# mozendr/FHE-SPEAR

Measured on AMD Instinct MI355X. Metric: BSGS matvecs/sec at d=2048,N=16384,L0=36; sec/RWKV-block at 1/2/4/8 GPU, higher is better.
Workload: dtype u64

## Files before the change

### fhe-spear_amd/csrc/fhs_host.hip

```cpp
#include <execinfo.h>
#include <hip/hip_runtime.h>
#include <unistd.h>

#include <algorithm>
#include <csignal>
#include <atomic>
#include <cmath>
#include <complex>
#include <cstdio>
#include <cstring>
#include <map>
#include <unordered_map>
#include <chrono>
#include <memory>
#include <mutex>
#include <set>
#include <string>
#include <thread>
#include <vector>

#include "../../include/fhespear.h"
#include "fhs_kernels.h"
#include "fhs_modarith.h"
#include "fhs_tables.h"

using fhs::DevTables;
using fhs::KsItem;

static thread_local std::string g_err;
static fhs_status fail(fhs_status code, const std::string& msg) {
    g_err = msg;
    return code;
}
static void segv_trace(int sig) {
    void* fr[64];
    const int n = backtrace(fr, 64);
    static const char hdr[] = "[fhespear] native backtrace:\n";
    (void)!write(2, hdr, sizeof(hdr) - 1);
    backtrace_symbols_fd(fr, n, 2);
    signal(sig, SIG_DFL);
    raise(sig);
}
__attribute__((constructor)) static void segv_trace_install() {
    if (getenv("FHESPEAR_SEGV_TRACE")) signal(SIGSEGV, segv_trace);
}
static fhs_status hip_fail(hipError_t e, const char* where) {
    if (e == hipErrorOutOfMemory || e == hipErrorMemoryAllocation)
        return fail(FHS_ERR_OOM, std::string("HIP out of memory in ") + where);
    return fail(FHS_ERR_HIP, std::string("HIP error in ") + where + ": " + hipGetErrorString(e));
}
#define HIPCHK(expr, where)                                  \
    do {                                                     \
        hipError_t _e = (expr);                              \
        if (_e != hipSuccess) return hip_fail(_e, where);    \
    } while (0)

extern "C" const char* fhs_last_error(void) { return g_err.c_str(); }
extern "C" const char* fhs_version(void) { return "fhespear-mi355x 0.1 (gfx950)"; }
extern "C" int fhs_device_count(void) {
    int n = 0;
    if (hipGetDeviceCount(&n) != hipSuccess) return 0;
    return n;
}
extern "C" fhs_status fhs_device_pci_bus_id(int device, char* buf, int len) {
    if (!buf || len < 13) return fail(FHS_ERR_INVALID, "device_pci_bus_id: buffer of at least 13 bytes");
    hipError_t e = hipDeviceGetPCIBusId(buf, len, device);
    if (e != hipSuccess) return hip_fail(e, "device_pci_bus_id");
    return FHS_OK;
}

extern "C" fhs_status fhs_create_coeff_modulus(uint64_t N, const int* bits, int n, uint64_t* out) {
    if (!bits || !out || n <= 0 || N < 2 || (N & (N - 1))) return fail(FHS_ERR_INVALID, "create_coeff_modulus: bad args");
    for (int i = 0; i < n; ++i)
        if (bits[i] < 2 || bits[i] > 61) return fail(FHS_ERR_INVALID, "create_coeff_modulus: bit size must be in [2, 61]");
    if (!coeff_modulus_search(N, bits, n, out)) return fail(FHS_ERR_INVALID, "create_coeff_modulus: not enough primes");
    return FHS_OK;
}
extern "C" uint64_t fhs_galois_elt_from_step(int step, uint64_t N) { return galois_elt_from_step(step, N); }

struct PendingRot {
    KsItem item;
    fhs_ciphertext* out;
    const fhs_ciphertext* in;
};

struct fhs_context {
    int device = 0;
    hipStream_t st = nullptr;
    std::recursive_mutex mu;
    uint64_t N = 0;
    int logN = 0, L0 = 0, P = 0, K = 0, dnum = 0;
    std::vector<uint64_t> q;
    std::vector<uint64_t> elts;
    DevTables T{};
    std::vector<void*> tables;
    void* items_dev = nullptr;
    void* ptrs_dev = nullptr;
    std::vector<PendingRot> pending;
    int pending_l = -1;
    std::set<const void*> pending_refs;
    std::set<const void*> pending_outs;
    int debug_fail_flushes = 0;
    int debug_fail_alloc = -1;
    std::vector<std::complex<double>> fft_w;
    std::vector<std::complex<double>> dec_twist;
    std::vector<uint64_t> slot_index;
    std::atomic<uint64_t> bytes_live{0};
    std::atomic<int> refs{1};
    std::unordered_map<size_t, std::vector<void*>> free_blocks;
    std::unordered_map<const void*, uint64_t*> key_a;
    size_t cached_bytes = 0;
    size_t cache_cap = 0;
    uint64_t cache_tick = 0;
    std::unordered_map<size_t, uint64_t> size_tick;
    uint32_t timer_mask = 0;
    std::vector<hipEvent_t> timer_open;
    std::vector<std::vector<std::pair<hipEvent_t, hipEvent_t>>> timer_pairs;
    fhs::KTimer ktimer{};
    unsigned char* ring = nullptr;
    size_t ring_head = 0;
    int ring_seg = 0;
    static constexpr size_t kRingBytes = 16u << 20;
    static constexpr int kRingSegs = 8;
    static constexpr size_t kSegBytes = kRingBytes / kRingSegs;
    hipEvent_t ring_ev[kRingSegs] = {};
    uint64_t ring_waits = 0, ring_blocked = 0;
    fhs::Stager stager{};
    std::map<std::pair<int, int>, std::vector<uint64_t>> crt_cache;
    double* readback = nullptr;
    size_t readback_bytes = 0;
    std::map<std::pair<const uint64_t*, int>, uint64_t*> seal_corr;
    size_t seal_corr_bytes = 0;
    size_t seal_corr_cap = 0;
    fhs::SealHoist seal_hoist{};
    enum { SCR_KS, SCR_BSGS_INNER, SCR_BSGS_WS, SCR_BSGS_SUM, SCR_RESCALE, SCR_ENC_PTRS, SCR_COUNT };
    uint64_t* scr[SCR_COUNT] = {};
    size_t scr_bytes[SCR_COUNT] = {};
    static constexpr int kMaxItems = 512;
    static constexpr int kMaxPtrs = 1 << 16;
};

struct fhs_ciphertext {
    fhs_context* ctx;
    uint64_t* d;
    int ncomp, ci, l;
    double scale;
    bool lost = false;
    struct PtSlab* slab = nullptr;
};
struct PtSlab {
    uint64_t* base;
    size_t bytes;
    int refs;
};
struct fhs_plaintext {
    fhs_context* ctx;
    uint64_t* d;
    int ci, l;
    double scale;
    PtSlab* slab = nullptr;
    uint64_t* dc = nullptr;
    int tlog = 0;
    PtSlab* cslab = nullptr;
};
struct fhs_secret_key {
    fhs_context* ctx;
    uint64_t* s;
    PrfKey key;
    uint64_t ctr;
    uint64_t pk_gen = 0;
};
struct fhs_public_key {
    fhs_context* ctx;
    uint64_t* pk;
    PrfKey rng;
    uint64_t ctr;
};
struct fhs_relin_key {
    fhs_context* ctx;
    uint64_t* key;
};
struct fhs_galois_keys {
    fhs_context* ctx;
    std::map<uint64_t, uint64_t*> keys;
};

static void ctx_retain(fhs_context* c) { c->refs.fetch_add(1); }

static std::mutex g_live_mu;
static std::set<fhs_context*> g_live;
static void trim_cache(fhs_context* c);
static void release_at_exit() {
    std::lock_guard<std::mutex> lk(g_live_mu);
    for (fhs_context* c : g_live) {
        std::unique_lock<std::recursive_mutex> cl(c->mu, std::try_to_lock);
        if (cl.owns_lock()) trim_cache(c);
    }
}
static void ctx_release(fhs_context* c);

static size_t key_words(const fhs_context* c) { return (size_t)c->dnum * c->K * c->N + (size_t)c->dnum; }
static size_t key_words_full(const fhs_context* c) { return (size_t)c->dnum * 2 * c->K * c->N; }
static void dfree(fhs_context* c, void* p, size_t bytes);
static const uint64_t* key_akey(const fhs_context* c, const uint64_t* key) {
    auto it = c->key_a.find(key);
    return it == c->key_a.end() ? nullptr : it->second;
}
static void drop_seal_corr(fhs_context* c, const uint64_t* key);
static void free_key(fhs_context* c, uint64_t* key) {
    if (!key) return;
    drop_seal_corr(c, key);
    auto it = c->key_a.find(key);
    if (it != c->key_a.end()) {
        dfree(c, it->second, 8ull * c->dnum * c->K * c->N);
        c->key_a.erase(it);
    }
    dfree(c, key, 8 * key_words(c));
}

static void ctx_sync(fhs_context* c) {
    hipStreamSynchronize(c->st);
}
static void trim_cache(fhs_context* c) {
    if (c->free_blocks.empty()) return;
    if (getenv("FHESPEAR_TRACE_LIFETIME"))
        fprintf(stderr, "[fhespear] trim: %zu cached bytes in %zu sizes, %llu live\n", c->cached_bytes,
                c->free_blocks.size(), (unsigned long long)c->bytes_live.load());
    ctx_sync(c);
    for (auto& kv : c->free_blocks)
        for (void* p : kv.second) (void)hipFree(p);
    c->free_blocks.clear();
    c->cached_bytes = 0;
}
static void trim_other_caches(fhs_context* self) {
    std::lock_guard<std::mutex> lk(g_live_mu);
    for (fhs_context* c : g_live) {
        if (c == self || c->device != self->device) continue;
        std::unique_lock<std::recursive_mutex> cl(c->mu, std::try_to_lock);
        if (cl.owns_lock()) trim_cache(c);
    }
}
static void evict_cold(fhs_context* c, size_t keep) {
    std::vector<void*> victims;
    while (c->cached_bytes > c->cache_cap) {
        size_t victim = 0;
        uint64_t oldest = ~0ull;
        for (auto& kv : c->free_blocks)
            if (kv.first != keep && !kv.second.empty() && c->size_tick[kv.first] < oldest) {
                oldest = c->size_tick[kv.first];
                victim = kv.first;
            }
        if (!victim) victim = keep;
        auto& v = c->free_blocks[victim];
        while (!v.empty() && c->cached_bytes > c->cache_cap) {
            victims.push_back(v.back());
            v.pop_back();
            c->cached_bytes -= victim;
        }
        if (v.empty()) c->free_blocks.erase(victim);
    }
    if (victims.empty()) return;
    ctx_sync(c);
    for (void* p : victims) (void)hipFree(p);
}
static hipError_t dalloc(fhs_context* c, uint64_t** p, size_t bytes) {
    if (c->debug_fail_alloc >= 0 && c->debug_fail_alloc-- == 0) return hipErrorOutOfMemory;
    bytes = bytes ? bytes : 8;
    c->size_tick[bytes] = ++c->cache_tick;
    auto it = c->free_blocks.find(bytes);
    if (it != c->free_blocks.end() && !it->second.empty()) {
        *p = static_cast<uint64_t*>(it->second.back());
        it->second.pop_back();
        c->cached_bytes -= bytes;
        c->bytes_live += bytes;
        return hipSuccess;
    }
    void* v = nullptr;
    hipError_t e = hipMalloc(&v, bytes);
    if (e == hipErrorOutOfMemory || e == hipErrorMemoryAllocation) {
        (void)hipGetLastError();
        trim_cache(c);
        trim_other_caches(c);
        e = hipMalloc(&v, bytes);
    }
    if (e == hipSuccess) {
        *p = (uint64_t*)v;
        c->bytes_live += bytes;
    } else {
        (void)hipGetLastError();
    }
    return e;
}
static void dfree(fhs_context* c, void* p, size_t bytes) {
    if (!p) return;
    bytes = bytes ? bytes : 8;
    c->free_blocks[bytes].push_back(p);
    c->cached_bytes += bytes;
    c->bytes_live -= bytes;
    c->size_tick[bytes] = ++c->cache_tick;
    if (c->cached_bytes > c->cache_cap) evict_cold(c, bytes);
}
struct DevTmp {
    fhs_context* c;
    uint64_t* p = nullptr;
// ... 383 lines not shown
    }
    const int U = (int)uniq.size();
    const size_t wsb = fhs::keyswitch_workspace_bytes(c->T, R, U, l);
    uint64_t* ws = nullptr;
    HostTrace ht;
    hipError_t e = c->debug_fail_flushes > 0 ? (--c->debug_fail_flushes, hipErrorOutOfMemory)
                                             : scratch(c, fhs_context::SCR_KS, wsb, &ws);
    ht.mark("flush: workspace");
    if (e != hipSuccess) return drop_pending(c, hip_fail(e, "key-switch workspace"));
    fhs::SealHoist* sh = nullptr;
    if (c->T.ks_seal && U < R) {
        e = seal_prepare(c, items, l);
        if (e == hipSuccess) sh = &c->seal_hoist;
        else if (e == hipErrorOutOfMemory || e == hipErrorMemoryAllocation) {
            for (auto& it : items) it.corr = nullptr;
            e = hipSuccess;
        }
        ht.mark("flush: seal corrections");
        if (e != hipSuccess) return drop_pending(c, hip_fail(e, "seal corrections"));
    }
    e = fhs::launch_keyswitch(c->T, items.data(), R, reinterpret_cast<const fhs::u64* const*>(uniq.data()), U, l, ws,
                              wsb, c->items_dev, c->stager, c->st, c->timer_mask ? &c->ktimer : nullptr, sh);
    ht.mark("flush: launch keyswitch");
    if (e != hipSuccess) return drop_pending(c, hip_fail(e, "key-switch launch"));
    return drop_pending(c, FHS_OK);
}

struct Guard {
    fhs_context* c;
    std::lock_guard<std::recursive_mutex> lk;
    explicit Guard(fhs_context* c_) : c(c_), lk(c_->mu) {}
};
static fhs_status live_ct(const fhs_ciphertext* a) {
    if (a && a->lost) return fail(FHS_ERR_INVALID, "ciphertext lost: the queued rotation producing it could not run "
                                                   "(an earlier call reported why)");
    return FHS_OK;
}
#define LIVE(ct)                                   \
    do {                                           \
        fhs_status _ls = live_ct(ct);              \
        if (_ls != FHS_OK) return _ls;             \
    } while (0)
#define ENTER(ctx)                                                           \
    if (!(ctx)) return fail(FHS_ERR_INVALID, "null context");               \
    Guard _g(ctx);                                                           \
    (void)hipGetLastError();  \
    do {                                                                     \
        fhs_status _s = flush(ctx);                                          \
        if (_s != FHS_OK) return _s;                                         \
    } while (0)

static void ctx_free(fhs_context* c);
static hipError_t upload_table(fhs_context* c, const void* src, size_t bytes, const void** dst) {
    void* d = nullptr;
    const hipError_t e = hipMalloc(&d, bytes);
    if (e != hipSuccess) return e;
    c->tables.push_back(d);
    *dst = d;
    return hipMemcpy(d, src, bytes, hipMemcpyHostToDevice);
}
extern "C" fhs_status fhs_context_create(uint64_t N, const uint64_t* primes, int nprimes, int special,
                                         const uint64_t* galois_elts, int n_elts, int device, fhs_context** out) {
    if (!out) return fail(FHS_ERR_INVALID, "context_create: null argument");
    if (const char* bad = context_params_error(N, primes, nprimes, special, galois_elts, n_elts))
        return fail(FHS_ERR_INVALID, bad);
    segv_trace_install();
    int ndev = 0;
    if (hipGetDeviceCount(&ndev) != hipSuccess || ndev == 0)
        return fail(FHS_ERR_NODEVICE, "no HIP device: libfhespear_hip needs an MI355X (gfx950)");
    if (device < 0 || device >= ndev) return fail(FHS_ERR_INVALID, "context_create: bad device index");
    HIPCHK(hipSetDevice(device), "hipSetDevice");

    HostTables H;
    if (const char* bad = build_host_tables(N, primes, nprimes, special, H)) return fail(FHS_ERR_INVALID, bad);

    std::unique_ptr<fhs_context, void (*)(fhs_context*)> c(new fhs_context, ctx_free);
    c->device = device;
    c->N = N; c->logN = H.logN; c->K = H.K; c->P = H.P; c->L0 = H.L0; c->dnum = H.dnum;
    c->q.assign(primes, primes + nprimes);
    c->elts = galois_elts && n_elts > 0 ? std::vector<uint64_t>(galois_elts, galois_elts + n_elts) : default_galois_elts(N);
    c->fft_w = std::move(H.fft_w);
    c->slot_index = std::move(H.slot_index);
    HIPCHK(hipStreamCreateWithFlags(&c->st, hipStreamNonBlocking), "hipStreamCreate");
    {
        static std::once_flag exit_once;
        std::call_once(exit_once, [] { atexit(release_at_exit); });
        size_t free_b = 0, total_b = 0;
        (void)hipMemGetInfo(&free_b, &total_b);
        c->cache_cap = total_b / 4;
        if (const char* e = getenv("FHESPEAR_CACHE_BYTES")) c->cache_cap = strtoull(e, nullptr, 10);
        c->seal_corr_cap = total_b ? total_b / 16 : (size_t)16 << 30;
        if (const char* e = getenv("FHESPEAR_SEAL_CORR_BYTES")) c->seal_corr_cap = strtoull(e, nullptr, 10);
    }
    DevTables& T = c->T;
    T.N = H.N; T.logN = H.logN; T.L0 = H.L0; T.P = H.P; T.K = H.K; T.dnum = H.dnum;
    T.max_qbits = H.max_qbits; T.modup_dp = H.modup_dp; T.md_xform = H.md_xform;
    T.conv_b59 = H.conv_b59; T.all_b59 = H.all_b59;
#define UP(field, count) \
    HIPCHK(upload_table(c.get(), H.field.data(), sizeof(H.field[0]) * (count), (const void**)&T.field), "tables")
#define UP_ALL(field) UP(field, H.field.size())
    UP_ALL(primes); UP_ALL(tw_fwd); UP_ALL(tw_inv);
    UP_ALL(modup_intt); UP_ALL(modup_hat); UP_ALL(modup_R); UP_ALL(modup_Q); UP_ALL(modup_xd); UP_ALL(modup_xt);
    UP_ALL(md_xd); UP_ALL(md_intt); UP_ALL(md_hat); UP_ALL(md_pinv);
    UP_ALL(rescale); UP_ALL(pow2);
    UP_ALL(dec_w); UP(dec_twist, N / 2); UP_ALL(dec_pos);
    UP_ALL(enc_w); UP_ALL(enc_twist); UP_ALL(enc_pos);
#undef UP_ALL
#undef UP
    c->dec_twist = std::move(H.dec_twist);
    HIPCHK(hipHostMalloc(reinterpret_cast<void**>(&c->ring), fhs_context::kRingBytes, hipHostMallocDefault),
           "staging ring");
    c->stager = fhs::Stager{c.get(), stage_h2d};
    HIPCHK(hipMalloc(&c->items_dev, (sizeof(KsItem) + sizeof(void*)) * fhs_context::kMaxItems), "items buffer");
    c->tables.push_back(c->items_dev);
    HIPCHK(hipMalloc(&c->ptrs_dev, sizeof(void*) * 2 * fhs_context::kMaxPtrs), "pointer buffer");
    c->tables.push_back(c->ptrs_dev);
    {
        std::lock_guard<std::mutex> lk(g_live_mu);
        g_live.insert(c.get());
    }
    *out = c.release();
    return FHS_OK;
}

static void ctx_free(fhs_context* c) {
    const bool trace = getenv("FHESPEAR_TRACE_LIFETIME") != nullptr;
    if (trace)
        fprintf(stderr, "[fhespear] context %p: freeing (%zu cached bytes, %llu live)\n", (void*)c, c->cached_bytes,
                (unsigned long long)c->bytes_live.load());
    {
        Guard g(c);
        flush(c);
        if (c->st) {
            hipStreamSynchronize(c->st);
            ctx_sync(c);
        }
        for (void* p : c->tables) hipFree(p);
        for (auto& kv : c->seal_corr) hipFree(kv.second);
        c->seal_corr.clear();
        if (c->seal_hoist.zflag_dev) hipFree(c->seal_hoist.zflag_dev);
        if (c->seal_hoist.zflag_host) hipHostFree(c->seal_hoist.zflag_host);
        for (int k = 0; k < fhs_context::SCR_COUNT; ++k)
            if (c->scr[k]) hipFree(c->scr[k]);
        {
            std::lock_guard<std::mutex> lk(g_live_mu);
            g_live.erase(c);
        }
        for (auto& kv : c->free_blocks)
            for (void* p : kv.second) hipFree(p);
        c->free_blocks.clear();
        if (c->ring) hipHostFree(c->ring);
        if (c->readback) hipHostFree(c->readback);
        for (hipEvent_t e : c->ring_ev)
            if (e) hipEventDestroy(e);
        for (auto& v : c->timer_pairs)
            for (auto& pr : v) { ev_put(pr.first); ev_put(pr.second); }
        for (hipEvent_t e : c->timer_open)
            if (e) ev_put(e);
        if (c->st) hipStreamDestroy(c->st);
    }
    delete c;
    if (trace) fprintf(stderr, "[fhespear] context %p: freed\n", (void*)c);
}
static void ctx_release(fhs_context* c) {
    if (c->refs.fetch_sub(1) == 1) ctx_free(c);
}
extern "C" fhs_status fhs_context_destroy(fhs_context* c) {
    if (!c) return FHS_OK;
    ctx_release(c);
    return FHS_OK;
}
extern "C" fhs_status fhs_context_info(const fhs_context* c, uint64_t* N, int* L0, int* P, int* n_elts) {
    if (!c) return fail(FHS_ERR_INVALID, "null context");
    if (N) *N = c->N;
    if (L0) *L0 = c->L0;
    if (P) *P = c->P;
    if (n_elts) *n_elts = (int)c->elts.size();
    return FHS_OK;
}
extern "C" fhs_status fhs_context_galois_elts(const fhs_context* c, uint64_t* out) {
    if (!c || !out) return fail(FHS_ERR_INVALID, "null argument");
    std::copy(c->elts.begin(), c->elts.end(), out);
    return FHS_OK;
}
extern "C" fhs_status fhs_synchronize(fhs_context* c) {
    ENTER(c);
    HIPCHK(hipStreamSynchronize(c->st), "hipStreamSynchronize");
    return FHS_OK;
}
extern "C" fhs_status fhs_memory_in_use(fhs_context* c, uint64_t* bytes) {
    if (!c || !bytes) return fail(FHS_ERR_INVALID, "null argument");
    *bytes = c->bytes_live.load();
    return FHS_OK;
}

static bool os_random(void* buf, size_t n) {
    FILE* f = fopen("/dev/urandom", "rb");
    if (!f) return false;
    const size_t got = fread(buf, 1, n, f);
    fclose(f);
    return got == n;
}
static uint64_t prf_u64(const PrfKey& K, uint64_t sid) {
    uint64_t w0, w1;
    prf128(K, sid, 0, w0, w1);
    return w0;
}
static uint64_t stream_id(uint64_t kind, uint64_t a, uint64_t b) { return (kind << 56) | (a << 16) | b; }
static bool parity_rng() {
    const char* v = getenv("FHESPEAR_PARITY_RNG");
    if (!v || strcmp(v, "1") != 0) return false;
    static std::atomic<bool> warned{false};
    if (!warned.exchange(true))
        fprintf(stderr, "[fhespear] FHESPEAR_PARITY_RNG=1: deterministic encryption randomness (parity tests "
                        "only; never for real data)\n");
    return true;
}
enum { ST_SECRET = 1, ST_PUBKEY = 2, ST_RELIN = 3, ST_GALOIS = 4, ST_ENC_SYM = 5, ST_ENC_ASYM = 6, ST_PK_RNG = 7 };

static hipError_t sample_small_ntt(fhs_context* c, int mode, const PrfKey& K, uint64_t sid, uint64_t* out, int limbs) {
    hipError_t e = fhs::launch_sample(c->T, mode, K, sid, out, limbs, c->st);
    if (e != hipSuccess) return e;
    return fhs::launch_ntt_fwd(c->T, out, limbs, limbs, 1, 0, c->st);
}

extern "C" fhs_status fhs_secret_key_create(fhs_context* c, const uint8_t* key32, fhs_secret_key** out) {
    ENTER(c);
    if (!out) return fail(FHS_ERR_INVALID, "null out");
    PrfKey K{};
    if (key32) {
        for (int w = 0; w < 8; ++w)
            K.k[w] = (uint32_t)key32[4 * w] | ((uint32_t)key32[4 * w + 1] << 8) | ((uint32_t)key32[4 * w + 2] << 16) |
                     ((uint32_t)key32[4 * w + 3] << 24);
    } else if (!os_random(K.k, sizeof(K.k))) {
        return fail(FHS_ERR_INVALID, "secret_key: /dev/urandom unavailable");
    }
    uint64_t ctr0 = 0;
    if (!parity_rng() && !os_random(&ctr0, sizeof ctr0)) return fail(FHS_ERR_INVALID, "secret_key: /dev/urandom unavailable");
    auto sk = adopt_key(new fhs_secret_key{c, nullptr, K, ctr0 & ((1ull << 39) - 1)});
    HIPCHK(dalloc(c, &sk->s, 8ull * c->K * c->N), "secret key");
    HIPCHK(sample_small_ntt(c, fhs::SAMPLE_TERNARY, sk->key, stream_id(ST_SECRET, 0, 0), sk->s, c->K),
// ... 296 lines not shown
    delete ct;
    ctx_release(c);
    return FHS_OK;
}
extern "C" fhs_status fhs_plaintext_destroy(fhs_plaintext* pt) {
    if (!pt) return FHS_OK;
    fhs_context* c = pt->ctx;
    {
        Guard g(c);
        if (pt->slab) {
            if (--pt->slab->refs == 0) {
                dfree(c, pt->slab->base, pt->slab->bytes);
                delete pt->slab;
            }
        } else {
            dfree(c, pt->d, pt_bytes(pt));
        }
        if (pt->cslab && --pt->cslab->refs == 0) {
            dfree(c, pt->cslab->base, pt->cslab->bytes);
            delete pt->cslab;
        }
    }
    delete pt;
    ctx_release(c);
    return FHS_OK;
}
static constexpr int kMaxBatch = 4096;
extern "C" fhs_status fhs_ciphertext_info(const fhs_ciphertext* ct, int* ncomp, int* ci, int* l, double* scale) {
    if (!ct) return fail(FHS_ERR_INVALID, "null ciphertext");
    if (ncomp) *ncomp = ct->ncomp;
    if (ci) *ci = ct->ci;
    if (l) *l = ct->l;
    if (scale) *scale = ct->scale;
    return FHS_OK;
}
extern "C" fhs_status fhs_ciphertext_set_scale(fhs_ciphertext* ct, double scale) {
    if (!ct) return fail(FHS_ERR_INVALID, "null ciphertext");
    ct->scale = scale;
    return FHS_OK;
}
extern "C" fhs_status fhs_plaintext_info(const fhs_plaintext* pt, int* ci, int* l, double* scale) {
    if (!pt) return fail(FHS_ERR_INVALID, "null plaintext");
    if (ci) *ci = pt->ci;
    if (l) *l = pt->l;
    if (scale) *scale = pt->scale;
    return FHS_OK;
}
extern "C" fhs_status fhs_ciphertext_export(fhs_context* c, const fhs_ciphertext* ct, uint64_t* host) {
    ENTER(c);
    if (!ct || !host) return fail(FHS_ERR_INVALID, "null argument");
    LIVE(ct);
    return export_dev(c, ct->d, ct_bytes(ct), host);
}
extern "C" fhs_status fhs_plaintext_export(fhs_context* c, const fhs_plaintext* pt, uint64_t* host) {
    ENTER(c);
    if (!pt || !host) return fail(FHS_ERR_INVALID, "null argument");
    PT_DENSE(pd, pt, "plaintext_export");
    return export_dev(c, pd, pt_bytes(pt), host);
}
extern "C" fhs_status fhs_ciphertext_import(fhs_context* c, const uint64_t* host, int ncomp, int ci, double scale,
                                            fhs_ciphertext** out) {
    ENTER(c);
    if (!host || !out || ncomp < 2 || ncomp > 3) return fail(FHS_ERR_INVALID, "ciphertext_import: bad args");
    NEW_CT(ct, ncomp, ci, scale);
    HIPCHK(hipMemcpyAsync(ct->d, host, ct_bytes(ct.p), hipMemcpyHostToDevice, c->st), "ciphertext_import");
    HIPCHK(hipStreamSynchronize(c->st), "ciphertext_import");
    *out = ct.release();
    return FHS_OK;
}
extern "C" fhs_status fhs_plaintext_import(fhs_context* c, const uint64_t* host, int ci, double scale,
                                           fhs_plaintext** out) {
    ENTER(c);
    if (!host || !out) return fail(FHS_ERR_INVALID, "plaintext_import: bad args");
    NEW_PT(pt, ci, scale);
    HIPCHK(hipMemcpyAsync(pt->d, host, pt_bytes(pt.p), hipMemcpyHostToDevice, c->st), "plaintext_import");
    HIPCHK(hipStreamSynchronize(c->st), "plaintext_import");
    *out = pt.release();
    return FHS_OK;
}
extern "C" fhs_status fhs_debug_fail_next_flushes(fhs_context* c, int count) {
    if (!c || count < 0) return fail(FHS_ERR_INVALID, "debug_fail_next_flushes: bad args");
    Guard g(c);
    c->debug_fail_flushes = count;
    return FHS_OK;
}
extern "C" fhs_status fhs_debug_fail_alloc(fhs_context* c, int nth, int* was_armed) {
    if (!c) return fail(FHS_ERR_INVALID, "debug_fail_alloc: null context");
    Guard g(c);
    if (was_armed) *was_armed = c->debug_fail_alloc >= 0;
    c->debug_fail_alloc = nth < 0 ? -1 : nth;
    return FHS_OK;
}
extern "C" fhs_status fhs_debug_launch_ledger(int op, char* buf, uint64_t len, uint64_t* needed) {
    if (op == FHS_LEDGER_ARM || op == FHS_LEDGER_DISARM) {
        fhs::ledger_arm(op == FHS_LEDGER_ARM);
        return FHS_OK;
    }
    if (op != FHS_LEDGER_READ) return fail(FHS_ERR_INVALID, "debug_launch_ledger: unknown operation");
    const std::string names = fhs::ledger_read();
    if (needed) *needed = names.size() + 1;
    if (!buf || len < names.size() + 1) return fail(FHS_ERR_INVALID, "debug_launch_ledger: buffer too short");
    memcpy(buf, names.c_str(), names.size() + 1);
    return FHS_OK;
}
extern "C" fhs_status fhs_ciphertext_device_ptr(const fhs_ciphertext* ct, void** dptr, uint64_t* bytes) {
    if (!ct || !dptr) return fail(FHS_ERR_INVALID, "null argument");
    fhs_context* c = ct->ctx;
    Guard g(c);
    fhs_status s = flush(c);
    if (s != FHS_OK) return s;
    LIVE(ct);
    *dptr = ct->d;
    if (bytes) *bytes = ct_bytes(ct);
    return FHS_OK;
}

static void fft_inplace(std::vector<std::complex<double>>& a, const std::vector<std::complex<double>>& w, int logN,
                        size_t wstride = 1) {
    const size_t n = a.size();
    for (size_t i = 0; i < n; ++i) {
        const size_t r = h_bitrev((uint32_t)i, logN);
        if (r > i) std::swap(a[i], a[r]);
    }
    double* x = reinterpret_cast<double*>(a.data());
    const double* wt = reinterpret_cast<const double*>(w.data());
    for (size_t len = 2; len <= n; len <<= 1) {
        const size_t step = n / len * wstride, h = len / 2;
        for (size_t i = 0; i < n; i += len) {
            for (size_t k = 0; k < h; ++k) {
                const double wr = wt[2 * k * step], wi = wt[2 * k * step + 1];
                double* u = x + 2 * (i + k);
                double* v = x + 2 * (i + k + h);
                const double vr = v[0] * wr - v[1] * wi, vi = v[0] * wi + v[1] * wr;
                v[0] = u[0] - vr;
                v[1] = u[1] - vi;
                u[0] += vr;
                u[1] += vi;
            }
        }
    }
}


static hipError_t enc_periods(fhs_context* c, const double* dvals, size_t cnt, size_t n, size_t stride, bool is_real,
                              DevTmp& tl) {
    static const bool dense = getenv("FHESPEAR_ENCODE_DENSE") != nullptr;
    const int smax = fhs::encode_sparse_max_log(c->logN);
    if (dense || smax < 1 || n != c->N / 2 || cnt == 0) return hipSuccess;
    hipError_t e = tl.alloc((cnt + 7) & ~(size_t)7);
    if (e != hipSuccess) return e;
    return fhs::launch_enc_period(dvals, (int)cnt, n, stride, is_real, smax, tl.as<unsigned char>(), c->st);
}
static fhs_status new_pts_compact(fhs_context* c, size_t count, int ci, double scale, int tlog, fhs_plaintext** outs) {
    const int l = c->L0 + 1 - ci;
    const size_t per = (size_t)l * (c->N >> tlog);
    auto* cs = new PtSlab{nullptr, 8 * count * per, 0};
    hipError_t e = dalloc_fit(c, &cs->base, &cs->bytes);
    if (e != hipSuccess) {
        delete cs;
        return hip_fail(e, "plaintext allocation");
    }
    for (size_t k = 0; k < count; ++k) {
        outs[k] = new fhs_plaintext{c, nullptr, ci, l, scale};
        outs[k]->dc = cs->base + k * per;
        outs[k]->tlog = tlog;
        outs[k]->cslab = cs;
// ... 1011 lines not shown
    fhs_ciphertext* r;
    fhs_status s = new_ct(c, 2, a->ci, a->scale, &r);
    if (s != FHS_OK) return s;
    const size_t S = (size_t)a->l * c->N;
    c->pending.push_back(PendingRot{KsItem{a->d + S, a->d, nullptr, it->second, r->d, r->d + S, elt, 0,
                                           key_akey(c, it->second)}, r, a});
    c->pending_l = a->l;
    c->pending_refs.insert(r);
    c->pending_refs.insert(a);
    c->pending_outs.insert(r);
    *out = r;
    return FHS_OK;
}
extern "C" fhs_status fhs_rotate(fhs_context* c, const fhs_ciphertext* a, int step, const fhs_galois_keys* gk,
                                 fhs_ciphertext** out) {
    if (!c) return fail(FHS_ERR_INVALID, "null context");
    Guard g(c);
    if (step == 0 || std::abs(step) >= (int)(c->N / 2)) {
        if (step == 0) return fail(FHS_ERR_INVALID, "rotate: step 0 (use apply_galois for conjugation)");
        return fail(FHS_ERR_INVALID, "rotate: |step| must be < slot count");
    }
    return queue_rotation(c, a, fhs_galois_elt_from_step(step, c->N), gk, out);
}
extern "C" fhs_status fhs_apply_galois(fhs_context* c, const fhs_ciphertext* a, uint64_t elt, const fhs_galois_keys* gk,
                                       fhs_ciphertext** out) {
    if (!c) return fail(FHS_ERR_INVALID, "null context");
    Guard g(c);
    return queue_rotation(c, a, elt, gk, out);
}
extern "C" fhs_status fhs_rotate_many(fhs_context* c, const fhs_ciphertext* const* in, const int* steps, int n,
                                      const fhs_galois_keys* gk, fhs_ciphertext** out) {
    if (!c) return fail(FHS_ERR_INVALID, "null context");
    Guard g(c);
    for (int i = 0; i < n; ++i) {
        fhs_status s = queue_rotation(c, in[i], fhs_galois_elt_from_step(steps[i], c->N), gk, &out[i]);
        if (s != FHS_OK) return s;
    }
    return flush(c);
}

static fhs_status bsgs_core(fhs_context* c, const fhs_ciphertext* const* baby, int G, const uint64_t* const* pt_ptrs,
                            int D, int B, int ci, double pt_scale, const fhs_galois_keys* gk, fhs_ciphertext** out,
                            const uint64_t* giant_elts = nullptr, bool rescale = true, int ptl = 0) {
    if (G < 1 || D < 1 || !baby) return fail(FHS_ERR_INVALID, "bsgs: bad G/D");
    const int Beff = std::min(B, (D + G - 1) / G);
    if (Beff < 1) return fail(FHS_ERR_INVALID, "bsgs: no giant groups");
    if (G > 2048 || (size_t)D + G > (size_t)fhs_context::kMaxPtrs) return fail(FHS_ERR_INVALID, "bsgs: too many diagonals");
    const int l = baby[0]->l;
    for (int b = 0; b < G; ++b) {
        if (!baby[b] || baby[b]->l != l || baby[b]->ncomp != 2 || baby[b]->ci != ci)
            return fail(FHS_ERR_LEVEL, "bsgs: baby steps and diagonals must share one chain index");
        LIVE(baby[b]);
    }
    if (rescale && l < 2) return fail(FHS_ERR_LEVEL, "bsgs: no level left for the final rescale");
    if (giant_elts && giant_elts[0] != 1) return fail(FHS_ERR_INVALID, "linear_transform: giant group 0 must be the identity");
    HostTrace ht;
    std::vector<const uint64_t*> keys(Beff, nullptr), akeys(Beff, nullptr);
    for (int g = 1; g < Beff; ++g) {
        const uint64_t elt = giant_elts ? giant_elts[g] : fhs_galois_elt_from_step(g * G, c->N);
        auto it = gk->keys.find(elt);
        if (it == gk->keys.end()) return fail(FHS_ERR_KEY, "bsgs: galois key for a giant step is missing");
        keys[g] = it->second;
        akeys[g] = key_akey(c, it->second);
    }
    const size_t S = (size_t)l * c->N;
    std::vector<const uint64_t*> ptrs(G + D);
    for (int b = 0; b < G; ++b) ptrs[b] = baby[b]->d;
    for (int k = 0; k < D; ++k) ptrs[G + k] = pt_ptrs[k];
    ht.mark("keys+ptrs");
    HIPCHK(stage_h2d(c, c->ptrs_dev, ptrs.data(), sizeof(void*) * (G + D)), "bsgs");
    ht.mark("stage ptrs");
    const uint64_t* const* dbaby = reinterpret_cast<const uint64_t* const*>(c->ptrs_dev);
    const uint64_t* const* dpts = dbaby + G;
    uint64_t* inner = nullptr;
    HIPCHK(scratch(c, fhs_context::SCR_BSGS_INNER, 8ull * Beff * 2 * S, &inner), "bsgs inner products");
    const fhs::KTimer* tm = c->timer_mask ? &c->ktimer : nullptr;
    const size_t wsb = std::max<size_t>(8, fhs::bsgs_workspace_bytes(c->T, Beff - 1, l));
    uint64_t* ws = nullptr;
    HIPCHK(scratch(c, fhs_context::SCR_BSGS_WS, wsb, &ws), "bsgs workspace");
    uint64_t* sum = nullptr;
    HIPCHK(scratch(c, fhs_context::SCR_BSGS_SUM, 16 * S, &sum), "bsgs sum");
    ht.mark("workspaces");
    HIPCHK(fhs::launch_bsgs(c->T, dbaby, dpts, G, Beff, D, l, keys.data(), akeys.data(), giant_elts, inner, sum, ws, wsb,
                            c->items_dev, c->stager, c->st, tm, ptl),
           "bsgs");
    ht.mark("launch bsgs");
    if (!rescale) {
        NEW_CT(r, 2, ci, baby[0]->scale * pt_scale);
        HIPCHK(hipMemcpyAsync(r->d, sum, 8 * 2 * S, hipMemcpyDeviceToDevice, c->st), "linear_transform");
        *out = r.release();
        return FHS_OK;
    }
    NEW_CT(r, 2, ci + 1, baby[0]->scale * pt_scale / (double)c->q[l - 1]);
    uint64_t* scr = nullptr;
    HIPCHK(scratch(c, fhs_context::SCR_RESCALE, 16ull * c->N, &scr), "bsgs rescale");
    HIPCHK(fhs::launch_rescale(c->T, sum, r->d, scr, 2, l, c->st, tm), "bsgs rescale");
    ht.mark("rescale+frees");
    *out = r.release();
    return FHS_OK;
}

static int pts_ptl(const fhs_context* c, const fhs_plaintext* const* pts, int D) {
    static const bool dense = getenv("FHESPEAR_BSGS_DENSE") != nullptr;
    if (dense || D < 1 || c->T.max_qbits > 59 || !pts[0]->dc) return 0;
    for (int k = 1; k < D; ++k)
        if (!pts[k]->dc || pts[k]->tlog != pts[0]->tlog) return 0;
    return pts[0]->tlog;
}
extern "C" fhs_status fhs_bsgs_multiply_accumulate(fhs_context* c, const fhs_ciphertext* const* baby, int G,
                                                   const fhs_plaintext* const* pts, int D, int B,
                                                   const fhs_galois_keys* gk, fhs_ciphertext** out) {
    ENTER(c);
    if (!pts || !gk || !out || !baby) return fail(FHS_ERR_INVALID, "null argument");
    std::vector<const uint64_t*> p(D);
    for (int k = 0; k < D; ++k) {
        if (!pts[k] || pts[k]->ci != baby[0]->ci) return fail(FHS_ERR_LEVEL, "bsgs: diagonal at a different chain index");
        if (!scales_close(pts[k]->scale, pts[0]->scale)) return fail(FHS_ERR_SCALE, "bsgs: diagonal scales differ");
    }
    const int ptl = pts_ptl(c, pts, D);
    for (int k = 0; k < D; ++k) {
        p[k] = pts[k]->dc;
        if (!ptl) HIPCHK(pt_dense(c, pts[k], &p[k]), "bsgs");
    }
    return bsgs_core(c, baby, G, p.data(), D, B, baby[0]->ci, pts[0]->scale, gk, out, nullptr, true, ptl);
}

static fhs_status inner_products_core(fhs_context* c, const fhs_ciphertext* const* baby, int G,
                                      const fhs_plaintext* const* pts, int B, uint64_t* dst) {
    if (G < 1 || G > 2048 || B < 1) return fail(FHS_ERR_INVALID, "bsgs_inner_products: 1 <= G <= 2048, B >= 1");
    const int D = B * G, ci = baby[0]->ci, l = baby[0]->l;
    if ((size_t)D + G > (size_t)fhs_context::kMaxPtrs) return fail(FHS_ERR_INVALID, "bsgs_inner_products: too many plaintexts");
    std::vector<const uint64_t*> ptrs(G + D);
    for (int b = 0; b < G; ++b) {
        if (!baby[b] || baby[b]->l != l || baby[b]->ncomp != 2 || baby[b]->ci != ci)
            return fail(FHS_ERR_LEVEL, "bsgs_inner_products: baby steps must share one chain index");
        LIVE(baby[b]);
        ptrs[b] = baby[b]->d;
    }
    for (int k = 0; k < D; ++k) {
        if (!pts[k] || pts[k]->ci != ci) return fail(FHS_ERR_LEVEL, "bsgs_inner_products: plaintext at a different chain index");
        if (!scales_close(pts[k]->scale, pts[0]->scale)) return fail(FHS_ERR_SCALE, "bsgs_inner_products: plaintext scales differ");
    }
    const int ptl = pts_ptl(c, pts, D);
    for (int k = 0; k < D; ++k) {
        ptrs[G + k] = pts[k]->dc;
        if (!ptl) HIPCHK(pt_dense(c, pts[k], &ptrs[G + k]), "bsgs_inner_products");
    }
    HIPCHK(stage_h2d(c, c->ptrs_dev, ptrs.data(), sizeof(void*) * (G + D)), "bsgs_inner_products");
    const uint64_t* const* dbaby = reinterpret_cast<const uint64_t* const*>(c->ptrs_dev);
    HIPCHK(fhs::launch_bsgs_inner(c->T, dbaby, dbaby + G, G, 0, B, D, l, dst, c->st, ptl), "bsgs_inner_products");
    return FHS_OK;
}
extern "C" fhs_status fhs_bsgs_inner_products(fhs_context* c, const fhs_ciphertext* const* baby, int G,
                                              const fhs_plaintext* const* pts, int B, fhs_ciphertext** outs) {
    ENTER(c);
    if (!pts || !outs || !baby || !baby[0]) return fail(FHS_ERR_INVALID, "null argument");
    const int ci = baby[0]->ci;
    const size_t S = (size_t)baby[0]->l * c->N;
    uint64_t* inner = nullptr;
    HIPCHK(scratch(c, fhs_context::SCR_BSGS_INNER, 8ull * std::max(B, 1) * 2 * S, &inner), "bsgs_inner_products");
    fhs_status cs = inner_products_core(c, baby, G, pts, B, inner);
    if (cs != FHS_OK) return cs;
    BatchOutT<fhs_ciphertext> bo(outs, (size_t)B);
    for (int g = 0; g < B; ++g) {
        fhs_status st = new_ct(c, 2, ci, baby[0]->scale * pts[0]->scale, &outs[g]);
        if (st != FHS_OK) return st;
        HIPCHK(hipMemcpyAsync(outs[g]->d, inner + (size_t)g * 2 * S, 16 * S, hipMemcpyDeviceToDevice, c->st),
// ... 56 lines not shown
    uint64_t* tdst = (!rk && !rescale) ? outs[0]->d : t3;
    HIPCHK(fhs::launch_dot_tensor(c->T, dq, dq + J, J, C, l, tdst, c->st, tm), "dot_product_many");
    if (rk) {
        uint64_t* kdst = rescale ? relin : outs[0]->d;
        const uint64_t* akey = key_akey(c, rk->key);
        for (int c0 = 0; c0 < C; c0 += kDotKsBatch) {
            const int R = std::min(kDotKsBatch, C - c0);
            std::vector<KsItem> items(R);
            std::vector<const uint64_t*> uniq(R);
            for (int r = 0; r < R; ++r) {
                const uint64_t* t = t3 + (size_t)(c0 + r) * 3 * S;
                uint64_t* o = kdst + (size_t)(c0 + r) * 2 * S;
                items[r] = KsItem{t + 2 * S, t, t + S, rk->key, o, o + S, 1, (uint64_t)r, akey};
                uniq[r] = t + 2 * S;
            }
            HIPCHK(fhs::launch_keyswitch(c->T, items.data(), R, reinterpret_cast<const fhs::u64* const*>(uniq.data()), R,
                                         l, ws, wsb, c->items_dev, c->stager, c->st, tm), "key-switch");
        }
    }
    if (rescale) HIPCHK(fhs::launch_rescale(c->T, rk ? relin : t3, outs[0]->d, scr, ocomp * C, l, c->st, tm), "rescale");
    return bo.keep(FHS_OK);
}

template <int FOLD>
static void dot_accumulate_host(const RedU& R, const uint64_t* a0, const uint64_t* a1, const uint64_t* b0,
                                const uint64_t* b1, int J, uint64_t* out3) {
    for (int j0 = 0; j0 < J; j0 += kDotWindowMax) {
        const int Jw = std::min(kDotWindowMax, J - j0);
        Dot3 s;
        dot3_clear(s);
        for (int j = 0; j < Jw; ++j)
            dot3_term<FOLD>(s, j, unpack30(pack30(a0[j0 + j])), unpack30(pack30(a1[j0 + j])), split30(b0[j0 + j]),
                            split30(b1[j0 + j]));
        uint64_t prev[3] = {out3[0], out3[1], out3[2]};
        dot3_finish(s, R, j0 ? prev : nullptr, out3);
    }
}
extern "C" fhs_status fhs_debug_dot_accumulate(uint64_t q, const uint64_t* a0, const uint64_t* a1, const uint64_t* b0,
                                               const uint64_t* b1, int J, uint64_t* out3) {
    if (!a0 || !a1 || !b0 || !b1 || !out3 || J < 1) return fail(FHS_ERR_INVALID, "debug_dot_accumulate: bad argument");
    if (q < 3 || q >= (1ull << 60)) return fail(FHS_ERR_INVALID, "debug_dot_accumulate: q must be < 2^60");
    for (int j = 0; j < J; ++j)
        if (a0[j] >= q || a1[j] >= q || b0[j] >= q || b1[j] >= q)
            return fail(FHS_ERR_INVALID, "debug_dot_accumulate: operands must be < q");
    const uint64_t w = pm_word(q, 14);
    const hu128 r = ~(hu128)0 / q;
    const RedU R{q, (uint64_t)r, (uint64_t)(r >> 64), (unsigned)(w & 127), (unsigned)((w >> 8) & 0xFFFFFFFFu), false, false};
    out3[0] = out3[1] = out3[2] = 0;
    if (q < (1ull << 59)) dot_accumulate_host<16>(R, a0, a1, b0, b1, J, out3);
    else dot_accumulate_host<8>(R, a0, a1, b0, b1, J, out3);
    return FHS_OK;
}

template <class Src>
static fhs_status giant_steps_core(fhs_context* c, Src src, int k, int ci, double scale, const uint64_t* elts,
                                   const fhs_galois_keys* gk, fhs_ciphertext** out) {
    const int l = c->L0 + 1 - ci;
    for (int j = 0; j < k; ++j) {
        if ((elts[j] & 1) == 0 || elts[j] >= 2 * c->N) return fail(FHS_ERR_INVALID, "bsgs_giant_steps: bad Galois element");
        if (j > 0 && elts[j] == 1) return fail(FHS_ERR_INVALID, "bsgs_giant_steps: only the first term may be unrotated");
    }
    const int pad = elts[0] == 1 ? 0 : 1, B = k + pad;
    std::vector<uint64_t> ge(B, 1);
    std::vector<const uint64_t*> keys(B, nullptr), akeys(B, nullptr);
    for (int g = 1; g < B; ++g) {
        ge[g] = elts[g - pad];
        auto it = gk->keys.find(ge[g]);
        if (it == gk->keys.end()) return fail(FHS_ERR_KEY, "bsgs_giant_steps: galois key missing");
        keys[g] = it->second;
        akeys[g] = key_akey(c, it->second);
    }
    const size_t S = (size_t)l * c->N;
    uint64_t *inner = nullptr, *ws = nullptr, *sum = nullptr;
    HIPCHK(scratch(c, fhs_context::SCR_BSGS_INNER, 8ull * B * 2 * S, &inner), "bsgs_giant_steps");
    if (pad) HIPCHK(hipMemsetAsync(inner, 0, 16 * S, c->st), "bsgs_giant_steps");
    for (int j = 0; j < k; ++j)
        HIPCHK(hipMemcpyAsync(inner + (size_t)(j + pad) * 2 * S, src(j), 16 * S, hipMemcpyDeviceToDevice, c->st),
               "bsgs_giant_steps");
    const size_t wsb = std::max<size_t>(8, fhs::bsgs_workspace_bytes(c->T, B - 1, l));
    HIPCHK(scratch(c, fhs_context::SCR_BSGS_WS, wsb, &ws), "bsgs_giant_steps");
    HIPCHK(scratch(c, fhs_context::SCR_BSGS_SUM, 16 * S, &sum), "bsgs_giant_steps");
    const fhs::KTimer* tm = c->timer_mask ? &c->ktimer : nullptr;
    HIPCHK(fhs::launch_bsgs(c->T, nullptr, nullptr, 1, B, B, l, keys.data(), akeys.data(), ge.data(), inner, sum, ws, wsb,
                            c->items_dev, c->stager, c->st, tm),
           "bsgs_giant_steps");
    NEW_CT(r, 2, ci, scale);
    HIPCHK(hipMemcpyAsync(r->d, sum, 16 * S, hipMemcpyDeviceToDevice, c->st), "bsgs_giant_steps");
    *out = r.release();
    return FHS_OK;
}
extern "C" fhs_status fhs_bsgs_giant_steps(fhs_context* c, const fhs_ciphertext* const* inners, int k,
                                           const uint64_t* elts, const fhs_galois_keys* gk, fhs_ciphertext** out) {
    ENTER(c);
    if (!inners || !elts || !gk || !out || k < 1 || !inners[0]) return fail(FHS_ERR_INVALID, "null argument");
    if (k > 511) return fail(FHS_ERR_INVALID, "bsgs_giant_steps: 1 <= k <= 511");
    const int l = inners[0]->l, ci = inners[0]->ci;
    for (int j = 0; j < k; ++j) {
        if (!inners[j] || inners[j]->ncomp != 2 || inners[j]->l != l || inners[j]->ci != ci)
            return fail(FHS_ERR_LEVEL, "bsgs_giant_steps: inner products must be 2-component at one chain index");
        LIVE(inners[j]);
        if (!scales_close(inners[j]->scale, inners[0]->scale)) return fail(FHS_ERR_SCALE, "bsgs_giant_steps: scales differ");
    }
    return giant_steps_core(c, [&](int j) { return inners[j]->d; }, k, ci, inners[0]->scale, elts, gk, out);
}
extern "C" fhs_status fhs_bsgs_giant_steps_device(fhs_context* c, const uint64_t* src, int k, int chain_index,
                                                  double scale, const uint64_t* elts, const fhs_galois_keys* gk,
                                                  fhs_ciphertext** out) {
    ENTER(c);
    if (!src || !elts || !gk || !out) return fail(FHS_ERR_INVALID, "null argument");
    if (k < 1 || k > 511) return fail(FHS_ERR_INVALID, "bsgs_giant_steps: 1 <= k <= 511");
    if (chain_index < 1 || chain_index > c->L0) return fail(FHS_ERR_LEVEL, "bsgs_giant_steps: bad chain index");
    const size_t W = 2 * (size_t)(c->L0 + 1 - chain_index) * c->N;
    return giant_steps_core(c, [&](int j) { return src + (size_t)j * W; }, k, chain_index, scale, elts, gk, out);
}

extern "C" fhs_status fhs_linear_transform(fhs_context* c, const fhs_ciphertext* const* baby, int G,
                                           const fhs_plaintext* const* pts, int D, int B, const uint64_t* giant_elts,
                                           const fhs_galois_keys* gk, int rescale, fhs_ciphertext** out) {
    ENTER(c);
    if (!pts || !gk || !out || !baby || !giant_elts) return fail(FHS_ERR_INVALID, "null argument");
    if (B < 1 || D != B * G) return fail(FHS_ERR_INVALID, "linear_transform: expects D = B * G plaintexts");
    std::vector<const uint64_t*> p(D);
    for (int k = 0; k < D; ++k) {
        if (!pts[k] || pts[k]->ci != baby[0]->ci) return fail(FHS_ERR_LEVEL, "linear_transform: plaintext at a different chain index");
        if (!scales_close(pts[k]->scale, pts[0]->scale)) return fail(FHS_ERR_SCALE, "linear_transform: plaintext scales differ");
    }
    const int ptl = pts_ptl(c, pts, D);
    for (int k = 0; k < D; ++k) {
        p[k] = pts[k]->dc;
        if (!ptl) HIPCHK(pt_dense(c, pts[k], &p[k]), "linear_transform");
    }
    for (int g = 0; g < B; ++g)
        if ((giant_elts[g] & 1) == 0 || giant_elts[g] >= 2 * c->N) return fail(FHS_ERR_INVALID, "linear_transform: bad Galois element");
    return bsgs_core(c, baby, G, p.data(), D, B, baby[0]->ci, pts[0]->scale, gk, out, giant_elts, rescale != 0, ptl);
}

static uint64_t dbl_int_mod(double p, uint64_t q) {
    const bool neg = p < 0;
    const double a = std::fabs(p);
    uint64_t r;
    if (a < 18446744073709551616.0) {
        r = (uint64_t)a % q;
    } else {
        int e;
        const double f = std::frexp(a, &e);
        const uint64_t m = (uint64_t)std::ldexp(f, 53);
        r = h_mulmod(m % q, h_pow(2, (uint64_t)(e - 53), q), q);
    }
    return neg && r ? q - r : r;
}
static fhs_status scalar_consts(fhs_context* c, double v, int l, fhs::ScalarConsts& K) {
    if (!std::isfinite(v)) return fail(FHS_ERR_INVALID, "constant is not finite");
    if (l > fhs::kMaxScalarLimbs) return fail(FHS_ERR_INVALID, "too many limbs for a constant op");
    const double p = std::round(v);
    for (int i = 0; i < l; ++i) {
        K.v[i] = dbl_int_mod(p, c->q[i]);
        K.vs[i] = h_shoup(K.v[i], c->q[i]);
    }
    return FHS_OK;
}
extern "C" fhs_status fhs_multiply_const(fhs_context* c, const fhs_ciphertext* a, double value, double const_scale,
                                         fhs_ciphertext** out) {
    ENTER(c);
    if (!a || !out) return fail(FHS_ERR_INVALID, "null argument");
    LIVE(a);
    if (!(const_scale > 0) || !std::isfinite(const_scale)) return fail(FHS_ERR_INVALID, "multiply_const: bad scale");
    fhs::ScalarConsts K;
// ... 445 lines not shown
```

### fhe-spear_amd/csrc/fhs_kernels.h

```cpp
#pragma once
#include <hip/hip_runtime.h>
#include <stdint.h>

#include <string>

struct PrfKey;

namespace fhs {

typedef uint64_t u64;

struct DevTables {
    const void* primes;
    const u64* tw_fwd;
    const u64* tw_inv;
    const u64* modup_intt;
    const u64* modup_hat;
    const u64* modup_R;
    const u64* modup_Q;
    const u64* modup_xd;
    const u64* modup_xt;
    const u64* md_xd;
    const u64* md_intt;
    const u64* md_hat;
    const u64* md_pinv;
    const u64* rescale;
    const u64* pow2;
    const double* enc_w;
    const double* enc_twist;
    const unsigned* enc_pos;
    const double* dec_w;
    const double* dec_twist;
    const unsigned* dec_pos;
    int N, logN, L0, P, K, dnum;
    int ks_seal;
    int max_qbits;
    int md_xform;
    int conv_b59;
    int all_b59;
    int modup_dp;
};
#ifndef FHS_NTT_HALF_MIN
#define FHS_NTT_HALF_MIN 14
#endif
constexpr bool ks_uses_half(int logN) { return logN >= 9; }
static_assert(FHS_NTT_HALF_MIN >= 9, "N = 256 runs the full-limb kernels only");
inline bool modup_xform(const DevTables& T, int l) { return T.modup_dp == 3 && l % 3 == 0 && ks_uses_half(T.logN); }

struct KsItem {
    const u64* a;
    const u64* add0;
    const u64* add1;
    const u64* key;
    u64* out0;
    u64* out1;
    u64 elt;
    u64 src;
    const u64* akey;
    const u64* corr;
};

struct SealHoist {
    unsigned* zflag_dev;
    unsigned* zflag_host;
    unsigned long long hoisted = 0, fallback = 0;
};
hipError_t launch_seal_corr(const DevTables& T, const u64* key, const u64* akey, u64 elt, int l, u64* mask_scratch,
                            u64* out, hipStream_t st);

enum KernelId { KID_BSGS_INNER = 0, KID_MODUP = 1, KID_KS_IP = 2, KID_MODDOWN = 3, KID_KS_INTT = 4, KID_SPECIAL_INTT = 5,
                KID_GIANT_SUM = 6, KID_GIANT_FINAL = 7, KID_RESCALE = 8, KID_DOT_TENSOR = 9, KID_ENCRYPT_PK = 10,
                KID_COUNT = 11 };
struct KTimer {
    void* ctx;
    void (*rec)(void* ctx, int id, int begin, hipStream_t st);
};
#define FHS_TMARK(tm, id, b, st) do { if (tm) (tm)->rec((tm)->ctx, (id), (b), (st)); } while (0)

hipError_t launch_ntt_fwd(const DevTables& T, u64* data, int limbs, int l_split, int npoly, size_t poly_stride,
                          hipStream_t st);
hipError_t launch_ntt_inv(const DevTables& T, u64* data, int limbs, int l_split, int npoly, size_t poly_stride,
                          hipStream_t st);
hipError_t launch_eltwise(const DevTables& T, int op, const u64* a, const u64* b, u64* out, int ncomp, int l,
                          size_t a_cstride, size_t b_cstride, hipStream_t st);
hipError_t launch_tensor(const DevTables& T, const u64* a, const u64* b, u64* out3, int l, hipStream_t st);
hipError_t launch_rescale(const DevTables& T, const u64* in, u64* out, u64* scratch, int ncomp, int l,
                          hipStream_t st, const KTimer* tm = nullptr);
struct Stager {
    void* user;
    hipError_t (*h2d)(void* user, void* dst, const void* src, size_t bytes);
};
hipError_t launch_keyswitch(const DevTables& T, const KsItem* items_host, int R, const u64* const* uniq_host, int U,
                            int l, u64* workspace, size_t ws_bytes, void* items_dev, const Stager& sg, hipStream_t st,
                            const KTimer* tm, SealHoist* sh = nullptr);
size_t keyswitch_workspace_bytes(const DevTables& T, int R, int U, int l);

size_t bsgs_workspace_bytes(const DevTables& T, int R, int l);
hipError_t launch_bsgs(const DevTables& T, const u64* const* baby_dev, const u64* const* pts_dev, int G, int B, int D,
                       int l, const u64* const* keys_host, const u64* const* akeys_host, const u64* giant_elts, u64* inner,
                       u64* out, u64* workspace, size_t ws_bytes, void* items_dev, const Stager& sg, hipStream_t st,
                       const KTimer* tm, int ptl = 0);
hipError_t launch_bsgs_inner(const DevTables& T, const u64* const* baby_dev, const u64* const* pts_dev, int G, int g0,
                             int g1, int D, int l, u64* inner, hipStream_t st, int ptl = 0);
hipError_t launch_dot_tensor(const DevTables& T, const u64* const* q_dev, const u64* const* db_dev, int J, int C, int l,
                             u64* out3, hipStream_t st, const KTimer* tm = nullptr);
hipError_t launch_encode(const DevTables& T, const double* vals, int count, size_t n, size_t stride, bool is_real,
                         double scale, u64* const* outs_dev, int l, hipStream_t st,
                         double* coef_scratch = nullptr, const unsigned char* tlog = nullptr,
                         u64* const* couts_dev = nullptr, int ss = 0);
hipError_t launch_enc_period(const double* vals, int count, size_t n, size_t stride, bool is_real, int smax,
                             unsigned char* tlog, hipStream_t st);
int encode_sparse_max_log(int logN);
hipError_t launch_expand_compact(const u64* dc, u64* d, int l, int N, int tl, hipStream_t st);
hipError_t launch_sample(const DevTables& T, int mode, const ::PrfKey& K, u64 sid, u64* out, int l, hipStream_t st,
                         int npoly = 1, u64 sid_step = 0, u64* const* outs_dev = nullptr);
hipError_t launch_switch_key_assemble(const DevTables& T, u64* b_out, const u64* a, const u64* e_ntt, const u64* s_ntt,
                                      const u64* snew_ntt, int digit, hipStream_t st);
hipError_t launch_galois_perm(const DevTables& T, const u64* in, u64* out, int limbs, u64 elt, hipStream_t st);
hipError_t launch_encrypt_sym_batch(const DevTables& T, const ::PrfKey& K, u64 sid_mask, u64 sid_err, u64 sid_step,
                                    u64* const* cts_dev, const u64* s, const u64* const* pts_dev, int count, int l,
                                    signed char* small, u64* eb, hipStream_t st, const double* coef = nullptr);
hipError_t launch_encode_coef(const DevTables& T, const double* vals, int count, size_t n, size_t stride, bool is_real,
                              double scale, double* coef, hipStream_t st, const unsigned char* tlog = nullptr);
hipError_t launch_encrypt_pk_batch(const DevTables& T, const ::PrfKey& K, u64 sid, u64 sid_step, u64* cts,
                                   const u64* pk0, const u64* pk1, const u64* const* pts_dev, const u64* pt,
                                   const double* coef, int count, int l, signed char* small, u64* ub, hipStream_t st,
                                   const KTimer* tm = nullptr);
hipError_t launch_encrypt_combine(const DevTables& T, int mode, u64* c0, u64* c1, const u64* s_or_pk0, const u64* pk1,
                                  const u64* u_ntt, const u64* e0, const u64* e1, const u64* pt, int l, hipStream_t st);
hipError_t launch_decrypt(const DevTables& T, const u64* ct, int ncomp, const u64* s, u64* out, int l, hipStream_t st);
hipError_t launch_decrypt_many(const DevTables& T, const u64* const* cts_dev, int count, int ncomp, const u64* s, u64* out,
                               size_t out_stride, int l, hipStream_t st);
hipError_t launch_diag_gather(const double* M1, const double* M2, int D, int G, int n, int k0, int rows, int trans,
                              double* out, hipStream_t st);
hipError_t launch_decode_slots(const DevTables& T, const double* m, const double* scales, int count, double* spec,
                               int nslots, double* out, hipStream_t st);
hipError_t launch_key_prod(const DevTables& T, const u64* a, const u64* b, u64* out, int limbs, hipStream_t st);
constexpr int kCrtMaxL = 7;
struct CrtConsts {
    int l, W;
    u64 q[kCrtMaxL], ihat[kCrtMaxL], ihat_s[kCrtMaxL];
    u64 hat[kCrtMaxL][kCrtMaxL + 1];
    u64 Q[kCrtMaxL + 1], halfQ[kCrtMaxL + 1];
};
hipError_t launch_crt_compose(const CrtConsts& K, const u64* limbs, double* out, int N, hipStream_t st);
constexpr int kCrtVtabWords = 3 + kCrtMaxL + 1;
struct CrtJob {
    CrtConsts K;
    const u64* limbs;
    double* out;
    const u64* extra;
    const u64* vtab;
    unsigned* flag;
    int nx, pad;
};
hipError_t launch_crt_compose_jobs(const CrtJob* jobs_dev, int count, int max_nx, int N, hipStream_t st);

constexpr int kMaxScalarLimbs = 64;
struct ScalarConsts {
    u64 v[kMaxScalarLimbs];
    u64 vs[kMaxScalarLimbs];
};
enum ScalarOp { SCALAR_MUL = 0, SCALAR_ADD = 1 };
hipError_t launch_scalar(const DevTables& T, int op, const u64* a, u64* out, int ncomp, int l, const ScalarConsts& K,
                         hipStream_t st);
hipError_t launch_mod_raise(const DevTables& T, const u64* in, int l, u64* out, u64* scratch, int ncomp,
                            hipStream_t st);

hipError_t launch_encode_int128(const DevTables& T, const int64_t* hi, const u64* lo, int count, u64* const* outs_dev,
                                int l, hipStream_t st);

enum EltOp { OP_ADD = 0, OP_SUB = 1, OP_NEG = 2, OP_MULP = 3, OP_ADDP = 4, OP_SUBP = 5, OP_SUBNEG = 6 };
enum SampleMode { SAMPLE_UNIFORM = 0, SAMPLE_TERNARY = 1, SAMPLE_CBD = 2, SAMPLE_SEEDED = 3, SAMPLE_TESTDATA = 4 };

void ledger_arm(bool on);
std::string ledger_read();

}
```

### fhe-spear_amd/csrc/fhs_kernels.hip

```cpp
#include "fhs_kernels.h"
typedef unsigned long long u64x2_t __attribute__((ext_vector_type(2)));
#ifndef FHS_MODUP_STORE_AUX
#define FHS_MODUP_STORE_AUX 2
#endif
#ifndef FHS_KSIP_UNROLL
#define FHS_KSIP_UNROLL 4
#endif
#include "fhs_ntt.h"
#include "fhs_buffer.h"

#include <atomic>
#include <cxxabi.h>
#include <mutex>
#include <set>
#include <string>
#include <cstdio>
#include <cstdlib>
#include <cstring>
#include <vector>
#include <algorithm>

#define FHS_INNER_WAVES 16
#define FHS_INNER_VEC 2
#ifndef FHS_MODUPH_CH
#define FHS_MODUPH_CH 2
#endif
#ifndef FHS_MODUPH_RL
#define FHS_MODUPH_RL 3
#endif
#define FHS_NTT_RL 3
#ifndef FHS_FWD_FIRST3
#define FHS_FWD_FIRST3 1
#endif
#ifndef FHS_KSIP_HALVES
#define FHS_KSIP_HALVES 1
#endif

namespace fhs {

static std::atomic<bool> g_ledger_armed{false};
static std::mutex g_ledger_mu;
static std::set<const void*> g_ledger;
static void ledger_note(const void* k) {
    std::lock_guard<std::mutex> g(g_ledger_mu);
    g_ledger.insert(k);
}
#define FHS_LAUNCH(K, ...)                                                                                 \
    do {                                                                                                   \
        if (g_ledger_armed.load(std::memory_order_relaxed)) ledger_note(reinterpret_cast<const void*>(K)); \
        hipLaunchKernelGGL(K, __VA_ARGS__);                                                                \
    } while (0)
void ledger_arm(bool on) {
    std::lock_guard<std::mutex> g(g_ledger_mu);
    if (on) g_ledger.clear();
    g_ledger_armed.store(on, std::memory_order_relaxed);
}
static std::string ledger_normalise(const std::string& demangled) {
    auto outside = [](const std::string& s, const char* tok, bool last) {
        const size_t n = strlen(tok);
        long found = -1;
        int depth = 0;
        for (size_t i = 0; i < s.size(); ++i) {
            if (s[i] == '<') ++depth;
            else if (s[i] == '>') --depth;
            else if (depth == 0 && s.compare(i, n, tok) == 0) {
                found = (long)i;
                if (!last) break;
            }
        }
        return found;
    };
    std::string s = demangled;
    long i = outside(s, "(", false);
    if (i >= 0) s.resize(i);
    i = outside(s, " ", true);
    if (i >= 0) s.erase(0, i + 1);
    i = outside(s, "::", true);
    if (i >= 0) s.erase(0, i + 2);
    return s;
}
std::string ledger_read() {
    std::vector<const void*> ptrs;
    {
        std::lock_guard<std::mutex> g(g_ledger_mu);
        ptrs.assign(g_ledger.begin(), g_ledger.end());
    }
    std::set<std::string> names;
    for (const void* p : ptrs) {
        const char* mangled = hipKernelNameRefByPtr(p, nullptr);
        if (!mangled || !*mangled) {
            char buf[32];
            snprintf(buf, sizeof buf, "?%p", p);
            names.insert(buf);
            continue;
        }
        int status = 0;
        char* d = abi::__cxa_demangle(mangled, nullptr, nullptr, &status);
        names.insert(ledger_normalise(status == 0 && d ? d : mangled));
        free(d);
    }
    std::string out;
    for (const std::string& n : names) out += n + "\n";
    return out;
}

#define FHS_DISPATCH_LOGN(logN, ...)                   \
    switch (logN) {                                    \
        case 8: { constexpr int LOGN = 8; __VA_ARGS__; } break;   \
        case 9: { constexpr int LOGN = 9; __VA_ARGS__; } break;   \
        case 10: { constexpr int LOGN = 10; __VA_ARGS__; } break; \
        case 11: { constexpr int LOGN = 11; __VA_ARGS__; } break; \
        case 12: { constexpr int LOGN = 12; __VA_ARGS__; } break; \
        case 13: { constexpr int LOGN = 13; __VA_ARGS__; } break; \
        case 14: { constexpr int LOGN = 14; __VA_ARGS__; } break; \
        case 15: { constexpr int LOGN = 15; __VA_ARGS__; } break; \
        default: return hipErrorInvalidValue;          \
    }

__device__ __forceinline__ const PrimeK& PK(const DevTables& T, int i) {
    return reinterpret_cast<const PrimeK*>(T.primes)[i];
}

__host__ __device__ __forceinline__ int xcd_grid(int E, int M) { return 8 * ((E + 7) / 8) * M; }
__device__ __forceinline__ bool xcd_tinner(int E, int M, int& t, int& m) {
    const int b = blockIdx.x, x = b & 7, k = b >> 3, nx = (E - x + 7) >> 3;
    if (nx <= 0 || k >= nx * M) return false;
    t = x + 8 * (k % nx);
    m = k / nx;
    return true;
}
__host__ __device__ __forceinline__ int xcd_grid_q(int E, int M) { return 8 * ((E + 3) / 4) * ((M + 1) / 2); }
__device__ __forceinline__ bool xcd_quadpair(int E, int M, int& t, int& m) {
    const int b = blockIdx.x, x = b & 7, k = b >> 3, pg = x & 3, mh = x >> 2;
    const int nx = (E - pg + 3) >> 2, nm = (M - mh + 1) >> 1;
    if (nx <= 0 || nm <= 0 || k >= nx * nm) return false;
    t = pg + 4 * (k % nx);
    m = mh + 2 * (k / nx);
    return true;
}
__device__ __forceinline__ bool plain_tm(int E, int M, int& t, int& m) {
    t = blockIdx.x % E;
    m = blockIdx.x / E;
    return m < M;
}
__device__ __forceinline__ bool xcd_touter(int E, int M, int& t, int& m) {
    const int b = blockIdx.x, x = b & 7, k = b >> 3, nx = (E - x + 7) >> 3;
    if (nx <= 0 || k >= nx * M) return false;
    t = x + 8 * (k / M);
    m = k % M;
    return true;
}
__device__ __forceinline__ int limb_prime(int b, int l_split, int L0) { return b < l_split ? b : L0 + (b - l_split); }

__device__ __forceinline__ int galois_src(int e, u64 elt, int logN) {
    if (elt == 1) return e;
    const unsigned r = __brev((unsigned)e) >> (32 - logN);
    const u64 m = (u64)2 << logN;
    const u64 e2 = ((2 * (u64)r + 1) * elt) & (m - 1);
    return (int)(__brev((unsigned)((e2 - 1) >> 1)) >> (32 - logN));
}

template <int LOGN, bool B59>
__device__ __forceinline__ bool lazy_of(const RedU& R) { return (B59 && LOGN <= 14) || R.lazy; }

template <int LOGN>
constexpr size_t lds_bytes() { return (size_t)((1 << LOGN) + (1 << LOGN) / 16) * 8; }

template <int LOGN> constexpr bool ntt_half() { return LOGN >= FHS_NTT_HALF_MIN; }
template <int LOGN, bool H = ntt_half<LOGN>()> constexpr int ntt_threads() { return H ? (1 << LOGN) / 32 : (1 << LOGN) / 16; }
template <int LOGN, bool H = ntt_half<LOGN>()> constexpr int ntt_lds_words() {
    return H ? (1 << (LOGN - 1)) + (1 << (LOGN - 1)) / 16 : (1 << LOGN) + (1 << LOGN) / 16;
}
#ifndef FHS_FULL_FORM_MAX_WG
#define FHS_FULL_FORM_MAX_WG 256
#endif
#define FHS_NTT_LAUNCH(K, nwg, grid, st, ...)                                                          \
    do {                                                                                               \
        constexpr bool FH_ = (LOGN > 14);                      \
        if ((nwg) < FHS_FULL_FORM_MAX_WG && !FH_)                                                      \
            FHS_LAUNCH((K<LOGN, FH_>), grid, dim3(ntt_threads<LOGN, FH_>()), 0, st, __VA_ARGS__); \
        else                                                                                           \
            FHS_LAUNCH((K<LOGN>), grid, dim3(ntt_threads<LOGN>()), 0, st, __VA_ARGS__);        \
    } while (0)
struct Tw4 {
    u64 w1, w1p, w2, w2p, w3, w3p;
};
__device__ __forceinline__ Tw4 ld_tw4(const u64* __restrict__ tw) {
    Tw4 t;
    ld_tw(tw, 1, t.w1, t.w1p);
    ld_tw(tw, 2, t.w2, t.w2p);
    ld_tw(tw, 3, t.w3, t.w3p);
    return t;
}
template <int TH>
__device__ __forceinline__ void fwd_quad_first2(u64 x[4], const Tw4& w, u64 q, bool lazy, u64* lds, int tid, int c,
                                                u64 hi[16]) {
    const u64 q2 = 2 * q;
#pragma unroll
    for (int k = 0; k < 2; ++k) {
        const u64 tt = shoup_lazy(x[2 + k], w.w1, w.w1p, q);
        const u64 X = x[k];
        x[k] = X + tt;
        x[2 + k] = X + (q2 - tt);
    }
    if (!lazy) {
        x[0] = x[0] >= q2 ? x[0] - q2 : x[0];
        x[2] = x[2] >= q2 ? x[2] - q2 : x[2];
    }
    const u64 ta = shoup_lazy(x[1], w.w2, w.w2p, q), tb = shoup_lazy(x[3], w.w3, w.w3p, q);
    lds[row_pad<TH>(tid, c)] = x[0] + ta;
    lds[row_pad<TH>(tid, c + 8)] = x[0] + (q2 - ta);
    hi[c] = x[2] + tb;
    hi[c + 8] = x[2] + (q2 - tb);
}
template <int TH>
__device__ __forceinline__ void fwd_oct_first3(u64 x[8], const u64* __restrict__ tw, u64 q, bool lazy, u64* lds,
                                               int tid, int c, u64 hi[16]) {
    const u64 q2 = 2 * q;
    auto bfly = [&](int a, int b, int wi) {
        u64 w, wp;
        ld_tw(tw, wi, w, wp);
        u64 X = x[a];
        if (!lazy) X = X >= q2 ? X - q2 : X;
        const u64 t = shoup_lazy(x[b], w, wp, q);
        x[a] = X + t;
        x[b] = X + (q2 - t);
    };
#pragma unroll
    for (int k = 0; k < 4; ++k) bfly(k, k + 4, 1);
#pragma unroll
    for (int k = 0; k < 8; k += 4) {
        bfly(k, k + 2, 2 + k / 4);
        bfly(k + 1, k + 3, 2 + k / 4);
    }
// ... 325 lines not shown
    constexpr int N = 1 << LOGN, NH = N / 2, TH = N / 32;
    __shared__ __attribute__((aligned(16))) u64 lds[ntt_lds_words<LOGN, true>()];
    const int i = blockIdx.x, comp = blockIdx.y, g = blockIdx.z, tid = threadIdx.x;
    const PrimeK& P = PK(T, i);
    const RedU RU = redu(P);
    const u64* rs = T.rescale + ((size_t)l * T.L0 + i) * 4;
    const u64 inv = rs[0], inv_s = rs[1], hq = rs[2], q = RU.q;
    const PrimeK& PL = PK(T, l - 1);
    const u64 qL = PL.q, halfL = qL >> 1;
    const u64* twL = T.tw_inv + (size_t)(l - 1) * N * 2;
    const u64* tw = T.tw_fwd + (size_t)i * N * 2;
    const u64* pr = pre + (size_t)comp * 2 * 16 * TH + tid;
    auto conv = [&](u64 y) { return submod(reduce64(addmod(csub(y, qL), halfL, qL), P), hq, q); };
    u64 hi[16];
#pragma unroll
    for (int c = 0; c < 4; ++c) {
        u64 x[8];
#pragma unroll
        for (int j = 0; j < 2; ++j) {
            const int r = c + 4 * j;
            u64 y[4] = {pr[(size_t)r * TH], pr[(size_t)(r + 8) * TH], pr[(size_t)(16 + r) * TH], pr[(size_t)(24 + r) * TH]};
            inv_quad_last2(y, twL, qL, PL.ninv, PL.ninv_s, PL.w1ninv, PL.w1ninv_s);
            x[j] = conv(y[0]);
            x[j + 2] = conv(y[1]);
            x[4 + j] = conv(y[2]);
            x[6 + j] = conv(y[3]);
        }
        fwd_oct_first3<TH>(x, tw, q, RU.lazy, lds, tid, c, hi);
    }
    if (g) {
#pragma unroll
        for (int c = 0; c < 16; ++c) lds[row_pad<TH>(tid, c)] = hi[c];
    }
    __syncthreads();
    const u64* a = in + ((size_t)comp * l + i) * N;
    u64* o = out + ((size_t)comp * (l - 1) + i) * N;
    constexpr bool WLX = FHS_NTT_WAVELOCAL && fwd_exit_wave_local<LOGN - 1, 3, 2>();
    ntt_fwd_lds<LOGN - 1, 3, 16, 2, WLX>(lds, tid, tw, q, RU.lazy, 1 + g);
    if constexpr (WLX) {
        const int wb = wl_base<LOGN - 1, 16, 8>(tid), wp = lds_pad(wb);
#pragma unroll
        for (int c = 0; c < 16; ++c) {
            const int off = wl_off<LOGN - 1, 16, 8>(c);
            const int e = g * NH + wb + off;
            o[e] = shoup(submod(a[e], fwd_canon(lds[wp + off + off / 16], RU), q), inv, inv_s, q);
        }
    } else {
#pragma unroll
        for (int c = 0; c < 16; ++c) {
            const int e = g * NH + tid + c * TH;
            o[e] = shoup(submod(a[e], fwd_canon(lds[row_pad<TH>(tid, c)], RU), q), inv, inv_s, q);
        }
    }
}
#ifndef FHS_SPLIT_MAX_WG
#define FHS_SPLIT_MAX_WG 256
#endif
hipError_t launch_rescale(const DevTables& T, const u64* in, u64* out, u64* scratch, int ncomp, int l,
                          hipStream_t st, const KTimer* tm) {
    FHS_TMARK(tm, KID_RESCALE, 1, st);
    FHS_DISPATCH_LOGN(T.logN, {
        if constexpr (LOGN == 15) {
            if (ncomp <= 2) {
                FHS_LAUNCH((k_rescale_intt_hs<LOGN>), dim3(2, ncomp), dim3(ntt_threads<LOGN, true>()), 0, st, T,
                           in, scratch, l);
                FHS_LAUNCH((k_rescale_ntt_hs<LOGN>), dim3(l - 1, ncomp, 2), dim3(ntt_threads<LOGN, true>()), 0, st,
                           T, in, scratch, out, l);
                break;
            }
        }
        FHS_NTT_LAUNCH(k_rescale_intt, ncomp, dim3(ncomp), st, T, in, scratch, l);
        FHS_NTT_LAUNCH(k_rescale_ntt, (l - 1) * ncomp, dim3(l - 1, ncomp), st, T, in, scratch, out, l);
    });
    FHS_TMARK(tm, KID_RESCALE, 0, st);
    return hipGetLastError();
}

template <int LOGN>
__global__ void __launch_bounds__((1 << LOGN) / 16) k_ks_intt(DevTables T, const u64* const* uniq, u64* acoef, int l, int U) {
    constexpr int N = 1 << LOGN, TH = N / 16;
    __shared__ __attribute__((aligned(16))) u64 lds[ntt_lds_words<LOGN, false>()];
    const int tid = threadIdx.x;
    int i, u;
    if (!plain_tm(l, U, i, u)) return;
    const PrimeK& P = PK(T, i);
    const u64* src = uniq[u] + (size_t)i * N;
#pragma unroll
    for (int c = 0; c < 16; ++c) lds[row_pad<TH>(tid, c)] = src[tid + c * TH];
    __syncthreads();
    const u64* cst = T.modup_intt + ((size_t)l * T.L0 + i) * 4;
    ntt_inv_lds<LOGN, FHS_NTT_RL>(lds, tid, T.tw_inv + (size_t)i * N * 2, P.q, cst[0], cst[1], cst[2], cst[3]);
    u64* dst = acoef + ((size_t)u * l + i) * N;
#pragma unroll
    for (int k = 0; k < 16; ++k) dst[tid + k * TH] = csub(lds[row_pad<TH>(tid, k)], P.q);
}

template <int LOGN>
__global__ void __launch_bounds__((1 << LOGN) / 32, 4) k_ks_intt_h(DevTables T, const u64* const* uniq, u64* acoef,
                                                                   int l, int U) {
    constexpr int N = 1 << LOGN, NH = N / 2, TH = N / 32;
    __shared__ __attribute__((aligned(16))) u64 lds[(1 << (LOGN - 1)) + (1 << (LOGN - 1)) / 16];
    const int tid = threadIdx.x;
    int i, u;
    if (!plain_tm(l, U, i, u)) return;
    const PrimeK& P = PK(T, i);
    const u64 q = P.q;
    const __amdgpu_buffer_rsrc_t rs = brsrc(uniq[u] + (size_t)i * N, N * 8);
    const u64* tw = T.tw_inv + (size_t)i * N * 2;
    u64 lo[16];
    constexpr bool WLI = FHS_NTT_WAVELOCAL && (LOGN - 2) % FHS_NTT_RL == 0;
    constexpr int GS = 1 << FHS_NTT_RL;
    const int tb = WLI ? wl_base<LOGN - 1, 16, GS>(tid) : tid;
    auto eoff = [&](int c) { return WLI ? wl_off<LOGN - 1, 16, GS>(c) : c * TH; };
    auto lidx = [&](int c) { return WLI ? lds_pad(tb) + eoff(c) + eoff(c) / 16 : row_pad<TH>(tid, c); };
#pragma unroll 1
    for (int h = 0; h < 2; ++h) {
        if (h) __syncthreads();
        u64 v[16];
#pragma unroll
        for (int c = 0; c < 16; ++c) v[c] = bload64(rs, tb * 8, (h * NH + eoff(c)) * 8);
#pragma unroll
        for (int c = 0; c < 16; ++c) lds[lidx(c)] = v[c];
        if constexpr (!WLI) __syncthreads();
        ntt_inv_half_lds<LOGN - 1, FHS_NTT_RL, 16, 1, WLI>(lds, tid, tw, q, 1 + h);
        if (h == 0) {
#pragma unroll
            for (int c = 0; c < 16; ++c) lo[c] = lds[row_pad<TH>(tid, c)];
        }
    }
    const u64* cst = T.modup_intt + ((size_t)l * T.L0 + i) * 4;
    const u64 s0 = cst[0], s0s = cst[1], s1 = cst[2], s1s = cst[3];
    const __amdgpu_buffer_rsrc_t rd = brsrc(acoef + ((size_t)u * l + i) * N, N * 8);
#pragma unroll
    for (int c = 0; c < 8; ++c) {
        u64 x[4] = {lo[c], lo[c + 8], lds[row_pad<TH>(tid, c)], lds[row_pad<TH>(tid, c + 8)]};
        inv_quad_last2(x, tw, q, s0, s0s, s1, s1s);
#pragma unroll
        for (int k = 0; k < 4; ++k)
            bstore64(csub(x[k], q), rd, tid * 8, ((k >> 1) * NH + (c + 8 * (k & 1)) * TH) * 8);
    }
}

__device__ __noinline__ int centered_exact(const u64* y, const u64* qs, int ns, int carry) {
    u64 X[10], Q[10], t[10];
    for (int w = 0; w < 10; ++w) { X[w] = 0; Q[w] = 0; }
    Q[0] = 1;
    for (int u = 0; u < ns; ++u) {
        u64 cy = 0;
        for (int w = 0; w < 10; ++w) {
            const u64 lo = Q[w] * qs[u], hi = __umul64hi(Q[w], qs[u]);
            const u64 z = lo + cy;
            cy = hi + (z < lo);
            Q[w] = z;
        }
    }
    for (int u = 0; u < ns; ++u) {
        for (int w = 0; w < 10; ++w) t[w] = 0;
        t[0] = y[u];
        for (int v = 0; v < ns; ++v) {
            if (v == u) continue;
            u64 cy = 0;
            for (int w = 0; w < 10; ++w) {
                const u64 lo = t[w] * qs[v], hi = __umul64hi(t[w], qs[v]);
                const u64 z = lo + cy;
                cy = hi + (z < lo);
                t[w] = z;
            }
        }
        u64 cy = 0;
        for (int w = 0; w < 10; ++w) {
            const u64 z1 = X[w] + t[w];
            const u64 c1 = z1 < X[w];
            const u64 z2 = z1 + cy;
            cy = c1 + (z2 < z1);
            X[w] = z2;
        }
    }
    const u64 mlt = (u64)(2 * carry + 1);
    u64 L[10], Rr[10], cl = 0, cr = 0;
    for (int w = 0; w < 10; ++w) {
        L[w] = (X[w] << 1) | cl;
        cl = X[w] >> 63;
        const u64 lo = Q[w] * mlt, hi = __umul64hi(Q[w], mlt);
        const u64 z = lo + cr;
        cr = hi + (z < lo);
        Rr[w] = z;
    }
    for (int w = 9; w >= 0; --w)
        if (L[w] != Rr[w]) return carry + (L[w] > Rr[w] ? 1 : 0);
    return carry + 1;
}

__global__ void k_centered(DevTables T, const u64* acoef, unsigned char* vout, int l, int U, unsigned* zflag) {
    const int N = T.N, P_ = T.P, dn = (l + P_ - 1) / P_;
    const int n = blockIdx.x * blockDim.x + threadIdx.x;
    const int j = blockIdx.y % dn, u = blockIdx.y / dn;
    if (n >= N || u >= U) return;
    const size_t idx = ((size_t)u * dn + j) * N + n;
    {
        const int s0 = j * P_, ns = min(s0 + P_, l) - s0;
        const u64* yb = acoef + ((size_t)u * l + s0) * N + n;
        int v;
        if (ns == 1) {
            const u64 y0 = yb[0];
            v = T.ks_seal ? 0 : (y0 > (PK(T, s0).q >> 1) ? 1 : 0);
            if (zflag && y0 == 0) atomicOr(zflag, 1u);
        } else {
            const u64* R = T.modup_R + (((size_t)l * T.dnum + j) * P_) * 2;
            constexpr int PMAX = 8;
            u64 y[PMAX];
#pragma unroll
            for (int k = 0; k < PMAX; ++k) y[k] = k < ns ? yb[(size_t)k * N] : 0;
            u64 lo = 0;
            int carry = 0;
#pragma unroll
            for (int k = 0; k < PMAX; ++k) {
                if (k < ns) {
                    const u64 F = y[k] * R[2 * k + 1] + __umul64hi(y[k], R[2 * k]);
                    lo += F;
                    carry += lo < F;
                }
            }
            const u64 half = 1ULL << 63;
            const u64 d = lo >= half ? lo - half : half - lo;
            if (d > 64) {
                v = carry + (lo >= half ? 1 : 0);
            } else {
                u64 ys[PMAX], qs[PMAX];
                for (int k = 0; k < ns; ++k) {
                    ys[k] = yb[(size_t)k * N];
                    qs[k] = PK(T, s0 + k).q;
                }
                v = centered_exact(ys, qs, ns, carry);
            }
        }
        vout[idx] = (unsigned char)v;
    }
}
__global__ void k_centered_x(DevTables T, u64* acoef, int l, int U) {
    const int N = T.N, dn = l / 3;
    const int n = blockIdx.x * blockDim.x + threadIdx.x;
    const int j = blockIdx.y % dn, u = blockIdx.y / dn;
    if (n >= N || u >= U) return;
    u64* yb = acoef + ((size_t)u * l + 3 * j) * N + n;
    const u64 y[3] = {yb[0], yb[N], yb[2 * (size_t)N]};
    u64 w[3];
    centered_x_pack(y, T.modup_xd + (size_t)j * 32, w);
    yb[0] = w[0];
    yb[N] = w[1];
    yb[2 * (size_t)N] = w[2];
}

static void launch_centered(const DevTables& T, u64* acoef, unsigned char* vout, int l, int U, hipStream_t st,
                            unsigned* zflag = nullptr) {
    const int dn = (l + T.P - 1) / T.P;
    if (modup_xform(T, l))
        FHS_LAUNCH(k_centered_x, dim3((T.N + 255) / 256, U * dn), dim3(256), 0, st, T, acoef, l, U);
    else
        FHS_LAUNCH(k_centered, dim3((T.N + 255) / 256, U * dn), dim3(256), 0, st, T, acoef, vout, l, U, zflag);
}

template <int LOGN>
__global__ void __launch_bounds__((1 << LOGN) / 16) k_modup(DevTables T, const u64* const* uniq, const u64* acoef,
                                                            const unsigned char* vcnt, u64* ext, int l, int U) {
    constexpr int N = 1 << LOGN;
    __shared__ __attribute__((aligned(16))) u64 lds[ntt_lds_words<LOGN, false>()];
    const int P_ = T.P, K = T.K, E = l + P_, dn = (l + P_ - 1) / P_;
    int t, mi;
    if (!xcd_tinner(E, dn * U, t, mi)) return;
    const int j = mi % dn, u = mi / dn;
    const int s0 = j * P_, s1 = min(s0 + P_, l), ns = s1 - s0;
    u64* o = ext + (((size_t)u * dn + j) * E + t) * N;
    if (t >= s0 && t < s1) return;
    const int pt = t < l ? t : T.L0 + (t - l);
    const PrimeK& PM = PK(T, pt);
    const u64 m = PM.q;
    const u64* yb = acoef + ((size_t)u * l + s0) * N;
    const u64* hat = T.modup_hat + (((size_t)l * T.dnum + j) * P_) * K + pt;
    const u64* qv = T.modup_Q + (((size_t)l * T.dnum + j) * K + pt) * 2;
    const u64 Qm = qv[0], nsQm = qv[1];
    const unsigned char* vb = vcnt + ((size_t)u * dn + j) * N;
    const RedU R = redu(PM);
    fwd_limb<LOGN, FHS_NTT_RL, false>(
        lds, threadIdx.x, T.tw_fwd + (size_t)pt * N * 2, R,
        [&](int e) {
            Acc3 a3 = {0, 0, 0};
            for (int w = 0; w < ns; ++w)
                acc3_mac(a3, split30(yb[(size_t)w * N + e]), split30(hat[(size_t)w * K]));
            u128 acc = {0, 0};
            acc3_fold(acc, a3);
            mac128(acc, (u64)(ns - vb[e]), Qm);
            return submod(reduce128(acc.lo, acc.hi, R), nsQm, m);
        },
        [&](int e, u64 v) { o[e] = v; });
}

template <int LOGN, bool B59>
__device__ __forceinline__ void modup_convert3x(const u64* yb, const u64* xt, const RedU& R, const u64* tw, int tid,
                                                u64* lds, u64 hi[16]) {
    constexpr int N = 1 << LOGN, NH = N / 2, TH = N / 32;
    const __amdgpu_buffer_rsrc_t ry = brsrc(yb, 3 * N * 8);
    const uint32_t e1 = (uint32_t)xt[0];
    const Split30 e2 = unpack30(xt[1]);
    const u64 c3 = xt[2], m = R.q;
    const int vo = tid * 8;
    const Tw4 w4 = ld_tw4(tw);
#pragma unroll
    for (int ch = 0; ch < 8; ++ch) {
        u64 V[3][4];
#pragma unroll
        for (int k = 0; k < 4; ++k) {
            const int e = (ch + 8 * (k & 1)) * TH + (k >= 2 ? NH : 0);
#pragma unroll
            for (int w = 0; w < 3; ++w) V[w][k] = bload64(ry, vo, (w * N + e) * 8);
        }
        u64 x[4];
#pragma unroll
        for (int k = 0; k < 4; ++k)
            x[k] = B59 ? convert3x_b59(V[0][k], V[1][k], V[2][k], e1, e2, c3, R.d, k < 2)
                       : convert3x_value(V[0][k], V[1][k], V[2][k], e1, e2, c3, R.b, R.d);
        fwd_quad_first2<TH>(x, w4, m, lazy_of<LOGN, B59>(R), lds, tid, ch, hi);
    }
}

template <int LOGN>
__device__ __forceinline__ void modup_convert1(const u64* yb, const unsigned char* vb, u64 negQ, u64 m, u64 w0,
                                               u64 w0p, int tid, u64* lds, u64 hi[16]) {
    constexpr int N = 1 << LOGN, NH = N / 2, TH = N / 32;
    const __amdgpu_buffer_rsrc_t ry = brsrc(yb, N * 8), rv = brsrc(vb, N);
    const u64 q2 = 2 * m;
#pragma unroll
    for (int ch = 0; ch < 4; ++ch) {
        u64 x[8];
#pragma unroll
        for (int k = 0; k < 8; ++k) {
            const int e = (ch * 4 + (k & 3)) * TH + (k >= 4 ? NH : 0);
            const u64 y = bload64(ry, tid * 8, e * 8);
            const uint32_t v = __builtin_amdgcn_raw_buffer_load_b8(rv, tid, e, 0);
            x[k] = y + (v ? negQ : 0);
        }
#pragma unroll
        for (int k = 0; k < 4; ++k) {
            const u64 tt = shoup_lazy(x[4 + k], w0, w0p, m);
            lds[row_pad<TH>(tid, ch * 4 + k)] = x[k] + tt;
            hi[ch * 4 + k] = x[k] + (q2 - tt);
        }
    }
}

template <int LOGN>
__device__ __forceinline__ void modup_convert1_r4(const u64* yb, const unsigned char* vb, u64 negQ, u64 m,
                                                  bool lazy, const u64* tw, int tid, u64* lds, u64 hi[16]) {
// ... 61 lines not shown
            const Split30 hw = split30(hat[(size_t)w * K]);
            const u64* yw = yb + (size_t)w * N + tid;
            u64 y[2 * CH];
#pragma unroll
            for (int k = 0; k < CH; ++k) {
                y[k] = yw[(ch * CH + k) * TH];
                y[CH + k] = yw[(ch * CH + k) * TH + NH];
            }
#pragma unroll
            for (int k = 0; k < 2 * CH; ++k) acc3_mac(a3[k], split30(y[k]), hw);
        }
        u64 x[2 * CH];
        if (R.cpm) {
#pragma unroll
            for (int k = 0; k < 2 * CH; ++k) {
                const uint32_t v = vv[k];
                const u64 vq = mul32w(v, (uint32_t)negQ) + ((u64)(v * (uint32_t)(negQ >> 32)) << 32);
                x[k] = acc3_reduce_pm(a3[k].L + vq, a3[k].M, a3[k].H, R.b, R.d);
            }
        } else {
#pragma unroll
            for (int k = 0; k < 2 * CH; ++k) {
                u128 acc = {0, 0};
                acc3_fold(acc, a3[k]);
                mac128(acc, (u64)(ns - vv[k]), Qm);
                x[k] = submod(reduce128(acc.lo, acc.hi, R), nsQm, m);
            }
        }
#pragma unroll
        for (int k = 0; k < CH; ++k) {
            [[maybe_unused]] const int e = tid + (ch * CH + k) * TH;
            const u64 tt = shoup_lazy(x[CH + k], w0, w0p, m);
            lds[row_pad<TH>(tid, ch * CH + k)] = x[k] + tt;
            hi[ch * CH + k] = x[k] + (q2 - tt);
        }
    }
    }
#pragma unroll 1
    for (int h = 0; h < 2; ++h) {
        if (h) {
            __syncthreads();
#pragma unroll
            for (int c = 0; c < 16; ++c) lds[row_pad<TH>(tid, c)] = hi[c];
        }
        __syncthreads();
        constexpr int S0 = (DP == 3 || (DP == 1 && B59)) ? 1 : 0;
        constexpr bool WLX = FHS_NTT_WAVELOCAL && fwd_exit_wave_local<LOGN - 1, FHS_MODUPH_RL, S0>();
        ntt_fwd_lds<LOGN - 1, FHS_MODUPH_RL, 16, S0, WLX>(lds, tid, tw, m, lazy_of<LOGN, B59>(R), 1 + h);
        const __amdgpu_buffer_rsrc_t ro = brsrc(o, N * 8);
        if constexpr (WLX) {
            constexpr int GS = 1 << FHS_MODUPH_RL;
            const int wb = wl_base<LOGN - 1, 16, GS>(tid), wp = lds_pad(wb);
            if (lazy_of<LOGN, B59>(R)) {
#pragma unroll
                for (int c = 0; c < 16; ++c) {
                    const int off = wl_off<LOGN - 1, 16, GS>(c);
                    bstore64_aux<FHS_MODUP_STORE_AUX>(pm_fold_lt60(lds[wp + off + off / 16], R), ro, wb * 8,
                                                      (h * NH + off) * 8);
                }
            } else {
#pragma unroll
                for (int c = 0; c < 16; ++c) {
                    const int off = wl_off<LOGN - 1, 16, GS>(c);
                    bstore64_aux<FHS_MODUP_STORE_AUX>(fwd_canon(lds[wp + off + off / 16], R), ro, wb * 8,
                                                      (h * NH + off) * 8);
                }
            }
        } else if (lazy_of<LOGN, B59>(R)) {
#pragma unroll
            for (int c = 0; c < 16; ++c)
                bstore64_aux<FHS_MODUP_STORE_AUX>(pm_fold_lt60(lds[row_pad<TH>(tid, c)], R), ro, tid * 8,
                                                  (h * NH + c * TH) * 8);
        } else {
#pragma unroll
            for (int c = 0; c < 16; ++c)
                bstore64_aux<FHS_MODUP_STORE_AUX>(fwd_canon(lds[row_pad<TH>(tid, c)], R), ro, tid * 8,
                                                  (h * NH + c * TH) * 8);
        }
    }
}
template <int LOGN, int DP, bool B59>
__global__ void __launch_bounds__((1 << LOGN) / 32, 4) k_modup_h(DevTables T, const u64* const* uniq,
                                                                 const u64* acoef, const unsigned char* vcnt, u64* ext,
                                                                 int l, int U) {
    __shared__ __attribute__((aligned(16))) u64 lds[modup_h_lds_words<LOGN>()];
    const int E = l + T.P, dn = (l + T.P - 1) / T.P;
    int t, mi;
    if (!xcd_quadpair(E, dn * U, t, mi)) return;
    modup_h_body<LOGN, DP, B59>(T, acoef, vcnt, ext, l, t, mi, threadIdx.x, lds);
}

template <int LOGN>
static void launch_modup(const DevTables& T, const u64* const* uniq, const u64* acoef, const unsigned char* vcnt,
                         u64* ext, int l, int U, hipStream_t st) {
    const int E = l + T.P, M = (l + T.P - 1) / T.P * U;
    void (*k)(DevTables, const u64* const*, const u64*, const unsigned char*, u64*, int, int);
    dim3 g(xcd_grid_q(E, M)), b((1 << LOGN) / 32);
    if constexpr (!ks_uses_half(LOGN)) {
        k = k_modup<LOGN>;
        g = dim3(xcd_grid(E, M));
        b = dim3((1 << LOGN) / 16);
    } else if (modup_xform(T, l)) {
        k = T.conv_b59 ? k_modup_h<LOGN, 3, true> : k_modup_h<LOGN, 3, false>;
    } else if (T.modup_dp == 1) {
        k = T.all_b59 ? k_modup_h<LOGN, 1, true> : k_modup_h<LOGN, 1, false>;
    } else {
        k = k_modup_h<LOGN, 0, false>;
    }
    FHS_LAUNCH(k, g, b, 0, st, T, uniq, acoef, vcnt, ext, l, U);
}

struct KsOps {
    __amdgpu_buffer_rsrc_t ext, own, key, akey;
    int sn8, n8;
    int per_r8, kn8;
    int jown;
};
__device__ __forceinline__ KsOps ks_ops(const DevTables& T, const KsItem& it, const u64* const* uniq, const u64* ext,
                                        int t, int pt, int l, int n, int sn) {
    const int N = T.N, P_ = T.P, E = l + P_, dn = (l + P_ - 1) / P_, K = T.K;
    KsOps o;
    o.ext = brsrc(ext + ((size_t)it.src * dn * E + t) * N, (uint32_t)((size_t)dn * E * N * 8));
    o.own = brsrc(uniq[it.src] + (size_t)t * N, (uint32_t)N * 8);
    o.key = brsrc(it.key + (size_t)pt * N, (uint32_t)((size_t)T.dnum * K * N * 8));
    o.akey = brsrc(it.akey ? it.akey + (size_t)pt * N : it.key, (uint32_t)((size_t)T.dnum * K * N * 8));
    o.sn8 = sn * 8;
    o.n8 = n * 8;
    o.per_r8 = E * N * 8;
    o.kn8 = K * N * 8;
    o.jown = t < l ? t / P_ : -1;
    return o;
}
constexpr int kBufNT = 2;
typedef const __attribute__((address_space(4))) u64* cu64p;
template <bool EXPLICIT_A>
__device__ __forceinline__ void ks_digit(const KsOps& o, u64 x, int j, u64 seed, u64 cx, const RedU& RD, unsigned qb,
                                         Acc3& a0, Acc3& a1) {
    const Split30 v = split30(x);
    acc3_mac(a0, v, split30(__builtin_bit_cast(u64, __builtin_amdgcn_raw_buffer_load_b64(o.key, o.n8, j * o.kn8,
                                                                                         kBufNT))));
    if constexpr (EXPLICIT_A)
        acc3_mac(a1, v, split30(__builtin_bit_cast(u64, __builtin_amdgcn_raw_buffer_load_b64(o.akey, o.n8, j * o.kn8,
                                                                                             kBufNT))));
    else
        acc3_mac(a1, v, split30(seeded_uniform_x(seed + cx, RD.q, qb)));
}
template <bool EXPLICIT_A>
__device__ __forceinline__ void ks_digits(const KsOps& o, const u64* seeds_g, u64 cx, const RedU& RD, unsigned qb,
                                          int dn, u128& c0, u128& c1) {
    const cu64p seeds = (cu64p)seeds_g;
    Acc3 a0 = {0, 0, 0}, a1 = {0, 0, 0};
#pragma unroll FHS_KSIP_UNROLL
    for (int j = 0; j < dn; ++j) {
        const bool own = j == o.jown;
        const u64 x = own ? bload64(o.own, o.sn8, 0) : bload64(o.ext, o.sn8, j * o.per_r8);
        ks_digit<EXPLICIT_A>(o, x, j, seeds[j], cx, RD, qb, a0, a1);
        if ((j & 7) == 7) {
            acc3_fold(c0, a0);
            acc3_fold(c1, a1);
        }
    }
    acc3_fold(c0, a0);
    acc3_fold(c1, a1);
}
__global__ void __launch_bounds__(256) k_ks_ip(DevTables T, const KsItem* items, const u64* const* uniq, const u64* ext,
                                                u64* acc, int l, int R, int t0) {
    const int N = T.N, P_ = T.P, K = T.K, E = l + P_, dn = (l + P_ - 1) / P_;
    const int NB = N >> 8;
    int t, m;
    if (!(t0 > 0 ? plain_tm(E - t0, R * NB, t, m) : xcd_touter(E - t0, R * NB, t, m))) return;
    t += t0;
    int r, nb;
    if (FHS_KSIP_HALVES && t0 == 0 && NB >= 2 && (size_t)dn * N * 8 > ((size_t)3 << 20)) {
        const int hb = NB >> 1, h = m / (R * hb), k = m % (R * hb);
        r = k / hb;
        nb = h * hb + k % hb;
    } else {
        r = m / NB;
        nb = m % NB;
    }
    const int n = (nb << 8) + threadIdx.x;
    const int pt = t < l ? t : T.L0 + (t - l);
    const RedU RD = redu(PK(T, pt));
    const KsItem it = items[r];
    const int sn = galois_src(n, it.elt, T.logN);
    const KsOps o = ks_ops(T, it, uniq, ext, t, pt, l, n, sn);
    const u64* seeds = it.key + (size_t)T.dnum * K * N;
    const u64 cx = seeded_ctr_mix(pt, n);
    const unsigned qb = 64 - __clzll(RD.q);
    u128 c0 = {0, 0}, c1 = {0, 0};
    if (it.akey)
        ks_digits<true>(o, seeds, cx, RD, qb, dn, c0, c1);
    else
        ks_digits<false>(o, seeds, cx, RD, qb, dn, c0, c1);
    u64 v0 = reduce128(c0.lo, c0.hi, RD), v1 = reduce128(c1.lo, c1.hi, RD);
    if (it.corr) {
        v0 = addmod(v0, it.corr[(size_t)t * N + n], RD.q);
        v1 = addmod(v1, it.corr[((size_t)E + t) * N + n], RD.q);
    }
    acc[(((size_t)r * 2 + 0) * E + t) * N + n] = v0;
    acc[(((size_t)r * 2 + 1) * E + t) * N + n] = v1;
}

__global__ void __launch_bounds__(256) k_ks_ip_sum(DevTables T, const KsItem* items, const u64* const* uniq,
                                                    const u64* ext, u64* acc, int l, int R) {
    const int N = T.N, P_ = T.P, K = T.K, E = l + P_, dn = (l + P_ - 1) / P_;
    const int NB = N >> 8;
    int t, m;
    if (!xcd_touter(l, NB, t, m)) return;
    const int n = (m << 8) + threadIdx.x;
    const RedU RD = redu(PK(T, t));
    const u64 q = RD.q;
    const u64 cx = seeded_ctr_mix(t, n);
    const unsigned qb = 64 - __clzll(q);
    u64 s0 = 0, s1 = 0, sadd = 0;
    for (int r = 0; r < R; ++r) {
        const KsItem it = items[r];
        const int sn = galois_src(n, it.elt, T.logN);
        const KsOps o = ks_ops(T, it, uniq, ext, t, t, l, n, sn);
        const u64* seeds = it.key + (size_t)T.dnum * K * N;
        u128 c0 = {0, 0}, c1 = {0, 0};
        if (it.akey)
            ks_digits<true>(o, seeds, cx, RD, qb, dn, c0, c1);
        else
            ks_digits<false>(o, seeds, cx, RD, qb, dn, c0, c1);
        s0 = addmod(s0, reduce128(c0.lo, c0.hi, RD), q);
        s1 = addmod(s1, reduce128(c1.lo, c1.hi, RD), q);
        if (it.corr) {
            s0 = addmod(s0, it.corr[(size_t)t * N + n], q);
            s1 = addmod(s1, it.corr[((size_t)E + t) * N + n], q);
        }
        sadd = addmod(sadd, bload64(brsrc(it.add0 + (size_t)t * N, (uint32_t)N * 8), o.sn8, 0), q);
    }
    const u64 pinv = T.md_pinv[2 * t], pinv_s = T.md_pinv[2 * t + 1];
    acc[((size_t)0 * E + t) * N + n] = addmod(shoup(s0, pinv, pinv_s, q), sadd, q);
    acc[((size_t)1 * E + t) * N + n] = shoup(s1, pinv, pinv_s, q);
}

template <int LOGN, bool H = ntt_half<LOGN>()>
__global__ void __launch_bounds__((ntt_threads<LOGN, H>())) k_ks_special_intt(DevTables T, const u64* acc, u64* ycoef, int l,
                                                                         int R) {
    constexpr int N = 1 << LOGN;
    __shared__ __attribute__((aligned(16))) u64 lds[ntt_lds_words<LOGN, H>()];
    const int k = blockIdx.x, comp = blockIdx.y, r = blockIdx.z;
    const int P_ = T.P, E = l + P_, pi = T.L0 + k;
    const PrimeK& P = PK(T, pi);
    const u64* src = acc + (((size_t)r * 2 + comp) * E + l + k) * N;
    u64* dst = ycoef + (((size_t)r * 2 + comp) * P_ + k) * N;
    const u64* cst = T.md_intt + (size_t)k * 4;
    const u64 p = P.q, half = T.ks_seal ? p >> 1 : 0;
    inv_limb<LOGN, FHS_NTT_RL, H>(lds, threadIdx.x, T.tw_inv + (size_t)pi * N * 2, P.q, cst[0], cst[1], cst[2], cst[3],
                               [&](int e) { return src[e]; }, [&](int e, u64 v) { dst[e] = csub(csub(v, p) + half, p); });
}

__global__ void k_special_x(DevTables T, u64* ycoef, int R2) {
    const int N = T.N, n = blockIdx.x * blockDim.x + threadIdx.x, rc = blockIdx.y;
    if (n >= N || rc >= R2) return;
    u64* yb = ycoef + (size_t)rc * 3 * N + n;
    const u64 y[3] = {yb[0], yb[N], yb[2 * (size_t)N]};
    u64 w[3];
    centered_x_pack(y, T.md_xd, w);
    yb[0] = w[0];
    yb[N] = w[1];
    yb[2 * (size_t)N] = w[2];
}

template <int LOGN>
__global__ void __launch_bounds__((1 << LOGN) / 16) k_moddown(DevTables T, const KsItem* items, const u64* acc,
                                                              const u64* ycoef, int l, int R) {
    constexpr int N = 1 << LOGN;
    __shared__ __attribute__((aligned(16))) u64 lds[ntt_lds_words<LOGN, false>()];
    const int P_ = T.P, E = l + P_;
    int i, m;
    if (!plain_tm(l, 2 * R, i, m)) return;
    const int comp = m & 1, r = m >> 1;
    const PrimeK& P = PK(T, i);
    const u64 q = P.q;
    const KsItem it = items[r];
    const u64* y = ycoef + ((size_t)r * 2 + comp) * P_ * N;
    const u64 halfq = T.ks_seal ? T.md_pinv[3 * T.L0 + i] : 0;
    const u64 pinv = T.md_pinv[2 * i], pinv_s = T.md_pinv[2 * i + 1];
    const u64* add = comp == 0 ? it.add0 : it.add1;
    const u64 aelt = comp == 0 ? it.elt : 1;
    u64* o = (comp == 0 ? it.out0 : it.out1) + (size_t)i * N;
    const u64* ac = acc + (((size_t)r * 2 + comp) * E + i) * N;
    fwd_limb<LOGN, FHS_NTT_RL, false>(
        lds, threadIdx.x, T.tw_fwd + (size_t)i * N * 2, redu(P),
        [&](int e) {
            u128 s = {0, 0};
            for (int k = 0; k < P_; ++k) mac128(s, y[(size_t)k * N + e], T.md_hat[(size_t)k * T.L0 + i]);
            return submod(reduce128(s.lo, s.hi, P), halfq, q);
        },
        [&](int e, u64 v) {
            u64 res = shoup(submod(ac[e], v, q), pinv, pinv_s, q);
            if (add) res = addmod(res, add[(size_t)i * N + galois_src(e, aelt, LOGN)], q);
            o[e] = res;
        });
}

template <int LOGN>
__device__ __forceinline__ void moddown_convert3(const u64* y, const u64* hat, int L0, const RedU& R, const u64* tw,
                                                 int tid, u64* lds, u64 hi[16]) {
    constexpr int N = 1 << LOGN, NH = N / 2, TH = N / 32;
    const __amdgpu_buffer_rsrc_t ry = brsrc(y, 3 * N * 8);
    const Split30 h0 = split30(hat[0]), h1 = split30(hat[L0]), h2 = split30(hat[2 * L0]);
    const u64 m = R.q;
    const int vo = tid * 8;
    const Tw4 w4 = ld_tw4(tw);
#pragma unroll
    for (int ch = 0; ch < 8; ++ch) {
        u64 v[3][4];
#pragma unroll
        for (int k = 0; k < 4; ++k) {
            const int e = (ch + 8 * (k & 1)) * TH + (k >= 2 ? NH : 0);
#pragma unroll
            for (int w = 0; w < 3; ++w) v[w][k] = bload64(ry, vo, (w * N + e) * 8);
        }
        u64 x[4];
#pragma unroll
        for (int k = 0; k < 4; ++k) {
            Acc3 a = {0, 0, 0};
            acc3_mac(a, split30(v[0][k]), h0);
            acc3_mac(a, split30(v[1][k]), h1);
            acc3_mac(a, split30(v[2][k]), h2);
            x[k] = acc3_reduce_pm(a.L, a.M, a.H, R.b, R.d);
        }
        fwd_quad_first2<TH>(x, w4, m, R.lazy, lds, tid, ch, hi);
    }
}

template <int LOGN, bool B59>
__device__ __forceinline__ void moddown_convert3x(const u64* y, const u64* xt, const RedU& R, const u64* tw, int tid,
                                                  u64* lds, u64 hi[16]) {
    constexpr int N = 1 << LOGN, NH = N / 2, TH = N / 32;
    const __amdgpu_buffer_rsrc_t ry = brsrc(y, 3 * N * 8);
    const uint32_t e1 = (uint32_t)xt[0];
    const Split30 e2 = unpack30(xt[1]);
    const int vo = tid * 8;
    const Tw4 w4 = ld_tw4(tw);
#pragma unroll
    for (int ch = 0; ch < 8; ++ch) {
        u64 v[3][4];
#pragma unroll
        for (int k = 0; k < 4; ++k) {
            const int e = (ch + 8 * (k & 1)) * TH + (k >= 2 ? NH : 0);
#pragma unroll
            for (int w = 0; w < 3; ++w) v[w][k] = bload64(ry, vo, (w * N + e) * 8);
        }
        u64 x[4];
#pragma unroll
        for (int k = 0; k < 4; ++k)
            x[k] = B59 ? convert3x_b59(v[0][k], v[1][k], v[2][k], e1, e2, 0, R.d, k < 2)
                       : convert3x_value(v[0][k], v[1][k], v[2][k], e1, e2, 0, R.b, R.d);
        fwd_quad_first2<TH>(x, w4, R.q, lazy_of<LOGN, B59>(R), lds, tid, ch, hi);
    }
}

// ... 147 lines not shown
        KsItem& it = items[r];
        if (it.elt != 1) {
            u64* pc = perm + (size_t)r * 2 * S;
            it.a = pc + S;
            if (it.add0) it.add0 = pc;
            it.elt = 1;
        }
        it.corr = nullptr;
        uniq[r] = it.a;
        it.src = (u64)r;
    }
}
constexpr int kPermBatch = 32;
struct PermBatch {
    const u64* in[kPermBatch];
    u64* out[kPermBatch];
    u64 elt[kPermBatch];
};
__global__ void __launch_bounds__(256) k_galois_perm_batch(DevTables T, PermBatch pb, int limbs) {
    const int y = blockIdx.y;
    const u64* in = pb.in[y];
    u64* out = pb.out[y];
    const u64 elt = pb.elt[y];
    const size_t S = (size_t)limbs * T.N;
    for (size_t idx = blockIdx.x * (size_t)blockDim.x + threadIdx.x; idx < S; idx += (size_t)gridDim.x * blockDim.x) {
        const size_t base = idx - idx % T.N;
        out[idx] = in[base + galois_src((int)(idx % T.N), elt, T.logN)];
    }
}
static hipError_t seal_permute(const DevTables& T, const KsItem* orig, int R, int l, u64* perm, hipStream_t st) {
    const size_t S = (size_t)l * T.N;
    PermBatch pb;
    int n = 0;
    const int gx = std::max(1, eltwise_grid(S) / 8);
    auto flush = [&]() -> hipError_t {
        if (!n) return hipSuccess;
        FHS_LAUNCH(k_galois_perm_batch, dim3(gx, n), dim3(256), 0, st, T, pb, l);
        n = 0;
        return hipGetLastError();
    };
    for (int r = 0; r < R; ++r) {
        const KsItem& it = orig[r];
        if (it.elt == 1) continue;
        u64* pc = perm + (size_t)r * 2 * S;
        for (int c = 1; c >= 0; --c) {
            const u64* src = c ? it.a : it.add0;
            if (!src) continue;
            pb.in[n] = src;
            pb.out[n] = pc + (c ? S : 0);
            pb.elt[n] = it.elt;
            if (++n == kPermBatch) {
                hipError_t e = flush();
                if (e != hipSuccess) return e;
            }
        }
    }
    return flush();
}

template <int LOGN>
static void ks_intt_stage(const DevTables& T, const u64* const* uniq, int U, int l, const KsBufs& b, hipStream_t st,
                          const KTimer* tm, unsigned* zflag = nullptr) {
    FHS_TMARK(tm, KID_KS_INTT, 1, st);
    bool half = false;
    if constexpr (ks_uses_half(LOGN)) {
        half = LOGN > 14 || l * U >= FHS_FULL_FORM_MAX_WG;
        if (half)
            FHS_LAUNCH((k_ks_intt_h<LOGN>), dim3(l * U), dim3((1 << LOGN) / 32), 0, st, T, uniq, b.acoef, l, U);
    }
    if constexpr (LOGN <= 14) {
        if (!half)
            FHS_LAUNCH((k_ks_intt<LOGN>), dim3(l * U), dim3((1 << LOGN) / 16), 0, st, T, uniq, b.acoef, l, U);
    }
    launch_centered(T, b.acoef, b.vcnt, l, U, st, zflag);
    FHS_TMARK(tm, KID_KS_INTT, 0, st);
}
template <int LOGN>
static void ks_modup_stage(const DevTables& T, const u64* const* uniq, int U, int l, const KsBufs& b, hipStream_t st,
                           const KTimer* tm) {
    FHS_TMARK(tm, KID_MODUP, 1, st);
    launch_modup<LOGN>(T, uniq, b.acoef, b.vcnt, b.ext, l, U, st);
    FHS_TMARK(tm, KID_MODUP, 0, st);
}
static void ks_ip_stage(const DevTables& T, const KsItem* it, const u64* const* uniq, int R, int l, const KsBufs& b,
                        hipStream_t st, const KTimer* tm) {
    FHS_TMARK(tm, KID_KS_IP, 1, st);
    FHS_LAUNCH(k_ks_ip, dim3(xcd_grid(l + T.P, R * (T.N >> 8))), dim3(256), 0, st, T, it, uniq, b.ext, b.acc, l, R,
               0);
    FHS_TMARK(tm, KID_KS_IP, 0, st);
}
static void giant_ip_stage(const DevTables& T, const KsItem* it, const u64* const* uniq, int R, int l, const KsBufs& b,
                           hipStream_t st, const KTimer* tm) {
    const int NB = T.N >> 8;
    FHS_TMARK(tm, KID_KS_IP, 1, st);
    FHS_LAUNCH(k_ks_ip, dim3(T.P * R * NB), dim3(256), 0, st, T, it, uniq, b.ext, b.acc, l, R, l);
    FHS_LAUNCH(k_ks_ip_sum, dim3(xcd_grid(l, NB)), dim3(256), 0, st, T, it, uniq, b.ext, b.acc, l, R);
    FHS_TMARK(tm, KID_KS_IP, 0, st);
}
template <int LOGN>
static void ks_special_intt_stage(const DevTables& T, int R, int l, const KsBufs& b, hipStream_t st, const KTimer* tm) {
    FHS_TMARK(tm, KID_SPECIAL_INTT, 1, st);
    FHS_NTT_LAUNCH(k_ks_special_intt, T.P * 2 * R, dim3(T.P, 2, R), st, T, b.acc, b.ycoef, l, R);
    FHS_TMARK(tm, KID_SPECIAL_INTT, 0, st);
}
template <int LOGN>
static hipError_t ks_moddown_stage(const DevTables& T, const KsItem* it, int R, int l, const KsBufs& b, hipStream_t st,
                                   const KTimer* tm) {
    FHS_TMARK(tm, KID_MODDOWN, 1, st);
    void (*k)(DevTables, const KsItem*, const u64*, const u64*, int, int);
    int nwg = l * 2 * R, threads = (1 << LOGN) / 32;
    const bool xform = ks_uses_half(LOGN) && T.md_xform;
    if constexpr (!ks_uses_half(LOGN)) {
        k = k_moddown<LOGN>;
        threads = (1 << LOGN) / 16;
    } else if (xform && T.conv_b59 && LOGN == 15 && nwg < FHS_SPLIT_MAX_WG) {
        k = k_moddown_h<LOGN, true, true, true>;
        nwg *= 2;
    } else if (xform) {
        k = T.conv_b59 ? k_moddown_h<LOGN, true, true> : k_moddown_h<LOGN, true>;
    } else {
        k = T.all_b59 ? k_moddown_h<LOGN, false, true> : k_moddown_h<LOGN, false>;
    }
    if (xform)
        FHS_LAUNCH(k_special_x, dim3((T.N + 255) / 256, 2 * R), dim3(256), 0, st, T, b.ycoef, 2 * R);
    FHS_LAUNCH(k, dim3(nwg), dim3(threads), 0, st, T, it, b.acc, b.ycoef, l, R);
    FHS_TMARK(tm, KID_MODDOWN, 0, st);
    return hipGetLastError();
}

static hipError_t upload_items(const KsItem* items, int R, const u64* const* uniq, int U, void* dev, const Stager& sg,
                               const KsItem** it_dev, const u64* const** uniq_dev) {
    static thread_local std::vector<unsigned char> buf;
    buf.resize(sizeof(KsItem) * R + sizeof(u64*) * U);
    memcpy(buf.data(), items, sizeof(KsItem) * R);
    memcpy(buf.data() + sizeof(KsItem) * R, uniq, sizeof(u64*) * U);
    hipError_t e = sg.h2d(sg.user, dev, buf.data(), buf.size());
    *it_dev = reinterpret_cast<const KsItem*>(dev);
    *uniq_dev = reinterpret_cast<const u64* const*>(static_cast<unsigned char*>(dev) + sizeof(KsItem) * R);
    return e;
}

__global__ void k_seal_mask(DevTables T, u64 elt, u64* out) {
    const int N = T.N, i = blockIdx.x * blockDim.x + threadIdx.x;
    if (i >= N) return;
    const u64 j = ((u64)i * elt) & (2 * (u64)N - 1);
    const u64 v = j >> T.logN;
    const size_t k = j & (N - 1);
    for (int t = 0; t < T.K; ++t) out[(size_t)t * N + k] = v;
}
__global__ void __launch_bounds__(256) k_seal_corr(DevTables T, const u64* key, const u64* akey, const u64* M,
                                                    int l, u64* out) {
    const int N = T.N, K = T.K, E = l + T.P;
    const int n = blockIdx.x * blockDim.x + threadIdx.x, t = blockIdx.y;
    if (n >= N || t >= E) return;
    const int pt = t < l ? t : T.L0 + (t - l);
    const RedU RD = redu(PK(T, pt));
    const u64 p = RD.q;
    const unsigned qb = 64 - __clzll(p);
    const u64* seeds = key + (size_t)T.dnum * K * N;
    const u64 cx = seeded_ctr_mix(pt, n);
    u128 s0 = {0, 0}, s1 = {0, 0};
    for (int j = 0; j < l; ++j) {
        if (j == t) continue;
        const u64 qj = reduce128(PK(T, j).q, 0, RD);
        const size_t kx = ((size_t)j * K + pt) * N + n;
        const u64 a = akey ? akey[kx] : seeded_uniform_x(seeds[j] + cx, p, qb);
        mac128(s0, key[kx], qj);
        mac128(s1, a, qj);
        if ((j & 7) == 7) {
            s0 = u128{reduce128(s0.lo, s0.hi, RD), 0};
            s1 = u128{reduce128(s1.lo, s1.hi, RD), 0};
        }
    }
    const u64 m = M[(size_t)pt * N + n];
    const u64 r0 = reduce128(s0.lo, s0.hi, RD), r1 = reduce128(s1.lo, s1.hi, RD);
    out[(size_t)t * N + n] = reduce128(r0 * m, __umul64hi(r0, m), RD);
    out[((size_t)E + t) * N + n] = reduce128(r1 * m, __umul64hi(r1, m), RD);
}
hipError_t launch_seal_corr(const DevTables& T, const u64* key, const u64* akey, u64 elt, int l, u64* mask_scratch,
                            u64* out, hipStream_t st) {
    if (T.P != 1 || l < 1 || l > T.L0 || !key || !out || !mask_scratch) return hipErrorInvalidValue;
    FHS_LAUNCH(k_seal_mask, dim3((T.N + 255) / 256), dim3(256), 0, st, T, elt, mask_scratch);
    hipError_t e = launch_ntt_fwd(T, mask_scratch, T.K, T.L0, 1, 0, st);
    if (e != hipSuccess) return e;
    FHS_LAUNCH(k_seal_corr, dim3((T.N + 255) / 256, l + T.P), dim3(256), 0, st, T, key, akey, mask_scratch,
               l, out);
    return hipGetLastError();
}

hipError_t launch_keyswitch(const DevTables& T, const KsItem* items_host, int R, const u64* const* uniq_host, int U,
                            int l, u64* ws, size_t ws_bytes, void* items_dev, const Stager& sg, hipStream_t st,
                            const KTimer* tm, SealHoist* sh) {
    if (keyswitch_workspace_bytes(T, R, U, l) > ws_bytes) return hipErrorInvalidValue;
    const KsItem* it;
    const u64* const* uq;
    std::vector<KsItem> sitems;
    std::vector<const u64*> suniq;
    bool hoist = T.ks_seal && sh && U < R;
    for (int r = 0; hoist && r < R; ++r) hoist = items_host[r].elt == 1 || items_host[r].corr;
    if (hoist) {
        hipError_t e = upload_items(items_host, R, uniq_host, U, items_dev, sg, &it, &uq);
        if (e == hipSuccess) e = hipMemsetAsync(sh->zflag_dev, 0, sizeof(unsigned), st);
        if (e != hipSuccess) return e;
        const KsBufs b = ks_carve(T, ws, R, U, l);
        FHS_DISPATCH_LOGN(T.logN, ks_intt_stage<LOGN>(T, uq, U, l, b, st, tm, sh->zflag_dev));
        e = hipMemcpyAsync(sh->zflag_host, sh->zflag_dev, sizeof(unsigned), hipMemcpyDeviceToHost, st);
        if (e == hipSuccess) e = hipStreamSynchronize(st);
        if (e != hipSuccess) return e;
        if (*(volatile unsigned*)sh->zflag_host) {
            ++sh->fallback;
            return launch_keyswitch(T, items_host, R, uniq_host, U, l, ws, ws_bytes, items_dev, sg, st, tm, nullptr);
        }
        ++sh->hoisted;
        FHS_DISPATCH_LOGN(T.logN, {
            ks_modup_stage<LOGN>(T, uq, U, l, b, st, tm);
            ks_ip_stage(T, it, uq, R, l, b, st, tm);
            ks_special_intt_stage<LOGN>(T, R, l, b, st, tm);
            e = ks_moddown_stage<LOGN>(T, it, R, l, b, st, tm);
        });
        if (e != hipSuccess) return e;
        return hipGetLastError();
    }
    if (T.ks_seal) {
        sitems.assign(items_host, items_host + R);
        suniq.resize(R);
        u64* perm = ws + ks_core_bytes(T, R, R, l) / 8;
        seal_rewrite(T, sitems.data(), R, suniq.data(), l, perm);
        hipError_t pe = seal_permute(T, items_host, R, l, perm, st);
        if (pe != hipSuccess) return pe;
        items_host = sitems.data();
        uniq_host = suniq.data();
        U = R;
    }
    hipError_t e = upload_items(items_host, R, uniq_host, U, items_dev, sg, &it, &uq);
    if (e != hipSuccess) return e;
    hipError_t me = hipSuccess;
    const KsBufs b = ks_carve(T, ws, R, U, l);
    FHS_DISPATCH_LOGN(T.logN, {
        ks_intt_stage<LOGN>(T, uq, U, l, b, st, tm);
        ks_modup_stage<LOGN>(T, uq, U, l, b, st, tm);
        ks_ip_stage(T, it, uq, R, l, b, st, tm);
        ks_special_intt_stage<LOGN>(T, R, l, b, st, tm);
        me = ks_moddown_stage<LOGN>(T, it, R, l, b, st, tm);
    });
    if (me != hipSuccess) return me;
    return hipGetLastError();
}

template <int VEC, int TL = 0>
__device__ __forceinline__ void ld_diag(const u64* limb, int voff, int soff, u64* out) {
    const __amdgpu_buffer_rsrc_t r = brsrc(limb, 0x7ffffff0);
    if constexpr (TL > 0) {
        static_assert(VEC == 2, "compact diagonals: two coefficients per lane");
        out[0] = out[1] = __builtin_bit_cast(u64, __builtin_amdgcn_raw_buffer_load_b64(r, voff, soff, kBufNT));
    } else if constexpr (VEC == 2) {
        const auto t = __builtin_amdgcn_raw_buffer_load_b128(r, voff, soff, kBufNT);
        out[0] = ((u64)t[1] << 32) | t[0];
        out[1] = ((u64)t[3] << 32) | t[2];
    } else {
        out[0] = __builtin_bit_cast(u64, __builtin_amdgcn_raw_buffer_load_b64(r, voff, soff, kBufNT));
    }
}
template <int VEC, int WAVES, int FOLD, bool ACC, int TL = 0>
__global__ void __launch_bounds__(64 * WAVES) k_bsgs_inner(DevTables T, const u64* const* __restrict__ baby,
                                                    const u64* const* __restrict__ pts, int G, int Gw, int g0, int g1,
                                                    int D, int l, u64* __restrict__ inner) {
    extern __shared__ __attribute__((aligned(16))) u64 sb[];
    constexpr int W = 64 * VEC;
    const int N = T.N;
    const int i = blockIdx.y, n0 = blockIdx.x * W, tid = threadIdx.x, lane = tid & 63;
    const int wave = __builtin_amdgcn_readfirstlane(tid >> 6);
    const size_t S = (size_t)l * N;
    const size_t off = (size_t)i * N + n0 + lane * VEC;
    const size_t dlimb = (size_t)i * (N >> TL);
    const int dvoff = ((lane * VEC) >> TL) * 8, dsoff = (n0 >> TL) * 8;
    u64 p[8][VEC];
    const int gcur = g0 + wave;
    auto full_batches = [&](int g) { return g < g1 ? max(0, min(Gw, D - g * G)) / 8 : 0; };
    int gf = gcur;
    while (gf < g1 && full_batches(gf) == 0) gf += WAVES;
    if (gf < g1) {
        const u64* const* pg0 = pts + (size_t)gf * G;
#pragma unroll
        for (int u = 0; u < 8; ++u) ld_diag<VEC, TL>(pg0[u] + dlimb, dvoff, dsoff, p[u]);
    }
    for (int idx = tid; idx < Gw * 2 * W; idx += 64 * WAVES) {
        const int b = idx / (2 * W), comp = (idx / W) & 1, c = idx % W;
        sb[idx] = pack30(baby[b][comp * S + (size_t)i * N + n0 + c]);
    }
    __syncthreads();
    const RedU R = redu(PK(T, i));
    for (int g = gcur; g < g1; g += WAVES) {
        const int bmax = min(Gw, D - g * G);
        if (bmax <= 0) continue;
        u128 c0[VEC], c1[VEC];
        Acc3 a0[VEC], a1[VEC];
#pragma unroll
        for (int v = 0; v < VEC; ++v) {
            c0[v] = c1[v] = u128{0, 0};
            a0[v] = a1[v] = Acc3{0, 0, 0};
        }
        const u64* const* pg = pts + (size_t)g * G;
        const int nb = bmax / 8;
        int gn = g + WAVES;
        while (gn < g1 && full_batches(gn) == 0) gn += WAVES;
        int b = 0;
        for (int bi = 0; bi < nb; ++bi, b += 8) {
            constexpr bool ROLL = FOLD == 16;
            if (!ROLL && bi > 0) {
#pragma unroll
                for (int u = 0; u < 8; ++u) ld_diag<VEC, TL>(pg[b + u] + dlimb, dvoff, dsoff, p[u]);
            }
            const u64* const* nxt = ROLL && bi + 1 < nb ? pg + b + 8 : nullptr;
#pragma unroll
            for (int h = 0; h < 8; h += 4) {
#pragma unroll
                for (int u = h; u < h + 4; ++u)
#pragma unroll
                    for (int v = 0; v < VEC; ++v) {
                        const Split30 y = split30(p[u][v]);
                        acc3_mac(a0[v], unpack30(sb[((b + u) * 2 + 0) * W + lane * VEC + v]), y);
                        acc3_mac(a1[v], unpack30(sb[((b + u) * 2 + 1) * W + lane * VEC + v]), y);
                    }
                if (h == 4 && (FOLD == 8 || (b & 15) == 8)) {
#pragma unroll
                    for (int v = 0; v < VEC; ++v) {
                        acc3_fold(c0[v], a0[v]);
                        acc3_fold(c1[v], a1[v]);
                    }
                }
                if (nxt) {
#pragma unroll
                    for (int u = h; u < h + 4; ++u) ld_diag<VEC, TL>(nxt[u] + dlimb, dvoff, dsoff, p[u]);
                }
            }
        }
        for (; b < bmax; ++b) {
            u64 q1[VEC];
            ld_diag<VEC, TL>(pg[b] + dlimb, dvoff, dsoff, q1);
#pragma unroll
            for (int v = 0; v < VEC; ++v) {
                const Split30 y = split30(q1[v]);
                acc3_mac(a0[v], unpack30(sb[(b * 2 + 0) * W + lane * VEC + v]), y);
                acc3_mac(a1[v], unpack30(sb[(b * 2 + 1) * W + lane * VEC + v]), y);
            }
        }
#pragma unroll
        for (int v = 0; v < VEC; ++v) {
            acc3_fold(c0[v], a0[v]);
            acc3_fold(c1[v], a1[v]);
        }
#pragma unroll
        for (int v = 0; v < VEC; ++v) {
            u64* o0 = inner + (size_t)g * 2 * S + off + v;
            u64 r0 = reduce128(c0[v].lo, c0[v].hi, R), r1 = reduce128(c1[v].lo, c1[v].hi, R);
            if constexpr (ACC) {
                r0 = addmod(r0, o0[0], R.q);
                r1 = addmod(r1, o0[S], R.q);
            }
            o0[0] = r0;
            o0[S] = r1;
        }
        if (gn < g1) {
            const u64* const* pgn = pts + (size_t)gn * G;
#pragma unroll
            for (int u = 0; u < 8; ++u) ld_diag<VEC, TL>(pgn[u] + dlimb, dvoff, dsoff, p[u]);
        }
    }
}

#ifndef FHS_GSUM_ICH
#define FHS_GSUM_ICH 4
#endif
__global__ void __launch_bounds__(256) k_giant_sum(DevTables T, const u64* bpart, const u64* ycoef, const u64* inner0,
                                                   u64* base, u64* convsum, int l, int R) {
    const int N = T.N, P_ = T.P, E = l + P_;
    const int n = blockIdx.x * blockDim.x + threadIdx.x, comp = blockIdx.y;
    if (n >= N) return;
    const int i0 = blockIdx.z * FHS_GSUM_ICH, i1 = min(i0 + FHS_GSUM_ICH, l);
    const size_t S = (size_t)l * N;
    constexpr int PMAX = 8;
    u64 ylo[PMAX], yhi[PMAX];
#pragma unroll
    for (int k = 0; k < PMAX; ++k) ylo[k] = yhi[k] = 0;
    for (int r = 0; r < R; ++r) {
        const u64* y = ycoef + ((size_t)r * 2 + comp) * P_ * N + n;
#pragma unroll
        for (int k = 0; k < PMAX; ++k) {
            if (k < P_) {
                const u64 v = y[(size_t)k * N];
                ylo[k] += v;
                yhi[k] += ylo[k] < v;
            }
        }
    }
    for (int i = i0; i < i1; ++i) {
        const PrimeK& P = PK(T, i);
        const u64 q = P.q;
        u128 cs = {0, 0};
#pragma unroll
        for (int k = 0; k < PMAX; ++k)
            if (k < P_) mac128(cs, reduce128(ylo[k], yhi[k], P), T.md_hat[(size_t)k * T.L0 + i]);
        if (T.ks_seal) {
            u128 h = {0, 0};
            mac128(h, (u64)R, T.md_pinv[3 * T.L0 + i]);
            const u64 rh = reduce128(h.lo, h.hi, P);
            cs.lo = reduce128(cs.lo, cs.hi, P);
            cs.hi = 0;
            cs.lo = submod(cs.lo, rh, q);
        }
        u64 cv = reduce128(cs.lo, cs.hi, P);
        const size_t idx = (size_t)comp * S + (size_t)i * N + n;
        const u64 bv = addmod(bpart[((size_t)comp * E + i) * N + n], inner0[idx], q);
        convsum[idx] = cv;
        base[idx] = bv;
    }
}
template <int LOGN, bool H = ntt_half<LOGN>()>
__global__ void __launch_bounds__((ntt_threads<LOGN, H>())) k_giant_final(DevTables T, const u64* base, const u64* convsum,
                                                                     u64* out, int l) {
    constexpr int N = 1 << LOGN;
    __shared__ __attribute__((aligned(16))) u64 lds[ntt_lds_words<LOGN, H>()];
    const int i = blockIdx.x, comp = blockIdx.y;
    const PrimeK& P = PK(T, i);
    const RedU RU = redu(P);
    const size_t off = ((size_t)comp * l + i) * N;
    const u64 pinv = T.md_pinv[2 * i], pinv_s = T.md_pinv[2 * i + 1], q = RU.q;
    fwd_limb<LOGN, FHS_NTT_RL, H>(lds, threadIdx.x, T.tw_fwd + (size_t)i * N * 2, RU,
                               [&](int e) { return convsum[off + e]; },
                               [&](int e, u64 v) { out[off + e] = submod(base[off + e], shoup(v, pinv, pinv_s, q), q); });
}

size_t bsgs_workspace_bytes(const DevTables& T, int R, int l) {
    return keyswitch_workspace_bytes(T, R, R, l) + 8 * (size_t)T.N * 4 * l;
}

template <class Each>
static hipError_t lds_opt_in(std::atomic<bool>& done, size_t bytes, Each each) {
    if (done.load(std::memory_order_acquire)) return hipSuccess;
    hipError_t e = hipSuccess;
    each([&](const void* k) {
        if (k && e == hipSuccess) e = hipFuncSetAttribute(k, hipFuncAttributeMaxDynamicSharedMemorySize, (int)bytes);
    });
    if (e == hipSuccess) done.store(true, std::memory_order_release);
    return e;
}

constexpr int kInnerWindow = 64;
typedef void (*InnerFn)(DevTables, const u64* const*, const u64* const*, int, int, int, int, int, int, u64*);
template <int VEC, int WAVES, int FOLD, int TL>
static InnerFn inner_kernel_acc(bool acc) {
    return acc ? k_bsgs_inner<VEC, WAVES, FOLD, true, TL> : k_bsgs_inner<VEC, WAVES, FOLD, false, TL>;
}
template <int VEC, int WAVES>
static InnerFn inner_kernel(bool fold16, bool acc, int ptl) {
    if (!fold16) return ptl == 0 ? inner_kernel_acc<VEC, WAVES, 8, 0>(acc) : nullptr;
    switch (ptl) {
        case 0: return inner_kernel_acc<VEC, WAVES, 16, 0>(acc);
        case 1: return inner_kernel_acc<VEC, WAVES, 16, 1>(acc);
        case 2: return inner_kernel_acc<VEC, WAVES, 16, 2>(acc);
        case 3: return inner_kernel_acc<VEC, WAVES, 16, 3>(acc);
    }
    return nullptr;
}
template <int VEC, int WAVES>
static hipError_t launch_inner_t(const DevTables& T, const u64* const* baby, const u64* const* pts, int G, int g0,
                                 int g1, int D, int l, u64* inner, hipStream_t st, int ptl) {
    constexpr int W = 64 * VEC;
    static std::atomic<bool> opted{false};
    hipError_t e = lds_opt_in(opted, (size_t)kInnerWindow * 2 * W * 8, [](auto f) {
        for (int fold16 = 0; fold16 < 2; ++fold16)
            for (int acc = 0; acc < 2; ++acc)
                for (int tl = 0; tl <= 3; ++tl)
                    f(reinterpret_cast<const void*>(inner_kernel<VEC, WAVES>(fold16, acc, tl)));
    });
    if (e != hipSuccess) return e;
    if (ptl < 0 || ptl > 3 || (ptl > 0 && (T.max_qbits > 59 || VEC != 2))) return hipErrorInvalidValue;
    for (int b0 = 0; b0 < G; b0 += kInnerWindow) {
        const int Gw = std::min(kInnerWindow, G - b0), Dw = D - b0;
        const size_t lds = (size_t)Gw * 2 * W * 8;
        const dim3 grid(T.N / W, l), block(64 * WAVES);
        const InnerFn k = inner_kernel<VEC, WAVES>(T.max_qbits <= 59, b0 > 0, ptl);
        FHS_LAUNCH(k, grid, block, lds, st, T, baby + b0, pts + b0, G, Gw, g0, g1, Dw, l, inner);
        e = hipGetLastError();
        if (e != hipSuccess) return e;
    }
    return hipSuccess;
}

hipError_t launch_bsgs_inner(const DevTables& T, const u64* const* baby_dev, const u64* const* pts_dev, int G, int g0,
                             int g1, int D, int l, u64* inner, hipStream_t st, int ptl) {
    if (T.N % 128 || G < 1) return hipErrorInvalidValue;
    return launch_inner_t<FHS_INNER_VEC, FHS_INNER_WAVES>(T, baby_dev, pts_dev, G, g0, g1, D, l, inner, st, ptl);
}

#define FHS_DOT_WAVES 8
#define FHS_DOT_VEC 2
constexpr int kDotBatch = 4;
template <int VEC, int WAVES, int FOLD, bool ACC>
__global__ void __launch_bounds__(64 * WAVES) k_dot_tensor(DevTables T, const u64* const* __restrict__ q,
                                                          const u64* const* __restrict__ db, int J, int Jw, int C, int l,
                                                          u64* __restrict__ out) {
    extern __shared__ __attribute__((aligned(16))) u64 sb[];
    constexpr int W = 64 * VEC;
    const int N = T.N;
    const int i = blockIdx.y, n0 = blockIdx.x * W, tid = threadIdx.x, lane = tid & 63;
    const int wave = __builtin_amdgcn_readfirstlane(tid >> 6);
    const size_t S = (size_t)l * N;
    const size_t limb = (size_t)i * N;
    const int dvoff = lane * VEC * 8, dsoff = n0 * 8;
    u64 p[kDotBatch][2][VEC];
    auto load_term = [&](const u64* ct, u64 (*dst)[VEC]) {
        ld_diag<VEC>(ct + limb, dvoff, dsoff, dst[0]);
// ... 17 lines not shown
        for (int v = 0; v < VEC; ++v) dot3_clear(s[v]);
        const u64* const* dc = db + (size_t)c * J;
        int j = 0;
        for (int bi = 0; bi < nb; ++bi, j += kDotBatch) {
            const u64* const* nxt = bi + 1 < nb ? dc + j + kDotBatch : nullptr;
#pragma unroll
            for (int u = 0; u < kDotBatch; ++u) {
#pragma unroll
                for (int v = 0; v < VEC; ++v)
                    dot3_term<FOLD>(s[v], j + u, unpack30(sb[((j + u) * 2 + 0) * W + lane * VEC + v]),
                                    unpack30(sb[((j + u) * 2 + 1) * W + lane * VEC + v]), split30(p[u][0][v]),
                                    split30(p[u][1][v]));
                if (nxt) load_term(nxt[u], p[u]);
            }
        }
        for (; j < Jw; ++j) {
            u64 t[2][VEC];
            load_term(dc[j], t);
#pragma unroll
            for (int v = 0; v < VEC; ++v)
                dot3_term<FOLD>(s[v], j, unpack30(sb[(j * 2 + 0) * W + lane * VEC + v]),
                                unpack30(sb[(j * 2 + 1) * W + lane * VEC + v]), split30(t[0][v]), split30(t[1][v]));
        }
        u64* o = out + (size_t)c * 3 * S + limb + n0 + lane * VEC;
#pragma unroll
        for (int v = 0; v < VEC; ++v) {
            u64 prev[3], r[3];
            if constexpr (ACC) {
                prev[0] = o[v];
                prev[1] = o[S + v];
                prev[2] = o[2 * S + v];
            }
            dot3_finish(s[v], R, ACC ? prev : nullptr, r);
            o[v] = r[0];
            o[S + v] = r[1];
            o[2 * S + v] = r[2];
        }
        if (c + WAVES < C && nb > 0) {
            const u64* const* dn = db + (size_t)(c + WAVES) * J;
#pragma unroll
            for (int u = 0; u < kDotBatch; ++u) load_term(dn[u], p[u]);
        }
    }
}
typedef void (*DotFn)(DevTables, const u64* const*, const u64* const*, int, int, int, int, u64*);
template <int VEC, int WAVES>
static DotFn dot_kernel(bool fold16, bool acc) {
    if (fold16) return acc ? k_dot_tensor<VEC, WAVES, 16, true> : k_dot_tensor<VEC, WAVES, 16, false>;
    return acc ? k_dot_tensor<VEC, WAVES, 8, true> : k_dot_tensor<VEC, WAVES, 8, false>;
}
template <int VEC, int WAVES>
static hipError_t launch_dot_t(const DevTables& T, const u64* const* q, const u64* const* db, int J, int C, int l, u64* out,
                               hipStream_t st) {
    constexpr int W = 64 * VEC;
    static std::atomic<bool> opted{false};
    hipError_t e = lds_opt_in(opted, (size_t)kDotWindowMax * 2 * W * 8, [](auto f) {
        for (int fold16 = 0; fold16 < 2; ++fold16)
            for (int acc = 0; acc < 2; ++acc) f(reinterpret_cast<const void*>(dot_kernel<VEC, WAVES>(fold16, acc)));
    });
    if (e != hipSuccess) return e;
    for (int j0 = 0; j0 < J; j0 += kDotWindowMax) {
        const int Jw = std::min(kDotWindowMax, J - j0);
        const size_t lds = (size_t)Jw * 2 * W * 8;
        const dim3 grid(T.N / W, l), block(64 * WAVES);
        const DotFn k = dot_kernel<VEC, WAVES>(T.max_qbits <= 59, j0 > 0);
        FHS_LAUNCH(k, grid, block, lds, st, T, q + j0, db + j0, J, Jw, C, l, out);
        e = hipGetLastError();
        if (e != hipSuccess) return e;
    }
    return hipSuccess;
}
hipError_t launch_dot_tensor(const DevTables& T, const u64* const* q_dev, const u64* const* db_dev, int J, int C, int l,
                             u64* out3, hipStream_t st, const KTimer* tm) {
    if (T.N % (64 * FHS_DOT_VEC) || J < 1 || C < 1) return hipErrorInvalidValue;
    FHS_TMARK(tm, KID_DOT_TENSOR, 1, st);
    const hipError_t e = launch_dot_t<FHS_DOT_VEC, FHS_DOT_WAVES>(T, q_dev, db_dev, J, C, l, out3, st);
    FHS_TMARK(tm, KID_DOT_TENSOR, 0, st);
    return e;
}

hipError_t launch_bsgs(const DevTables& T, const u64* const* baby_dev, const u64* const* pts_dev, int G, int B, int D,
                       int l, const u64* const* keys_host, const u64* const* akeys_host, const u64* giant_elts, u64* inner,
                       u64* out, u64* ws, size_t ws_bytes, void* items_dev, const Stager& sg, hipStream_t st,
                       const KTimer* tm, int ptl) {
    const int R = B - 1;
    const size_t N = T.N, S = (size_t)l * N;
    if (T.N % 128 || G < 1 || R > 512) return hipErrorInvalidValue;
    if (R > 0 && bsgs_workspace_bytes(T, R, l) > ws_bytes) return hipErrorInvalidValue;
    KsItem items[512];
    const u64* uniq[512];
    for (int r = 0; r < R; ++r) {
        const int g = r + 1;
        const u64* ct = inner + (size_t)g * 2 * S;
        u64 elt = 1;
        if (giant_elts) elt = giant_elts[g];
        else
            for (int s2 = 0; s2 < g * G; ++s2) elt = (elt * 5) & (2 * N - 1);
        items[r] = KsItem{ct + S, ct, nullptr, keys_host[g], nullptr, nullptr, elt, (u64)r,
                          akeys_host ? akeys_host[g] : nullptr};
        uniq[r] = ct + S;
    }
    std::vector<KsItem> seal_orig;
    u64* seal_perm = ws + ks_core_bytes(T, R, R, l) / 8;
    if (T.ks_seal && R > 0) {
        seal_orig.assign(items, items + R);
        seal_rewrite(T, items, R, uniq, l, seal_perm);
    }
    const KsItem* it = nullptr;
    const u64* const* uq = nullptr;
    if (R > 0) {
        hipError_t e = upload_items(items, R, uniq, R, items_dev, sg, &it, &uq);
        if (e != hipSuccess) return e;
    }
    hipError_t he = hipSuccess;
    if (pts_dev) {
        FHS_TMARK(tm, KID_BSGS_INNER, 1, st);
        he = launch_inner_t<FHS_INNER_VEC, FHS_INNER_WAVES>(T, baby_dev, pts_dev, G, 0, B, D, l, inner, st, ptl);
        FHS_TMARK(tm, KID_BSGS_INNER, 0, st);
        if (he != hipSuccess) return he;
    }
    if (R <= 0) return hipMemcpyAsync(out, inner, 8 * 2 * S, hipMemcpyDeviceToDevice, st);
    if (!seal_orig.empty()) {
        he = seal_permute(T, seal_orig.data(), R, l, seal_perm, st);
        if (he != hipSuccess) return he;
    }
    u64* base = ws + keyswitch_workspace_bytes(T, R, R, l) / 8;
    u64* convsum = base + 2 * S;
    FHS_DISPATCH_LOGN(T.logN, {
        const KsBufs b = ks_carve(T, ws, R, R, l);
        ks_intt_stage<LOGN>(T, uq, R, l, b, st, tm);
        ks_modup_stage<LOGN>(T, uq, R, l, b, st, tm);
        giant_ip_stage(T, it, uq, R, l, b, st, tm);
        ks_special_intt_stage<LOGN>(T, R, l, b, st, tm);
        FHS_TMARK(tm, KID_GIANT_SUM, 1, st);
        FHS_LAUNCH(k_giant_sum, dim3((T.N + 255) / 256, 2, (l + FHS_GSUM_ICH - 1) / FHS_GSUM_ICH), dim3(256), 0,
                   st, T, b.acc, b.ycoef, inner, base, convsum, l, R);
        FHS_TMARK(tm, KID_GIANT_SUM, 0, st);
        FHS_TMARK(tm, KID_GIANT_FINAL, 1, st);
        FHS_NTT_LAUNCH(k_giant_final, l * 2, dim3(l, 2), st, T, base, convsum, out, l);
        FHS_TMARK(tm, KID_GIANT_FINAL, 0, st);
    });
    return hipGetLastError();
}



__device__ __forceinline__ u64 rnd_testdata(u64 key, u64 ctr) { return sm64(key ^ sm64(ctr ^ 0xD1B54A32D192ED03ULL)); }

__global__ void k_sample(DevTables T, int mode, PrfKey K, u64 sid, u64* out, int l, u64 sid_step, u64* const* outs) {
    const int N = T.N;
    const size_t S = (size_t)l * N;
    sid += blockIdx.y * sid_step;
    out = outs ? outs[blockIdx.y] : out + blockIdx.y * S;
    for (size_t idx = blockIdx.x * (size_t)blockDim.x + threadIdx.x; idx < S; idx += (size_t)gridDim.x * blockDim.x) {
        const int i = (int)(idx / N), n = (int)(idx % N);
        const PrimeK& P = PK(T, i);
        u64 v;
        if (mode == SAMPLE_UNIFORM) {
            u64 hi, lo;
            prf128(K, sid, (uint32_t)idx, hi, lo);
            v = reduce128(lo, hi, P);
        } else if (mode == SAMPLE_SEEDED) {
            v = seeded_uniform_x(sid + seeded_ctr_mix(i, n), P.q, 64 - __clzll(P.q));
        } else if (mode == SAMPLE_TESTDATA) {
            const u64 ctr = 2 * ((u64)i * N + n);
            v = reduce128(rnd_testdata(sid, ctr + 1), rnd_testdata(sid, ctr), P);
        } else {
            u64 r, unused;
            prf128(K, sid, (uint32_t)n, r, unused);
            long long s;
            if (mode == SAMPLE_TERNARY) {
                const u64 t = r % 3;
                s = t == 2 ? -1 : (long long)t;
            } else {
                s = (long long)__popcll(r & 0x1FFFFFULL) - (long long)__popcll((r >> 21) & 0x1FFFFFULL);
            }
            v = s >= 0 ? (u64)s : P.q - (u64)(-s);
        }
        out[idx] = v;
    }
}
hipError_t launch_sample(const DevTables& T, int mode, const PrfKey& K, u64 sid, u64* out, int l, hipStream_t st,
                         int npoly, u64 sid_step, u64* const* outs_dev) {
    if (npoly < 1) return hipSuccess;
    const int g1 = eltwise_grid((size_t)l * T.N) / npoly, gx = g1 > 0 ? g1 : 1;
    FHS_LAUNCH(k_sample, dim3(gx, npoly), dim3(256), 0, st, T, mode, K, sid, out, l, sid_step, outs_dev);
    return hipGetLastError();
}

__global__ void k_swk(DevTables T, u64* b_out, const u64* a, const u64* e, const u64* s, const u64* snew, int j) {
    const int N = T.N, K = T.K;
    const size_t S = (size_t)K * N;
    for (size_t idx = blockIdx.x * (size_t)blockDim.x + threadIdx.x; idx < S; idx += (size_t)gridDim.x * blockDim.x) {
        const int i = (int)(idx / N);
        const PrimeK& P = PK(T, i);
        u64 v = submod(e[idx], mulmod(a[idx], s[idx], P), P.q);
        if (i < T.L0 && i / T.P == j) {
            const u64 pm = T.md_pinv[2 * T.L0 + i];
            v = addmod(v, mulmod(pm, snew[idx], P), P.q);
        }
        b_out[idx] = v;
    }
}
hipError_t launch_switch_key_assemble(const DevTables& T, u64* b_out, const u64* a, const u64* e_ntt, const u64* s_ntt,
                                      const u64* snew_ntt, int digit, hipStream_t st) {
    FHS_LAUNCH(k_swk, dim3(eltwise_grid((size_t)T.K * T.N)), dim3(256), 0, st, T, b_out, a, e_ntt, s_ntt,
               snew_ntt, digit);
    return hipGetLastError();
}

struct EncBatch {
    size_t ct, ue;
    const u64* const* pts;
};
__global__ void k_encrypt(DevTables T, int mode, u64* c0, u64* c1, const u64* s_or_pk0, const u64* pk1, const u64* u,
                          const u64* e0, const u64* e1, const u64* pt, int l, EncBatch B) {
    const int N = T.N;
    const size_t S = (size_t)l * N;
    if (const size_t y = blockIdx.y) {
        c0 += y * B.ct;
        c1 += y * B.ct;
        u += y * B.ue;
        e0 += y * B.ue;
        e1 += y * B.ue;
// ... 825 lines not shown
```

### fhe-spear_amd/python/pyPhantom/__init__.py

```python
from __future__ import annotations

import ctypes as C
import enum
import os
import sys
import threading
from pathlib import Path

import numpy as np

__version__ = "fhespear-mi355x-0.1"

_HERE = Path(__file__).resolve().parent
_LIB_CANDIDATES = [
    os.environ.get("FHESPEAR_LIB", ""),
    str(_HERE.parent.parent / "lib" / "libfhespear_hip.so"),
]


def _share_torch_hip_runtime():
    if os.environ.get("FHESPEAR_HIP_RUNTIME", "torch") != "torch":
        return None
    import importlib.util
    try:
# ... 64 lines not shown
    "fhs_galois_keys_bytes": (C.c_int, [_vp, _u64p]),
    "fhs_ciphertext_destroy": (C.c_int, [_vp]),
    "fhs_plaintext_destroy": (C.c_int, [_vp]),
    "fhs_ciphertext_info": (C.c_int, [_vp, _ip, _ip, _ip, _dblp]),
    "fhs_ciphertext_set_scale": (C.c_int, [_vp, C.c_double]),
    "fhs_plaintext_info": (C.c_int, [_vp, _ip, _ip, _dblp]),
    "fhs_ciphertext_export": (C.c_int, [_vp, _vp, _u64p]),
    "fhs_ciphertext_import": (C.c_int, [_vp, _u64p, C.c_int, C.c_int, C.c_double, C.POINTER(_vp)]),
    "fhs_plaintext_export": (C.c_int, [_vp, _vp, _u64p]),
    "fhs_plaintext_import": (C.c_int, [_vp, _u64p, C.c_int, C.c_double, C.POINTER(_vp)]),
    "fhs_ciphertext_device_ptr": (C.c_int, [_vp, C.POINTER(_vp), _u64p]),
    "fhs_encode": (C.c_int, [_vp, _dblp, C.c_size_t, C.c_double, C.c_int, C.POINTER(_vp)]),
    "fhs_encode_batch": (C.c_int, [_vp, _dblp, C.c_size_t, C.c_size_t, C.c_double, C.c_int, C.POINTER(_vp)]),
    "fhs_encode_real": (C.c_int, [_vp, _dblp, C.c_size_t, C.c_double, C.c_int, C.POINTER(_vp)]),
    "fhs_encode_real_batch": (C.c_int, [_vp, _dblp, C.c_size_t, C.c_size_t, C.c_double, C.c_int, C.POINTER(_vp)]),
    "fhs_decode": (C.c_int, [_vp, _vp, _dblp]),
    "fhs_decode_batch": (C.c_int, [_vp, _vp, C.c_int, C.c_int, _dblp]),
    "fhs_encrypt_symmetric": (C.c_int, [_vp, _vp, _vp, C.POINTER(_vp)]),
    "fhs_encrypt_symmetric_batch": (C.c_int, [_vp, _vp, _vp, C.c_int, _vp]),
    "fhs_encode_encrypt_symmetric_batch": (C.c_int, [_vp, _vp, _dblp, C.c_size_t, C.c_size_t, C.c_int, C.c_double,
                                                     C.c_int, _vp]),
    "fhs_decrypt_decode_batch": (C.c_int, [_vp, _vp, _vp, C.c_int, C.c_int, _dblp]),
    "fhs_encrypt_asymmetric": (C.c_int, [_vp, _vp, _vp, C.POINTER(_vp)]),
    "fhs_encrypt_asymmetric_batch": (C.c_int, [_vp, _vp, _vp, C.c_int, _vp]),
    "fhs_encode_encrypt_asymmetric_batch": (C.c_int, [_vp, _vp, _dblp, C.c_size_t, C.c_size_t, C.c_int, C.c_double,
                                                      C.c_int, _vp]),
    "fhs_decrypt": (C.c_int, [_vp, _vp, _vp, C.POINTER(_vp)]),
    "fhs_add": (C.c_int, [_vp, _vp, _vp, C.POINTER(_vp)]),
    "fhs_sub": (C.c_int, [_vp, _vp, _vp, C.c_int, C.POINTER(_vp)]),
    "fhs_negate": (C.c_int, [_vp, _vp, C.POINTER(_vp)]),
    "fhs_add_plain": (C.c_int, [_vp, _vp, _vp, C.POINTER(_vp)]),
    "fhs_sub_plain": (C.c_int, [_vp, _vp, _vp, C.POINTER(_vp)]),
    "fhs_multiply_plain": (C.c_int, [_vp, _vp, _vp, C.POINTER(_vp)]),
    "fhs_multiply": (C.c_int, [_vp, _vp, _vp, C.POINTER(_vp)]),
    "fhs_relinearize": (C.c_int, [_vp, _vp, _vp, C.POINTER(_vp)]),
    "fhs_rescale_to_next": (C.c_int, [_vp, _vp, C.POINTER(_vp)]),
    "fhs_mod_switch_to_next": (C.c_int, [_vp, _vp, C.POINTER(_vp)]),
    "fhs_mod_switch_to": (C.c_int, [_vp, _vp, C.c_int, C.POINTER(_vp)]),
    "fhs_plain_mod_switch_to_next": (C.c_int, [_vp, _vp, C.POINTER(_vp)]),
    "fhs_plain_mod_switch_to": (C.c_int, [_vp, _vp, C.c_int, C.POINTER(_vp)]),
    "fhs_rotate": (C.c_int, [_vp, _vp, C.c_int, _vp, C.POINTER(_vp)]),
    "fhs_apply_galois": (C.c_int, [_vp, _vp, _u64, _vp, C.POINTER(_vp)]),
    "fhs_rotate_many": (C.c_int, [_vp, C.POINTER(_vp), _ip, C.c_int, _vp, C.POINTER(_vp)]),
    "fhs_bsgs_multiply_accumulate": (C.c_int, [_vp, C.POINTER(_vp), C.c_int, C.POINTER(_vp), C.c_int, C.c_int, _vp,
                                               C.POINTER(_vp)]),
    "fhs_offload_plaintexts": (C.c_int, [_vp, C.POINTER(_vp), C.c_int, _u64p]),
    "fhs_upload_plaintexts": (C.c_int, [_vp, _u64p, C.c_int, C.c_int, C.c_double, C.POINTER(_vp)]),
    "fhs_bsgs_from_cpu": (C.c_int, [_vp, C.POINTER(_vp), C.c_int, _u64p, C.c_int, C.c_int, C.c_int, C.c_double, _vp,
                                    C.POINTER(_vp)]),
    "fhs_bsgs_inner_products": (C.c_int, [_vp, C.POINTER(_vp), C.c_int, C.POINTER(_vp), C.c_int, C.POINTER(_vp)]),
    "fhs_dot_product_many": (C.c_int, [_vp, C.POINTER(_vp), C.c_int, C.POINTER(_vp), C.c_int, _vp, C.c_int,
                                       C.POINTER(_vp)]),
    "fhs_bsgs_giant_steps": (C.c_int, [_vp, C.POINTER(_vp), C.c_int, _u64p, _vp, C.POINTER(_vp)]),
    "fhs_bsgs_inner_products_device": (C.c_int, [_vp, C.POINTER(_vp), C.c_int, C.POINTER(_vp), C.c_int, _vp]),
    "fhs_bsgs_giant_steps_device": (C.c_int, [_vp, _vp, C.c_int, C.c_int, C.c_double, _u64p, _vp, C.POINTER(_vp)]),
    "fhs_linear_transform": (C.c_int, [_vp, C.POINTER(_vp), C.c_int, C.POINTER(_vp), C.c_int, C.c_int, _u64p, _vp,
                                       C.c_int, C.POINTER(_vp)]),
    "fhs_multiply_const": (C.c_int, [_vp, _vp, C.c_double, C.c_double, C.POINTER(_vp)]),
    "fhs_add_const": (C.c_int, [_vp, _vp, C.c_double, C.POINTER(_vp)]),
    "fhs_mod_raise": (C.c_int, [_vp, _vp, C.POINTER(_vp)]),
    "fhs_bootstrap_evalmod": (C.c_int, [_vp, _vp, _vp, _dblp, _dblp, C.c_int, C.c_int, C.c_int, C.POINTER(_vp)]),
    "fhs_encode_precise": (C.c_int, [_vp, _dblp, C.c_size_t, C.c_size_t, C.c_double, C.c_int, C.POINTER(_vp)]),
    "fhs_encode_diagonals": (C.c_int, [_vp, _dblp, _dblp, C.c_int, C.c_int, C.c_double, C.c_int, C.POINTER(_vp)]),
    "fhs_encode_diagonals_ex": (C.c_int, [_vp, _vp, _vp, C.c_int64, C.c_int, C.c_int, C.c_int, C.c_double, C.c_int,
                                          C.POINTER(_vp)]),
    "fhs_encode_diagonals_rows": (C.c_int, [_vp, _vp, _vp, C.c_int64, C.c_int, C.c_int, C.c_int, C.c_double, C.c_int,
                                            _vp, C.c_int, C.POINTER(_vp)]),
    "fhs_host_alloc": (C.c_int, [_u64, C.POINTER(_vp)]),
    "fhs_host_free": (C.c_int, [_vp]),
    "fhs_random_plaintexts": (C.c_int, [_vp, _u64, C.c_int, C.c_int, C.c_double, C.POINTER(_vp)]),
    "fhs_event_record": (C.c_int, [_vp, C.POINTER(_vp)]),
    "fhs_event_elapsed": (C.c_int, [_vp, _vp, C.POINTER(C.c_float)]),
    "fhs_event_destroy": (C.c_int, [_vp]),
    "fhs_kernel_timer": (C.c_int, [_vp, C.c_int, C.POINTER(C.c_float), _ip, C.c_int]),
    "fhs_kernel_timer_arm": (C.c_int, [_vp, C.c_uint32]),
    "fhs_ciphertext_copy_to_device": (C.c_int, [_vp, _vp, _vp]),
    "fhs_ciphertext_from_device": (C.c_int, [_vp, _vp, C.c_int, C.c_int, C.c_double, C.POINTER(_vp)]),
    "fhs_ciphertext_copy_to_device_async": (C.c_int, [_vp, _vp, _vp]),
    "fhs_ciphertext_from_device_async": (C.c_int, [_vp, _vp, C.c_int, C.c_int, C.c_double, C.POINTER(_vp)]),
    "fhs_context_stream": (C.c_int, [_vp, C.POINTER(_vp)]),
    "fhs_staging_stats": (C.c_int, [_vp, C.POINTER(C.c_uint64), C.POINTER(C.c_uint64)]),
    "fhs_debug_fail_next_flushes": (C.c_int, [_vp, C.c_int]),
    "fhs_debug_fail_alloc": (C.c_int, [_vp, C.c_int, _ip]),
    "fhs_debug_launch_ledger": (C.c_int, [C.c_int, C.c_char_p, _u64, _u64p]),
}
_OPTIONAL = {
    "fhs_bsgs_multiply_accumulate": ("bsgs_multiply_accumulate",),
    "fhs_bsgs_from_cpu": ("bsgs_from_cpu", "bsgs_complete_from_cpu"),
    "fhs_upload_plaintexts": ("upload_plaintexts",),
    "fhs_offload_plaintexts": ("offload_plaintexts",),
    "fhs_encode_real_batch": ("ckks_encoder.encode_double_vector_batch",),
    "fhs_encode_batch": ("ckks_encoder.encode_complex_vector_batch",),
}
_DISABLED = {x.strip() for x in os.environ.get("FHESPEAR_DISABLE_SYMBOLS", "").split(",") if x.strip()}
_MISSING = []
for _name, (_res, _args) in _SIGS.items():
    try:
        if _name in _DISABLED:
            raise AttributeError(_name)
        _f = getattr(_lib, _name)
    except AttributeError:
        if _name in _OPTIONAL:
            _MISSING.append(_name)
            continue
        raise ImportError(f"pyPhantom: {LIB_PATH} lacks the required symbol {_name}") from None
    _f.restype = _res
    _f.argtypes = _args

_OOM, _HIP, _NODEV = 2, 3, 7


def _check(rc: int, what: str = ""):
    if rc == 0:
        return
    msg = (_lib.fhs_last_error() or b"").decode(errors="replace")
    if rc in (_OOM, _HIP, _NODEV):
        raise RuntimeError(f"{what}: {msg}" if what else msg)
    raise ValueError(f"{what}: {msg}" if what else msg)


def _u64_arr(values):
    a = np.ascontiguousarray(np.asarray(values, dtype=np.uint64))
    return a, a.ctypes.data_as(_u64p)


class scheme_type(enum.IntEnum):
    none = 0
    bgv = 1
    bfv = 2
    ckks = 3


class mul_tech_type(enum.IntEnum):
    none = 0
    behz = 1
    hps = 2
    hps_overq = 3
    hps_overq_leveled = 4


class sec_level_type(enum.IntEnum):
    none = 0
    tc128 = 1
    tc192 = 2
    tc256 = 3


class modulus(int):

    def value(self):
        return int(self)


def create_coeff_modulus(poly_modulus_degree, bit_sizes):
    bits = [int(b) for b in bit_sizes]
    arr = (C.c_int * len(bits))(*bits)
    out = np.zeros(len(bits), dtype=np.uint64)
    _check(_lib.fhs_create_coeff_modulus(int(poly_modulus_degree), arr, len(bits), out.ctypes.data_as(_u64p)),
           "create_coeff_modulus")
    return [modulus(int(x)) for x in out]


def get_elt_from_step(step, poly_modulus_degree):
    return int(_lib.fhs_galois_elt_from_step(int(step), int(poly_modulus_degree)))


# ... 740 lines not shown
        _check_key_shape(keys[e], want, f"galois_keys_from_numpy: key for element {e}")
    arr = np.ascontiguousarray(np.stack([np.asarray(keys[e], dtype=np.uint64) for e in elts]))
    e_arr = np.array(elts, dtype=np.uint64)
    h = _vp()
    _check(_lib.fhs_galois_keys_import(ctx._h, e_arr.ctypes.data_as(_u64p), len(elts), arr.ctypes.data_as(_u64p),
                                       C.byref(h)), "galois_keys_from_numpy")
    return galois_key(ctx, h)


def _switch_key_shape(ctx):
    return (-(-ctx.L0 // ctx.P), 2, ctx.L0 + ctx.P, ctx.N)


def _check_key_shape(arr, want, what):
    shape = tuple(np.shape(arr))
    if shape != tuple(want):
        raise ValueError(f"{what}: shape {shape}, this context needs {tuple(want)}")


def relin_key_from_numpy(ctx, key):
    _check_key_shape(key, _switch_key_shape(ctx), "relin_key_from_numpy")
    a = np.ascontiguousarray(key, dtype=np.uint64)
    h = _vp()
    _check(_lib.fhs_relin_key_import(ctx._h, a.ctypes.data_as(_u64p), C.byref(h)), "relin_key_from_numpy")
    return relin_key(ctx, h)


def secret_key_from_numpy(ctx, s_ntt):
    _check_key_shape(s_ntt, (ctx.L0 + ctx.P, ctx.N), "secret_key_from_numpy")
    a = np.ascontiguousarray(s_ntt, dtype=np.uint64)
    sk = secret_key.__new__(secret_key)
    sk._ctx, sk.seed = ctx, None
    h = _vp()
    _check(_lib.fhs_secret_key_import(ctx._h, a.ctypes.data_as(_u64p), C.byref(h)), "secret_key_from_numpy")
    sk._h = h
    return sk


class Event:
    def __init__(self, ctx):
        h = _vp()
        _check(_lib.fhs_event_record(ctx._h, C.byref(h)), "event")
        self._h = h

    def elapsed_ms(self, later):
        v = C.c_float()
        _check(_lib.fhs_event_elapsed(self._h, later._h, C.byref(v)), "event elapsed")
        return float(v.value)

    def __del__(self):
        if getattr(self, "_h", None):
            _lib is not None and _lib.fhs_event_destroy(self._h)
            self._h = None


KERNEL_IDS = {"k_bsgs_inner": 0, "k_modup": 1, "k_ks_ip": 2, "k_moddown": 3, "k_ks_intt": 4,
              "k_ks_special_intt": 5, "k_giant_sum": 6, "k_giant_final": 7, "rescale": 8, "k_dot_tensor": 9,
              "encrypt_pk": 10}


def kernel_timer_arm(ctx, names=None):
    ids = KERNEL_IDS.values() if names is None else [KERNEL_IDS[n] for n in names]
    mask = 0
    for i in ids:
        mask |= 1 << i
    _check(_lib.fhs_kernel_timer_arm(ctx._h, mask), "kernel_timer_arm")


def kernel_timer_read(ctx, reset=False):
    out = {}
    for name, kid in KERNEL_IDS.items():
        ms, n = C.c_float(), C.c_int()
        _check(_lib.fhs_kernel_timer(ctx._h, kid, C.byref(ms), C.byref(n), 0), "kernel_timer")
        out[name] = (float(ms.value), int(n.value))
    if reset:
        _check(_lib.fhs_kernel_timer(ctx._h, -1, None, None, 1), "kernel_timer")
    return out


def debug_fail_next_flushes(ctx, count=1):
    _check(_lib.fhs_debug_fail_next_flushes(ctx._h, int(count)), "debug_fail_next_flushes")


def debug_fail_alloc(ctx, nth):
    was = C.c_int()
    _check(_lib.fhs_debug_fail_alloc(ctx._h, int(nth), C.byref(was)), "debug_fail_alloc")
    return bool(was.value)


def debug_launch_ledger(op="read"):
    ops = {"arm": 0, "disarm": 1, "read": 2}
    if op not in ops:
        raise ValueError(f"debug_launch_ledger: op must be one of {sorted(ops)}")
    if op != "read":
        _check(_lib.fhs_debug_launch_ledger(ops[op], None, 0, None), "debug_launch_ledger")
        return None
    need = _u64()
    _lib.fhs_debug_launch_ledger(2, None, 0, C.byref(need))
    while True:
        buf = C.create_string_buffer(int(need.value))
        if _lib.fhs_debug_launch_ledger(2, buf, len(buf), C.byref(need)) == 0:
            return buf.value.decode().splitlines()
        if int(need.value) <= len(buf):
            _check(1, "debug_launch_ledger")


def staging_stats(ctx):
    a, b = C.c_uint64(), C.c_uint64()
    _check(_lib.fhs_staging_stats(ctx._h, C.byref(a), C.byref(b)), "staging_stats")
    return int(a.value), int(b.value)


def ciphertext_copy_to_device(ctx, ct, dst_ptr, sync=True):
    fn = _lib.fhs_ciphertext_copy_to_device if sync else _lib.fhs_ciphertext_copy_to_device_async
    _check(fn(ctx._h, ct._h, _vp(int(dst_ptr))), "copy_to_device")


def ciphertext_from_device(ctx, src_ptr, ncomp, chain_index, scale, sync=True):
    fn = _lib.fhs_ciphertext_from_device if sync else _lib.fhs_ciphertext_from_device_async
    h = _vp()
    _check(fn(ctx._h, _vp(int(src_ptr)), int(ncomp), int(chain_index), float(scale), C.byref(h)), "from_device")
    return ciphertext(ctx, h)


def context_stream(ctx):
    h = _vp()
    _check(_lib.fhs_context_stream(ctx._h, C.byref(h)), "context_stream")
    return int(h.value or 0)


from . import bootstrap as _bootstrap


class ckks_bootstrapper(_bootstrap.Bootstrapper):
    """bg:72-74, 112-116, 149-154: CKKS bootstrapping (pyPhantom/bootstrap.py) on the GPU ops."""


ckks_bootstrapper._ph = sys.modules[__name__]


def device_count():
    return int(_lib.fhs_device_count())


def device_pci_bus_id(device):
    buf = C.create_string_buffer(64)
    _check(_lib.fhs_device_pci_bus_id(int(device), buf, 64), "device_pci_bus_id")
    return buf.value.decode()


_lock = threading.Lock()

for _name in _MISSING:
    for _py in _OPTIONAL[_name]:
        _owner, _, _attr = _py.rpartition(".")
        if _owner:
            delattr(globals()[_owner], _attr)
        else:
            del globals()[_attr]
```

### include/fhespear.h

```cpp
#ifndef FHESPEAR_H
#define FHESPEAR_H
#include <stddef.h>
#include <stdint.h>

#ifdef __cplusplus
extern "C" {
#endif

typedef int fhs_status;
enum {
    FHS_OK = 0,
    FHS_ERR_INVALID = 1,
    FHS_ERR_OOM = 2,
    FHS_ERR_HIP = 3,
    FHS_ERR_LEVEL = 4,
    FHS_ERR_SCALE = 5,
    FHS_ERR_KEY = 6,
    FHS_ERR_NODEVICE = 7
};

typedef struct fhs_context fhs_context;
typedef struct fhs_ciphertext fhs_ciphertext;
typedef struct fhs_plaintext fhs_plaintext;
typedef struct fhs_secret_key fhs_secret_key;
typedef struct fhs_public_key fhs_public_key;
typedef struct fhs_relin_key fhs_relin_key;
typedef struct fhs_galois_keys fhs_galois_keys;

const char* fhs_last_error(void);
const char* fhs_version(void);
int fhs_device_count(void);
fhs_status fhs_device_pci_bus_id(int device, char* buf, int len);
fhs_status fhs_debug_fail_next_flushes(fhs_context* ctx, int count);
fhs_status fhs_debug_fail_alloc(fhs_context* ctx, int nth, int* was_armed);
enum { FHS_LEDGER_ARM = 0, FHS_LEDGER_DISARM = 1, FHS_LEDGER_READ = 2 };
fhs_status fhs_debug_launch_ledger(int op, char* buf, uint64_t len, uint64_t* needed);

fhs_status fhs_create_coeff_modulus(uint64_t N, const int* bit_sizes, int n, uint64_t* primes_out);
uint64_t fhs_galois_elt_from_step(int step, uint64_t N);

fhs_status fhs_context_create(uint64_t N, const uint64_t* primes, int nprimes, int special,
                              const uint64_t* galois_elts, int n_elts, int device, fhs_context** out);
fhs_status fhs_context_destroy(fhs_context* ctx);
fhs_status fhs_context_info(const fhs_context* ctx, uint64_t* N, int* L0, int* P, int* n_elts);
fhs_status fhs_context_galois_elts(const fhs_context* ctx, uint64_t* elts_out);
fhs_status fhs_synchronize(fhs_context* ctx);
fhs_status fhs_memory_in_use(fhs_context* ctx, uint64_t* bytes);

fhs_status fhs_secret_key_create(fhs_context* ctx, const uint8_t* key32 ,
                                 fhs_secret_key** out);
fhs_status fhs_secret_key_destroy(fhs_secret_key* sk);
fhs_status fhs_gen_public_key(fhs_context* ctx, fhs_secret_key* sk, fhs_public_key** out);
fhs_status fhs_gen_relin_key(fhs_context* ctx, fhs_secret_key* sk, fhs_relin_key** out);
fhs_status fhs_create_galois_keys(fhs_context* ctx, fhs_secret_key* sk, const uint64_t* elts, int n,
                                  fhs_galois_keys** out);
fhs_status fhs_public_key_destroy(fhs_public_key* pk);
fhs_status fhs_relin_key_destroy(fhs_relin_key* rk);
fhs_status fhs_galois_keys_destroy(fhs_galois_keys* gk);
fhs_status fhs_galois_keys_has(const fhs_galois_keys* gk, uint64_t elt, int* has);
fhs_status fhs_galois_key_export(fhs_context* ctx, const fhs_galois_keys* gk, uint64_t elt, uint64_t* host);
fhs_status fhs_relin_key_export(fhs_context* ctx, const fhs_relin_key* rk, uint64_t* host);
fhs_status fhs_secret_key_export(fhs_context* ctx, const fhs_secret_key* sk, uint64_t* host );
fhs_status fhs_galois_keys_import(fhs_context* ctx, const uint64_t* elts, int n,
                                  const uint64_t* host , fhs_galois_keys** out);
fhs_status fhs_relin_key_import(fhs_context* ctx, const uint64_t* host , fhs_relin_key** out);
fhs_status fhs_secret_key_import(fhs_context* ctx, const uint64_t* host ,
                                 fhs_secret_key** out);
#define FHS_KS_EXACT 0
#define FHS_KS_SEAL 1
fhs_status fhs_context_set_key_switch_mode(fhs_context* ctx, int mode);
fhs_status fhs_context_key_switch_mode(const fhs_context* ctx, int* mode);
fhs_status fhs_seal_hoist_stats(fhs_context* ctx, uint64_t* hoisted, uint64_t* fallback);
fhs_status fhs_public_key_export(fhs_context* ctx, const fhs_public_key* pk, uint64_t* host );
fhs_status fhs_galois_keys_bytes(const fhs_galois_keys* gk, uint64_t* bytes);

fhs_status fhs_ciphertext_destroy(fhs_ciphertext* ct);
fhs_status fhs_plaintext_destroy(fhs_plaintext* pt);
fhs_status fhs_ciphertext_info(const fhs_ciphertext* ct, int* ncomp, int* chain_index, int* nlimbs, double* scale);
fhs_status fhs_ciphertext_set_scale(fhs_ciphertext* ct, double scale);
fhs_status fhs_plaintext_info(const fhs_plaintext* pt, int* chain_index, int* nlimbs, double* scale);
fhs_status fhs_ciphertext_export(fhs_context* ctx, const fhs_ciphertext* ct, uint64_t* host);
fhs_status fhs_ciphertext_import(fhs_context* ctx, const uint64_t* host, int ncomp, int chain_index, double scale,
                                 fhs_ciphertext** out);
fhs_status fhs_plaintext_export(fhs_context* ctx, const fhs_plaintext* pt, uint64_t* host);
fhs_status fhs_plaintext_import(fhs_context* ctx, const uint64_t* host, int chain_index, double scale,
                                fhs_plaintext** out);
fhs_status fhs_ciphertext_device_ptr(const fhs_ciphertext* ct, void** dptr, uint64_t* bytes);

fhs_status fhs_encode(fhs_context* ctx, const double* re_im, size_t n, double scale, int chain_index,
                      fhs_plaintext** out);
fhs_status fhs_encode_batch(fhs_context* ctx, const double* re_im, size_t count, size_t n, double scale,
                            int chain_index, fhs_plaintext** out_array);
fhs_status fhs_encode_real(fhs_context* ctx, const double* values, size_t n, double scale, int chain_index,
                           fhs_plaintext** out);
fhs_status fhs_encode_real_batch(fhs_context* ctx, const double* values, size_t count, size_t n, double scale,
                                 int chain_index, fhs_plaintext** out_array);
fhs_status fhs_decode(fhs_context* ctx, const fhs_plaintext* pt, double* re_im_out);
fhs_status fhs_decode_batch(fhs_context* ctx, const fhs_plaintext* const* pts, int count, int nslots,
                            double* re_im_out);

fhs_status fhs_encrypt_symmetric(fhs_context* ctx, fhs_secret_key* sk, const fhs_plaintext* pt, fhs_ciphertext** out);
fhs_status fhs_encrypt_symmetric_batch(fhs_context* ctx, fhs_secret_key* sk, const fhs_plaintext* const* pts, int count,
                                       fhs_ciphertext** out_array);
fhs_status fhs_encode_encrypt_symmetric_batch(fhs_context* ctx, fhs_secret_key* sk, const double* values, size_t count,
                                              size_t n, int is_real, double scale, int chain_index,
                                              fhs_ciphertext** out_array);
fhs_status fhs_decrypt_decode_batch(fhs_context* ctx, fhs_secret_key* sk, const fhs_ciphertext* const* cts, int count,
                                    int nslots, double* re_im_out);
fhs_status fhs_encrypt_asymmetric(fhs_context* ctx, fhs_public_key* pk, const fhs_plaintext* pt, fhs_ciphertext** out);
fhs_status fhs_encrypt_asymmetric_batch(fhs_context* ctx, fhs_public_key* pk, const fhs_plaintext* const* pts, int count,
                                        fhs_ciphertext** out_array);
fhs_status fhs_encode_encrypt_asymmetric_batch(fhs_context* ctx, fhs_public_key* pk, const double* values, size_t count,
                                               size_t n, int is_real, double scale, int chain_index,
                                               fhs_ciphertext** out_array);
fhs_status fhs_decrypt(fhs_context* ctx, fhs_secret_key* sk, const fhs_ciphertext* ct, fhs_plaintext** out);

fhs_status fhs_add(fhs_context* ctx, const fhs_ciphertext* a, const fhs_ciphertext* b, fhs_ciphertext** out);
// ... 87 lines not shown
```

Before: 155.8.

## Fork giant-step special-limb chain onto a high-priority side stream

During the BSGS giant-step keyswitch, the modup is split into a special-limb part and a data-limb part. The special-limb inner product, special INTT and giant_sum run on a second high-priority stream, concurrently with the data-limb modup and inner-product sum on the main stream, and the two streams are joined before the final kernel. The modup grid now uses a balancing map that spreads special-limb blocks evenly across the 8 XCDs, and some kernels switch from the XCD mapping to a plain block mapping. This adds event fork/join overhead and extra stream synchronisation, and it only activates above a work threshold.

```diff
diff --git a/fhe-spear_amd/csrc/fhs_host.hip b/fhe-spear_amd/csrc/fhs_host.hip
--- a/fhe-spear_amd/csrc/fhs_host.hip
+++ b/fhe-spear_amd/csrc/fhs_host.hip
@@ -87,6 +87,7 @@
 struct fhs_context {
     int device = 0;
     hipStream_t st = nullptr;
+    fhs::KsSide side{};
     std::recursive_mutex mu;
     uint64_t N = 0;
     int logN = 0, L0 = 0, P = 0, K = 0, dnum = 0;
@@ -220,6 +221,7 @@
 
 static void ctx_sync(fhs_context* c) {
     hipStreamSynchronize(c->st);
+    if (c->side.st) hipStreamSynchronize(c->side.st);
 }
 static void trim_cache(fhs_context* c) {
     if (c->free_blocks.empty()) return;
@@ -769,6 +771,13 @@
     c->fft_w = std::move(H.fft_w);
     c->slot_index = std::move(H.slot_index);
     HIPCHK(hipStreamCreateWithFlags(&c->st, hipStreamNonBlocking), "hipStreamCreate");
+    {
+        int prio_lo = 0, prio_hi = 0;
+        HIPCHK(hipDeviceGetStreamPriorityRange(&prio_lo, &prio_hi), "hipDeviceGetStreamPriorityRange");
+        HIPCHK(hipStreamCreateWithPriority(&c->side.st, hipStreamNonBlocking, prio_hi), "hipStreamCreate (side)");
+    }
+    HIPCHK(hipEventCreateWithFlags(&c->side.fork, hipEventDisableTiming), "hipEventCreate (fork)");
+    HIPCHK(hipEventCreateWithFlags(&c->side.join, hipEventDisableTiming), "hipEventCreate (join)");
     {
         static std::once_flag exit_once;
         std::call_once(exit_once, [] { atexit(release_at_exit); });
@@ -844,6 +853,9 @@
             for (auto& pr : v) { ev_put(pr.first); ev_put(pr.second); }
         for (hipEvent_t e : c->timer_open)
             if (e) ev_put(e);
+        if (c->side.fork) hipEventDestroy(c->side.fork);
+        if (c->side.join) hipEventDestroy(c->side.join);
+        if (c->side.st) hipStreamDestroy(c->side.st);
         if (c->st) hipStreamDestroy(c->st);
     }
     delete c;
@@ -1306,6 +1318,13 @@
     if (!c || count < 0) return fail(FHS_ERR_INVALID, "debug_fail_next_flushes: bad args");
     Guard g(c);
     c->debug_fail_flushes = count;
+    return FHS_OK;
+}
+extern "C" fhs_status fhs_debug_force_fork(fhs_context* c, int on, uint64_t* forked) {
+    if (!c) return fail(FHS_ERR_INVALID, "debug_force_fork: null context");
+    Guard g(c);
+    if (on >= 0) c->side.min_wg = on ? 0 : fhs::kForkMinWg;
+    if (forked) *forked = c->side.forked;
     return FHS_OK;
 }
 extern "C" fhs_status fhs_debug_fail_alloc(fhs_context* c, int nth, int* was_armed) {
@@ -2483,7 +2502,7 @@
     HIPCHK(scratch(c, fhs_context::SCR_BSGS_SUM, 16 * S, &sum), "bsgs sum");
     ht.mark("workspaces");
     HIPCHK(fhs::launch_bsgs(c->T, dbaby, dpts, G, Beff, D, l, keys.data(), akeys.data(), giant_elts, inner, sum, ws, wsb,
-                            c->items_dev, c->stager, c->st, tm, ptl),
+                            c->items_dev, c->stager, c->st, tm, ptl, &c->side),
            "bsgs");
     ht.mark("launch bsgs");
     if (!rescale) {
@@ -2706,7 +2725,7 @@
     HIPCHK(scratch(c, fhs_context::SCR_BSGS_SUM, 16 * S, &sum), "bsgs_giant_steps");
     const fhs::KTimer* tm = c->timer_mask ? &c->ktimer : nullptr;
     HIPCHK(fhs::launch_bsgs(c->T, nullptr, nullptr, 1, B, B, l, keys.data(), akeys.data(), ge.data(), inner, sum, ws, wsb,
-                            c->items_dev, c->stager, c->st, tm),
+                            c->items_dev, c->stager, c->st, tm, 0, &c->side),
            "bsgs_giant_steps");
     NEW_CT(r, 2, ci, scale);
     HIPCHK(hipMemcpyAsync(r->d, sum, 16 * S, hipMemcpyDeviceToDevice, c->st), "bsgs_giant_steps");
diff --git a/fhe-spear_amd/csrc/fhs_kernels.h b/fhe-spear_amd/csrc/fhs_kernels.h
--- a/fhe-spear_amd/csrc/fhs_kernels.h
+++ b/fhe-spear_amd/csrc/fhs_kernels.h
@@ -90,6 +90,13 @@
     void* user;
     hipError_t (*h2d)(void* user, void* dst, const void* src, size_t bytes);
 };
+constexpr int kForkMinWg = 8 * 256;
+struct KsSide {
+    hipStream_t st = nullptr;
+    hipEvent_t fork = nullptr, join = nullptr;
+    int min_wg = kForkMinWg;
+    unsigned long long forked = 0;
+};
 hipError_t launch_keyswitch(const DevTables& T, const KsItem* items_host, int R, const u64* const* uniq_host, int U,
                             int l, u64* workspace, size_t ws_bytes, void* items_dev, const Stager& sg, hipStream_t st,
                             const KTimer* tm, SealHoist* sh = nullptr);
@@ -99,7 +106,7 @@
 hipError_t launch_bsgs(const DevTables& T, const u64* const* baby_dev, const u64* const* pts_dev, int G, int B, int D,
                        int l, const u64* const* keys_host, const u64* const* akeys_host, const u64* giant_elts, u64* inner,
                        u64* out, u64* workspace, size_t ws_bytes, void* items_dev, const Stager& sg, hipStream_t st,
-                       const KTimer* tm, int ptl = 0);
+                       const KTimer* tm, int ptl = 0, KsSide* side = nullptr);
 hipError_t launch_bsgs_inner(const DevTables& T, const u64* const* baby_dev, const u64* const* pts_dev, int G, int g0,
                              int g1, int D, int l, u64* inner, hipStream_t st, int ptl = 0);
 hipError_t launch_dot_tensor(const DevTables& T, const u64* const* q_dev, const u64* const* db_dev, int J, int C, int l,
diff --git a/fhe-spear_amd/csrc/fhs_kernels.hip b/fhe-spear_amd/csrc/fhs_kernels.hip
--- a/fhe-spear_amd/csrc/fhs_kernels.hip
+++ b/fhe-spear_amd/csrc/fhs_kernels.hip
@@ -8,6 +8,7 @@
 #endif
 #include "fhs_ntt.h"
 #include "fhs_buffer.h"
+#include "fhs_xcdmap.h"
 
 #include <atomic>
 #include <cxxabi.h>
@@ -121,35 +122,6 @@
     return reinterpret_cast<const PrimeK*>(T.primes)[i];
 }
 
-__host__ __device__ __forceinline__ int xcd_grid(int E, int M) { return 8 * ((E + 7) / 8) * M; }
-__device__ __forceinline__ bool xcd_tinner(int E, int M, int& t, int& m) {
-    const int b = blockIdx.x, x = b & 7, k = b >> 3, nx = (E - x + 7) >> 3;
-    if (nx <= 0 || k >= nx * M) return false;
-    t = x + 8 * (k % nx);
-    m = k / nx;
-    return true;
-}
-__host__ __device__ __forceinline__ int xcd_grid_q(int E, int M) { return 8 * ((E + 3) / 4) * ((M + 1) / 2); }
-__device__ __forceinline__ bool xcd_quadpair(int E, int M, int& t, int& m) {
-    const int b = blockIdx.x, x = b & 7, k = b >> 3, pg = x & 3, mh = x >> 2;
-    const int nx = (E - pg + 3) >> 2, nm = (M - mh + 1) >> 1;
-    if (nx <= 0 || nm <= 0 || k >= nx * nm) return false;
-    t = pg + 4 * (k % nx);
-    m = mh + 2 * (k / nx);
-    return true;
-}
-__device__ __forceinline__ bool plain_tm(int E, int M, int& t, int& m) {
-    t = blockIdx.x % E;
-    m = blockIdx.x / E;
-    return m < M;
-}
-__device__ __forceinline__ bool xcd_touter(int E, int M, int& t, int& m) {
-    const int b = blockIdx.x, x = b & 7, k = b >> 3, nx = (E - x + 7) >> 3;
-    if (nx <= 0 || k >= nx * M) return false;
-    t = x + 8 * (k / M);
-    m = k % M;
-    return true;
-}
 __device__ __forceinline__ int limb_prime(int b, int l_split, int L0) { return b < l_split ? b : L0 + (b - l_split); }
 
 __device__ __forceinline__ int galois_src(int e, u64 elt, int logN) {
@@ -641,7 +613,7 @@
     __shared__ __attribute__((aligned(16))) u64 lds[ntt_lds_words<LOGN, false>()];
     const int tid = threadIdx.x;
     int i, u;
-    if (!plain_tm(l, U, i, u)) return;
+    if (!plain_tm(blockIdx.x, l, U, i, u)) return;
     const PrimeK& P = PK(T, i);
     const u64* src = uniq[u] + (size_t)i * N;
 #pragma unroll
@@ -661,7 +633,7 @@
     __shared__ __attribute__((aligned(16))) u64 lds[(1 << (LOGN - 1)) + (1 << (LOGN - 1)) / 16];
     const int tid = threadIdx.x;
     int i, u;
-    if (!plain_tm(l, U, i, u)) return;
+    if (!plain_tm(blockIdx.x, l, U, i, u)) return;
     const PrimeK& P = PK(T, i);
     const u64 q = P.q;
     const __amdgpu_buffer_rsrc_t rs = brsrc(uniq[u] + (size_t)i * N, N * 8);
@@ -826,7 +798,7 @@
     __shared__ __attribute__((aligned(16))) u64 lds[ntt_lds_words<LOGN, false>()];
     const int P_ = T.P, K = T.K, E = l + P_, dn = (l + P_ - 1) / P_;
     int t, mi;
-    if (!xcd_tinner(E, dn * U, t, mi)) return;
+    if (!xcd_tinner(blockIdx.x, E, dn * U, t, mi)) return;
     const int j = mi % dn, u = mi / dn;
     const int s0 = j * P_, s1 = min(s0 + P_, l), ns = s1 - s0;
     u64* o = ext + (((size_t)u * dn + j) * E + t) * N;
@@ -1054,32 +1026,31 @@
 template <int LOGN, int DP, bool B59>
 __global__ void __launch_bounds__((1 << LOGN) / 32, 4) k_modup_h(DevTables T, const u64* const* uniq,
                                                                  const u64* acoef, const unsigned char* vcnt, u64* ext,
-                                                                 int l, int U) {
+                                                                 int l, int U, ModupMap mp) {
     __shared__ __attribute__((aligned(16))) u64 lds[modup_h_lds_words<LOGN>()];
-    const int E = l + T.P, dn = (l + T.P - 1) / T.P;
     int t, mi;
-    if (!xcd_quadpair(E, dn * U, t, mi)) return;
+    if (!modup_map(mp, blockIdx.x, l, T.P, t, mi)) return;
     modup_h_body<LOGN, DP, B59>(T, acoef, vcnt, ext, l, t, mi, threadIdx.x, lds);
 }
 
 template <int LOGN>
 static void launch_modup(const DevTables& T, const u64* const* uniq, const u64* acoef, const unsigned char* vcnt,
-                         u64* ext, int l, int U, hipStream_t st) {
-    const int E = l + T.P, M = (l + T.P - 1) / T.P * U;
-    void (*k)(DevTables, const u64* const*, const u64*, const unsigned char*, u64*, int, int);
-    dim3 g(xcd_grid_q(E, M)), b((1 << LOGN) / 32);
+                         u64* ext, int l, int U, hipStream_t st, int part = kModupAll) {
     if constexpr (!ks_uses_half(LOGN)) {
-        k = k_modup<LOGN>;
-        g = dim3(xcd_grid(E, M));
-        b = dim3((1 << LOGN) / 16);
-    } else if (modup_xform(T, l)) {
-        k = T.conv_b59 ? k_modup_h<LOGN, 3, true> : k_modup_h<LOGN, 3, false>;
-    } else if (T.modup_dp == 1) {
-        k = T.all_b59 ? k_modup_h<LOGN, 1, true> : k_modup_h<LOGN, 1, false>;
+        const int E = l + T.P, M = (l + T.P - 1) / T.P * U;
+        FHS_LAUNCH(k_modup<LOGN>, dim3(xcd_grid(E, M)), dim3((1 << LOGN) / 16), 0, st, T, uniq, acoef, vcnt, ext, l, U);
     } else {
-        k = k_modup_h<LOGN, 0, false>;
-    }
-    FHS_LAUNCH(k, g, b, 0, st, T, uniq, acoef, vcnt, ext, l, U);
+        void (*k)(DevTables, const u64* const*, const u64*, const unsigned char*, u64*, int, int, ModupMap);
+        if (modup_xform(T, l)) {
+            k = T.conv_b59 ? k_modup_h<LOGN, 3, true> : k_modup_h<LOGN, 3, false>;
+        } else if (T.modup_dp == 1) {
+            k = T.all_b59 ? k_modup_h<LOGN, 1, true> : k_modup_h<LOGN, 1, false>;
+        } else {
+            k = k_modup_h<LOGN, 0, false>;
+        }
+        const ModupMap mp = modup_map_build(l, T.P, U, part);
+        FHS_LAUNCH(k, dim3(mp.grid), dim3((1 << LOGN) / 32), 0, st, T, uniq, acoef, vcnt, ext, l, U, mp);
+    }
 }
 
 struct KsOps {
@@ -1136,11 +1107,11 @@
     acc3_fold(c1, a1);
 }
 __global__ void __launch_bounds__(256) k_ks_ip(DevTables T, const KsItem* items, const u64* const* uniq, const u64* ext,
-                                                u64* acc, int l, int R, int t0) {
+                                                u64* acc, int l, int R, int t0, int t1) {
     const int N = T.N, P_ = T.P, K = T.K, E = l + P_, dn = (l + P_ - 1) / P_;
     const int NB = N >> 8;
     int t, m;
-    if (!(t0 > 0 ? plain_tm(E - t0, R * NB, t, m) : xcd_touter(E - t0, R * NB, t, m))) return;
+    if (!(t0 > 0 ? plain_tm(blockIdx.x, t1 - t0, R * NB, t, m) : xcd_touter(blockIdx.x, t1, R * NB, t, m))) return;
     t += t0;
     int r, nb;
     if (FHS_KSIP_HALVES && t0 == 0 && NB >= 2 && (size_t)dn * N * 8 > ((size_t)3 << 20)) {
@@ -1179,7 +1150,7 @@
     const int N = T.N, P_ = T.P, K = T.K, E = l + P_, dn = (l + P_ - 1) / P_;
     const int NB = N >> 8;
     int t, m;
-    if (!xcd_touter(l, NB, t, m)) return;
+    if (!plain_tm(blockIdx.x, l, NB, t, m)) return;
     const int n = (m << 8) + threadIdx.x;
     const RedU RD = redu(PK(T, t));
     const u64 q = RD.q;
@@ -1244,7 +1215,7 @@
     __shared__ __attribute__((aligned(16))) u64 lds[ntt_lds_words<LOGN, false>()];
     const int P_ = T.P, E = l + P_;
     int i, m;
-    if (!plain_tm(l, 2 * R, i, m)) return;
+    if (!plain_tm(blockIdx.x, l, 2 * R, i, m)) return;
     const int comp = m & 1, r = m >> 1;
     const PrimeK& P = PK(T, i);
     const u64 q = P.q;
@@ -1558,19 +1529,47 @@
     launch_modup<LOGN>(T, uniq, b.acoef, b.vcnt, b.ext, l, U, st);
     FHS_TMARK(tm, KID_MODUP, 0, st);
 }
+struct SideFork {
+    KsSide* s;
+    hipStream_t st;
+    bool open = false;
+    SideFork(KsSide* s_, hipStream_t st_) : s(s_), st(st_) {}
+    SideFork(const SideFork&) = delete;
+    SideFork& operator=(const SideFork&) = delete;
+    ~SideFork() { (void)join(); }
+    hipError_t fork() {
+        hipError_t e = hipEventRecord(s->fork, st);
+        if (e == hipSuccess) e = hipStreamWaitEvent(s->st, s->fork, 0);
+        if (e != hipSuccess) return e;
+        open = true;
+        ++s->forked;
+        return hipSuccess;
+    }
+    hipError_t join() {
+        if (!open) return hipSuccess;
+        open = false;
+        hipError_t e = hipEventRecord(s->join, s->st);
+        if (e == hipSuccess) e = hipStreamWaitEvent(st, s->join, 0);
+        if (e != hipSuccess) (void)hipStreamSynchronize(s->st);
+        return e;
+    }
+};
+static bool side_forks(const KsSide* s, int logN, long long data_wg) {
+    return s && s->st && ks_uses_half(logN) && data_wg >= s->min_wg;
+}
 static void ks_ip_stage(const DevTables& T, const KsItem* it, const u64* const* uniq, int R, int l, const KsBufs& b,
-                        hipStream_t st, const KTimer* tm) {
-    FHS_TMARK(tm, KID_KS_IP, 1, st);
-    FHS_LAUNCH(k_ks_ip, dim3(xcd_grid(l + T.P, R * (T.N >> 8))), dim3(256), 0, st, T, it, uniq, b.ext, b.acc, l, R,
-               0);
-    FHS_TMARK(tm, KID_KS_IP, 0, st);
-}
-static void giant_ip_stage(const DevTables& T, const KsItem* it, const u64* const* uniq, int R, int l, const KsBufs& b,
-                           hipStream_t st, const KTimer* tm) {
+                        hipStream_t st, const KTimer* tm, int t0, int t1) {
     const int NB = T.N >> 8;
     FHS_TMARK(tm, KID_KS_IP, 1, st);
-    FHS_LAUNCH(k_ks_ip, dim3(T.P * R * NB), dim3(256), 0, st, T, it, uniq, b.ext, b.acc, l, R, l);
-    FHS_LAUNCH(k_ks_ip_sum, dim3(xcd_grid(l, NB)), dim3(256), 0, st, T, it, uniq, b.ext, b.acc, l, R);
+    FHS_LAUNCH(k_ks_ip, dim3(t0 > 0 ? plain_grid(t1 - t0, R * NB) : xcd_grid(t1, R * NB)), dim3(256), 0, st, T, it, uniq,
+               b.ext, b.acc, l, R, t0, t1);
+    FHS_TMARK(tm, KID_KS_IP, 0, st);
+}
+static void giant_ip_sum_stage(const DevTables& T, const KsItem* it, const u64* const* uniq, int R, int l, const KsBufs& b,
+                               hipStream_t st, const KTimer* tm) {
+    const int NB = T.N >> 8;
+    FHS_TMARK(tm, KID_KS_IP, 1, st);
+    FHS_LAUNCH(k_ks_ip_sum, dim3(plain_grid(l, NB)), dim3(256), 0, st, T, it, uniq, b.ext, b.acc, l, R);
     FHS_TMARK(tm, KID_KS_IP, 0, st);
 }
 template <int LOGN>
@@ -1664,6 +1663,15 @@
     return hipGetLastError();
 }
 
+template <int LOGN>
+static hipError_t ks_product_stages(const DevTables& T, const KsItem* it, const u64* const* uq, int R, int U, int l,
+                                    const KsBufs& b, hipStream_t st, const KTimer* tm) {
+    ks_modup_stage<LOGN>(T, uq, U, l, b, st, tm);
+    ks_ip_stage(T, it, uq, R, l, b, st, tm, 0, l + T.P);
+    ks_special_intt_stage<LOGN>(T, R, l, b, st, tm);
+    return ks_moddown_stage<LOGN>(T, it, R, l, b, st, tm);
+}
+
 hipError_t launch_keyswitch(const DevTables& T, const KsItem* items_host, int R, const u64* const* uniq_host, int U,
                             int l, u64* ws, size_t ws_bytes, void* items_dev, const Stager& sg, hipStream_t st,
                             const KTimer* tm, SealHoist* sh) {
@@ -1688,12 +1696,7 @@
             return launch_keyswitch(T, items_host, R, uniq_host, U, l, ws, ws_bytes, items_dev, sg, st, tm, nullptr);
         }
         ++sh->hoisted;
-        FHS_DISPATCH_LOGN(T.logN, {
-            ks_modup_stage<LOGN>(T, uq, U, l, b, st, tm);
-            ks_ip_stage(T, it, uq, R, l, b, st, tm);
-            ks_special_intt_stage<LOGN>(T, R, l, b, st, tm);
-            e = ks_moddown_stage<LOGN>(T, it, R, l, b, st, tm);
-        });
+        FHS_DISPATCH_LOGN(T.logN, e = ks_product_stages<LOGN>(T, it, uq, R, U, l, b, st, tm));
         if (e != hipSuccess) return e;
         return hipGetLastError();
     }
@@ -1714,10 +1717,7 @@
     const KsBufs b = ks_carve(T, ws, R, U, l);
     FHS_DISPATCH_LOGN(T.logN, {
         ks_intt_stage<LOGN>(T, uq, U, l, b, st, tm);
-        ks_modup_stage<LOGN>(T, uq, U, l, b, st, tm);
-        ks_ip_stage(T, it, uq, R, l, b, st, tm);
-        ks_special_intt_stage<LOGN>(T, R, l, b, st, tm);
-        me = ks_moddown_stage<LOGN>(T, it, R, l, b, st, tm);
+        me = ks_product_stages<LOGN>(T, it, uq, R, U, l, b, st, tm);
     });
     if (me != hipSuccess) return me;
     return hipGetLastError();
@@ -1848,9 +1848,11 @@
 #ifndef FHS_GSUM_ICH
 #define FHS_GSUM_ICH 4
 #endif
-__global__ void __launch_bounds__(256) k_giant_sum(DevTables T, const u64* bpart, const u64* ycoef, const u64* inner0,
-                                                   u64* base, u64* convsum, int l, int R) {
-    const int N = T.N, P_ = T.P, E = l + P_;
+#ifndef FHS_GSUM_RB
+#define FHS_GSUM_RB 8
+#endif
+__global__ void __launch_bounds__(256) k_giant_sum(DevTables T, const u64* ycoef, u64* convsum, int l, int R) {
+    const int N = T.N, P_ = T.P;
     const int n = blockIdx.x * blockDim.x + threadIdx.x, comp = blockIdx.y;
     if (n >= N) return;
     const int i0 = blockIdx.z * FHS_GSUM_ICH, i1 = min(i0 + FHS_GSUM_ICH, l);
@@ -1859,14 +1861,24 @@
     u64 ylo[PMAX], yhi[PMAX];
 #pragma unroll
     for (int k = 0; k < PMAX; ++k) ylo[k] = yhi[k] = 0;
-    for (int r = 0; r < R; ++r) {
-        const u64* y = ycoef + ((size_t)r * 2 + comp) * P_ * N + n;
-#pragma unroll
-        for (int k = 0; k < PMAX; ++k) {
-            if (k < P_) {
-                const u64 v = y[(size_t)k * N];
-                ylo[k] += v;
-                yhi[k] += ylo[k] < v;
+    for (int r0 = 0; r0 < R; r0 += FHS_GSUM_RB) {
+        u64 v[FHS_GSUM_RB][PMAX];
+#pragma unroll
+        for (int j = 0; j < FHS_GSUM_RB; ++j) {
+            const bool on = r0 + j < R;
+            const u64* y = ycoef + ((size_t)(on ? r0 + j : r0) * 2 + comp) * P_ * N + n;
+#pragma unroll
+            for (int k = 0; k < PMAX; ++k)
+                if (k < P_) v[j][k] = on ? y[(size_t)k * N] : 0;
+        }
+#pragma unroll
+        for (int j = 0; j < FHS_GSUM_RB; ++j) {
+#pragma unroll
+            for (int k = 0; k < PMAX; ++k) {
+                if (k < P_) {
+                    ylo[k] += v[j][k];
+                    yhi[k] += ylo[k] < v[j][k];
+                }
             }
         }
     }
@@ -1886,25 +1898,25 @@
             cs.lo = submod(cs.lo, rh, q);
         }
         u64 cv = reduce128(cs.lo, cs.hi, P);
-        const size_t idx = (size_t)comp * S + (size_t)i * N + n;
-        const u64 bv = addmod(bpart[((size_t)comp * E + i) * N + n], inner0[idx], q);
-        convsum[idx] = cv;
-        base[idx] = bv;
+        convsum[(size_t)comp * S + (size_t)i * N + n] = cv;
     }
 }
 template <int LOGN, bool H = ntt_half<LOGN>()>
-__global__ void __launch_bounds__((ntt_threads<LOGN, H>())) k_giant_final(DevTables T, const u64* base, const u64* convsum,
-                                                                     u64* out, int l) {
+__global__ void __launch_bounds__((ntt_threads<LOGN, H>())) k_giant_final(DevTables T, const u64* bpart, const u64* inner0,
+                                                                     const u64* convsum, u64* out, int l) {
     constexpr int N = 1 << LOGN;
     __shared__ __attribute__((aligned(16))) u64 lds[ntt_lds_words<LOGN, H>()];
     const int i = blockIdx.x, comp = blockIdx.y;
     const PrimeK& P = PK(T, i);
     const RedU RU = redu(P);
-    const size_t off = ((size_t)comp * l + i) * N;
+    const size_t off = ((size_t)comp * l + i) * N, boff = ((size_t)comp * (l + T.P) + i) * N;
     const u64 pinv = T.md_pinv[2 * i], pinv_s = T.md_pinv[2 * i + 1], q = RU.q;
     fwd_limb<LOGN, FHS_NTT_RL, H>(lds, threadIdx.x, T.tw_fwd + (size_t)i * N * 2, RU,
                                [&](int e) { return convsum[off + e]; },
-                               [&](int e, u64 v) { out[off + e] = submod(base[off + e], shoup(v, pinv, pinv_s, q), q); });
+                               [&](int e, u64 v) {
+                                   out[off + e] = submod(addmod(bpart[boff + e], inner0[off + e], q),
+                                                         shoup(v, pinv, pinv_s, q), q);
+                               });
 }
 
 size_t bsgs_workspace_bytes(const DevTables& T, int R, int l) {
@@ -2088,7 +2100,7 @@
 hipError_t launch_bsgs(const DevTables& T, const u64* const* baby_dev, const u64* const* pts_dev, int G, int B, int D,
                        int l, const u64* const* keys_host, const u64* const* akeys_host, const u64* giant_elts, u64* inner,
                        u64* out, u64* ws, size_t ws_bytes, void* items_dev, const Stager& sg, hipStream_t st,
-                       const KTimer* tm, int ptl) {
+                       const KTimer* tm, int ptl, KsSide* side) {
     const int R = B - 1;
     const size_t N = T.N, S = (size_t)l * N;
     if (T.N % 128 || G < 1 || R > 512) return hipErrorInvalidValue;
@@ -2130,22 +2142,48 @@
         he = seal_permute(T, seal_orig.data(), R, l, seal_perm, st);
         if (he != hipSuccess) return he;
     }
-    u64* base = ws + keyswitch_workspace_bytes(T, R, R, l) / 8;
-    u64* convsum = base + 2 * S;
+    u64* convsum = ws + keyswitch_workspace_bytes(T, R, R, l) / 8 + 2 * S;
+    hipError_t ge = hipSuccess;
     FHS_DISPATCH_LOGN(T.logN, {
         const KsBufs b = ks_carve(T, ws, R, R, l);
+        const int E = l + T.P, dn = (E - 1) / T.P;
+        SideFork sf(side, st);
+        auto special_chain = [&](hipStream_t cs) {
+            ks_ip_stage(T, it, uq, R, l, b, cs, tm, l, E);
+            ks_special_intt_stage<LOGN>(T, R, l, b, cs, tm);
+            FHS_TMARK(tm, KID_GIANT_SUM, 1, cs);
+            FHS_LAUNCH(k_giant_sum, dim3((T.N + 255) / 256, 2, (l + FHS_GSUM_ICH - 1) / FHS_GSUM_ICH), dim3(256), 0, cs, T,
+                       b.ycoef, convsum, l, R);
+            FHS_TMARK(tm, KID_GIANT_SUM, 0, cs);
+        };
         ks_intt_stage<LOGN>(T, uq, R, l, b, st, tm);
-        ks_modup_stage<LOGN>(T, uq, R, l, b, st, tm);
-        giant_ip_stage(T, it, uq, R, l, b, st, tm);
-        ks_special_intt_stage<LOGN>(T, R, l, b, st, tm);
-        FHS_TMARK(tm, KID_GIANT_SUM, 1, st);
-        FHS_LAUNCH(k_giant_sum, dim3((T.N + 255) / 256, 2, (l + FHS_GSUM_ICH - 1) / FHS_GSUM_ICH), dim3(256), 0,
-                   st, T, b.acc, b.ycoef, inner, base, convsum, l, R);
-        FHS_TMARK(tm, KID_GIANT_SUM, 0, st);
-        FHS_TMARK(tm, KID_GIANT_FINAL, 1, st);
-        FHS_NTT_LAUNCH(k_giant_final, l * 2, dim3(l, 2), st, T, base, convsum, out, l);
-        FHS_TMARK(tm, KID_GIANT_FINAL, 0, st);
+        if (!side_forks(side, LOGN, (long long)l * dn * R)) {
+            ks_modup_stage<LOGN>(T, uq, R, l, b, st, tm);
+            special_chain(st);
+            giant_ip_sum_stage(T, it, uq, R, l, b, st, tm);
+        } else {
+            if constexpr (ks_uses_half(LOGN)) {
+                FHS_TMARK(tm, KID_MODUP, 1, st);
+                launch_modup<LOGN>(T, uq, b.acoef, b.vcnt, b.ext, l, R, st, kModupSpecial);
+                FHS_TMARK(tm, KID_MODUP, 0, st);
+                ge = sf.fork();
+                if (ge == hipSuccess) {
+                    special_chain(side->st);
+                    FHS_TMARK(tm, KID_MODUP, 1, st);
+                    launch_modup<LOGN>(T, uq, b.acoef, b.vcnt, b.ext, l, R, st, kModupData);
+                    FHS_TMARK(tm, KID_MODUP, 0, st);
+                    giant_ip_sum_stage(T, it, uq, R, l, b, st, tm);
+                    ge = sf.join();
+                }
+            }
+        }
+        if (ge == hipSuccess) {
+            FHS_TMARK(tm, KID_GIANT_FINAL, 1, st);
+            FHS_NTT_LAUNCH(k_giant_final, l * 2, dim3(l, 2), st, T, b.acc, inner, convsum, out, l);
+            FHS_TMARK(tm, KID_GIANT_FINAL, 0, st);
+        }
     });
+    if (ge != hipSuccess) return ge;
     return hipGetLastError();
 }
 
diff --git a/fhe-spear_amd/csrc/fhs_xcdmap.h b/fhe-spear_amd/csrc/fhs_xcdmap.h
--- /dev/null
+++ b/fhe-spear_amd/csrc/fhs_xcdmap.h
@@ -0,0 +1,116 @@
+#pragma once
+
+#if defined(__HIPCC__)
+#define FHS_HD __host__ __device__ __forceinline__
+#else
+#define FHS_HD inline
+#endif
+
+namespace fhs {
+
+constexpr int kXcds = 8;
+
+FHS_HD int plain_grid(int E, int M) { return E * M; }
+FHS_HD bool plain_tm(int b, int E, int M, int& t, int& m) {
+    t = b % E;
+    m = b / E;
+    return m < M;
+}
+
+FHS_HD int xcd_grid(int E, int M) { return kXcds * ((E + 7) / 8) * M; }
+FHS_HD bool xcd_tinner(int b, int E, int M, int& t, int& m) {
+    const int x = b & 7, k = b >> 3, nx = (E - x + 7) >> 3;
+    if (nx <= 0 || k >= nx * M) return false;
+    t = x + 8 * (k % nx);
+    m = k / nx;
+    return true;
+}
+
+FHS_HD bool xcd_touter(int b, int E, int M, int& t, int& m) {
+    const int x = b & 7, k = b >> 3, nx = (E - x + 7) >> 3;
+    if (nx <= 0 || k >= nx * M) return false;
+    t = x + 8 * (k / M);
+    m = k % M;
+    return true;
+}
+
+enum ModupPart { kModupAll = 0, kModupSpecial = 1, kModupData = 2 };
+struct ModupMap {
+    int nd[kXcds];
+    int sp[kXcds + 1];
+    int grid;
+};
+FHS_HD int modup_real_limbs(int l, int P, int j, int pg) {
+    const int s0 = j * P, s1 = s0 + P < l ? s0 + P : l;
+    int n = 0;
+    for (int t = pg; t < l; t += 4) n += !(t >= s0 && t < s1);
+    return n;
+}
+inline ModupMap modup_map_build(int l, int P, int U, int part) {
+    const int E = l + P, dn = (E - 1) / P, M = dn * U;
+    ModupMap mp;
+    long long real[kXcds];
+    int cnt[kXcds];
+    for (int x = 0; x < kXcds; ++x) {
+        const int pg = x & 3, mh = x >> 2;
+        const int nxd = l > pg ? (l - pg + 3) >> 2 : 0, nm = M > mh ? (M - mh + 1) >> 1 : 0;
+        mp.nd[x] = part == kModupSpecial ? 0 : nxd * nm;
+        real[x] = 0;
+        cnt[x] = 0;
+        if (part == kModupSpecial) continue;
+        for (int j = 0; j < dn; ++j) {
+            const int same = (j & 1) == mh;
+            const int nu = dn & 1 ? (U + same) / 2 : same * U;
+            real[x] += (long long)nu * modup_real_limbs(l, P, j, pg);
+        }
+    }
+    const long long S = part == kModupData ? 0 : (long long)P * M;
+    long long left = S;
+    for (;;) {
+        long long lo = real[0] + cnt[0], next = -1;
+        for (int x = 1; x < kXcds; ++x) lo = real[x] + cnt[x] < lo ? real[x] + cnt[x] : lo;
+        int nlo = 0;
+        for (int x = 0; x < kXcds; ++x) {
+            const long long v = real[x] + cnt[x];
+            if (v == lo) ++nlo;
+            else if (next < 0 || v < next) next = v;
+        }
+        if (left <= 0) break;
+        long long rise = next < 0 ? (left + nlo - 1) / nlo : next - lo;
+        if (rise * nlo > left) rise = left / nlo;
+        if (rise == 0) {
+            for (int x = 0; x < kXcds && left > 0; ++x)
+                if (real[x] + cnt[x] == lo) { ++cnt[x]; --left; }
+            break;
+        }
+        for (int x = 0; x < kXcds; ++x)
+            if (real[x] + cnt[x] == lo) cnt[x] += (int)rise;
+        left -= rise * nlo;
+    }
+    mp.sp[0] = 0;
+    int g = 0;
+    for (int x = 0; x < kXcds; ++x) {
+        mp.sp[x + 1] = mp.sp[x] + cnt[x];
+        g = mp.nd[x] + cnt[x] > g ? mp.nd[x] + cnt[x] : g;
+    }
+    mp.grid = kXcds * g;
+    return mp;
+}
+FHS_HD bool modup_map(const ModupMap& mp, int b, int l, int P, int& t, int& m) {
+    const int x = b & 7, pg = x & 3, mh = x >> 2;
+    int k = b >> 3;
+    if (k < mp.nd[x]) {
+        const int nxd = (l - pg + 3) >> 2;
+        t = pg + 4 * (k % nxd);
+        m = mh + 2 * (k / nxd);
+        return true;
+    }
+    k -= mp.nd[x];
+    if (k >= mp.sp[x + 1] - mp.sp[x]) return false;
+    const int s = mp.sp[x] + k;
+    t = l + s % P;
+    m = s / P;
+    return true;
+}
+
+}
diff --git a/fhe-spear_amd/python/pyPhantom/__init__.py b/fhe-spear_amd/python/pyPhantom/__init__.py
--- a/fhe-spear_amd/python/pyPhantom/__init__.py
+++ b/fhe-spear_amd/python/pyPhantom/__init__.py
@@ -170,6 +170,7 @@
     "fhs_staging_stats": (C.c_int, [_vp, C.POINTER(C.c_uint64), C.POINTER(C.c_uint64)]),
     "fhs_debug_fail_next_flushes": (C.c_int, [_vp, C.c_int]),
     "fhs_debug_fail_alloc": (C.c_int, [_vp, C.c_int, _ip]),
+    "fhs_debug_force_fork": (C.c_int, [_vp, C.c_int, _u64p]),
     "fhs_debug_launch_ledger": (C.c_int, [C.c_int, C.c_char_p, _u64, _u64p]),
 }
 _OPTIONAL = {
@@ -1076,6 +1077,12 @@
     _check(_lib.fhs_debug_fail_next_flushes(ctx._h, int(count)), "debug_fail_next_flushes")
 
 
+def debug_force_fork(ctx, on=None):
+    n = C.c_uint64(0)
+    _check(_lib.fhs_debug_force_fork(ctx._h, -1 if on is None else int(bool(on)), C.byref(n)), "debug_force_fork")
+    return int(n.value)
+
+
 def debug_fail_alloc(ctx, nth):
     was = C.c_int()
     _check(_lib.fhs_debug_fail_alloc(ctx._h, int(nth), C.byref(was)), "debug_fail_alloc")
diff --git a/include/fhespear.h b/include/fhespear.h
--- a/include/fhespear.h
+++ b/include/fhespear.h
@@ -33,6 +33,7 @@
 fhs_status fhs_device_pci_bus_id(int device, char* buf, int len);
 fhs_status fhs_debug_fail_next_flushes(fhs_context* ctx, int count);
 fhs_status fhs_debug_fail_alloc(fhs_context* ctx, int nth, int* was_armed);
+fhs_status fhs_debug_force_fork(fhs_context* ctx, int on, uint64_t* forked);
 enum { FHS_LEDGER_ARM = 0, FHS_LEDGER_DISARM = 1, FHS_LEDGER_READ = 2 };
 fhs_status fhs_debug_launch_ledger(int op, char* buf, uint64_t len, uint64_t* needed);
 
```

Measured after the change: 162.5, median of 6. +4.3%, better.
